# zzuiekongning/MGDT-YOLO

Measured on AMD Instinct MI355X. Metric: images/sec @640x640 bs=32 per GPU, detection forward + NMS (whole job: 1 GPU(s)), higher is better.
Workload: dtype bf16; 1 GPU; mspa_c2f_gd_yolov8-n (MSPA-C2f + GD neck + Detect, nc=80) 640x640 inference, batch 32/GPU: forward + decode + NMS(conf 0.25, iou 0.7), hipGraph replay, 4 batches in flight (one captured graph per resident batch, replayed round-robin on 4 streams); global_batch=32, parallelism=replicas x1 (batch-sharded, no data-path collective), rccl_ranks=1, input=bfloat16 NCHW images, 8 different batches resident in HBM (600 MiB) cycled, detections_last_step=9600, weights=seeded random init (no checkpoints offline), batches_in_flight=4

## Files before the change

include/mgdt.h:

```cpp
#ifndef MGDT_H
#define MGDT_H
#include <stddef.h>
#include <stdint.h>

#ifdef __cplusplus
extern "C" {
#endif

typedef void* mgdt_stream;

typedef enum { MGDT_OK = 0, MGDT_BAD_SHAPE = -1, MGDT_BAD_DTYPE = -2, MGDT_LAUNCH_FAIL = -3, MGDT_BAD_ARG = -4,
               MGDT_WORKSPACE = -5 } mgdt_status;
typedef enum { MGDT_F32 = 0, MGDT_BF16 = 1, MGDT_U8 = 2  } mgdt_dtype;
typedef enum { MGDT_ACT_NONE = 0, MGDT_ACT_SILU = 1, MGDT_ACT_RELU = 2, MGDT_ACT_GELU = 3 } mgdt_act;

typedef struct {
  void* p;
  int32_t n, h, w, c;
  int64_t sn, sh, sw, sc;
} mgdt_view;

const char* mgdt_last_error(void);
const char* mgdt_version(void);

// ... 55 lines not shown
                         float stride, int a_off, int a_total, const mgdt_view* feat, float* y, unsigned long long* best_keys,
                         const void* wb3, const float* bb3, mgdt_stream s);
int mgdt_detect_tail_aug_fwd(const mgdt_view* tb, const mgdt_view* tc, const void* wb, const float* bb, const void* wc, const float* bc, int nc,
                             float stride, int a_off, int a_total, const mgdt_view* feat, float* y, unsigned long long* best_keys,
                             const void* wb3, const float* bb3, float aug_scale, int aug_flip, float aug_img_w, mgdt_stream s);

int mgdt_scale_img_fwd(const mgdt_view* x, int x_dtype, int flip, int hs, int ws, float pad, const mgdt_view* y, int y_dtype, mgdt_stream s);

int mgdt_csp_block_supported(int mode, int cin, int cout, int wd, int nbtl, int h, int w, int dtype);
int mgdt_csp_block_tiles(int mode, int n, int cin, int cout, int wd, int nbtl, int h, int w, int* geom8);
int mgdt_csp_block_fwd(int mode, const mgdt_view* x, const void* front, const float* front_bias, const void* const* mid,
                       const float* const* mid_bias, int nbtl, int shortcut, const void* back, const float* back_bias, int wd, int act,
                       const mgdt_view* y, float* pool, int dtype, mgdt_stream s);

size_t mgdt_pw_chain_packed_bytes(int wd, int dtype);
int mgdt_pw_chain_pack(int idx, const float* w_oi, const float* conv_bias, const float* bn_gamma, const float* bn_beta, const float* bn_mean,
                       const float* bn_var, float bn_eps, int wd, int dtype, void* packed, mgdt_stream s);
int mgdt_pw_chain3_fwd(const mgdt_view* x, const void* packed, int wd, int act, const mgdt_view* y, int dtype, mgdt_stream s);

int mgdt_conv1x1_inject_supported(int cin, int cout, int h, int w, int hg, int wg, int dtype);
int mgdt_conv1x1_inject_fwd(const mgdt_view* x, const void* packed_w, const float* bias, const mgdt_view* ga, const mgdt_view* gf,
                            const mgdt_view* y, int dtype, mgdt_stream s);

int mgdt_conv1x1_inject_conv_supported(int cin, int cmid, int cout2, int h, int w, int hg, int wg, int dtype);
int mgdt_conv1x1_inject_conv_fwd(const mgdt_view* x, const void* packed_w, const float* bias, const mgdt_view* ga, const mgdt_view* gf,
                                 const mgdt_view* gsrc, const void* packed_wg, const float* bias_g, int cmid,
                                 const void* packed_w2, const float* bias2, int act2, const mgdt_view* y2, int dtype, mgdt_stream s);

size_t mgdt_groupnorm_workspace_bytes(int n, int c);
int mgdt_groupnorm_fwd(const mgdt_view* x, const float* gamma, const float* beta, int groups, float eps, int act, void* ws, const mgdt_view* y,
                       int dtype, mgdt_stream s);
int mgdt_tood_layer_attn_fwd(const float* sums, int n, int c, int hw, const float* w1, const float* b1, const float* w2, const float* b2, int hid,
                             int stacked, float* scale, mgdt_stream s);
int mgdt_dcnv2_fwd(const mgdt_view* x, const mgdt_view* offset_mask, const float* w_gemm, const float* bias, const mgdt_view* y, int dtype,
                   mgdt_stream s);
int mgdt_dcnv2_mfma_fwd(const mgdt_view* x, const mgdt_view* offset_mask, const void* packed_w, const mgdt_view* y, int dtype, mgdt_stream s);
int mgdt_pixel_gate_fwd(const mgdt_view* x, const mgdt_view* gate, const mgdt_view* y, int dtype, mgdt_stream s);

int mgdt_conv_pack_direct(const float* w_oihw, const float* conv_bias, const float* bn_gamma, const float* bn_beta,
                          const float* bn_mean, const float* bn_var, float bn_eps, int cin_g, int cout, int k,
                          float* w_out, float* bias_out, mgdt_stream s);
int mgdt_conv2d_direct_fwd(const mgdt_view* x, int x_dtype, const float* w_gemm, const float* bias, int k, int stride,
                           int groups, int act, const mgdt_view* y, int dtype, mgdt_stream s);
enum { MGDT_DIRECT_STEM = 0, MGDT_DIRECT_GENERIC = 1, MGDT_DIRECT_REFUSED = 2 };
int mgdt_conv2d_direct_route(const mgdt_view* x, int x_dtype, const mgdt_view* y, int dtype, int k, int stride, int groups, int* out);

#define MGDT_SPR_SPLITS 16
int mgdt_spr_pool_fwd(const mgdt_view* x, float* pooled, int dtype, mgdt_stream s);
int mgdt_spr_attn_fwd(const float* pooled, const float* fc1_w, const float* fc1_b, const float* fc2_w,
                      const float* fc2_b, int n, int c, int groups, int h, int w, int softmax, float* attn, mgdt_stream s);
int mgdt_scale_channels_fwd(const mgdt_view* x, const float* attn, const mgdt_view* y, int dtype, mgdt_stream s);
int mgdt_spr_attn_scale_fwd(const float* pooled, int nsplit, int tiles_x, int tiles_y, const float* fc1_w, const float* fc1_b, const float* fc2_w, const float* fc2_b, int groups,
                            const mgdt_view* x, const mgdt_view* y, const mgdt_view* pool_a, const mgdt_view* pool_b, int dtype, mgdt_stream s);

int mgdt_sppf_pool_fwd(const mgdt_view* x, const mgdt_view* y1, const mgdt_view* y2, const mgdt_view* y3, int dtype,
                       mgdt_stream s);

int mgdt_adaptive_avgpool_fwd(const mgdt_view* x, const mgdt_view* y, int dtype, mgdt_stream s);
int mgdt_bilinear_fwd(const mgdt_view* x, const mgdt_view* y, int dtype, mgdt_stream s);
int mgdt_nearest_fwd(const mgdt_view* x, const mgdt_view* y, int dtype, mgdt_stream s);
int mgdt_copy_fwd(const mgdt_view* x, int x_dtype, const mgdt_view* y, int y_dtype, mgdt_stream s);
int mgdt_image_pad4_fwd(const mgdt_view* x, int x_dtype, const mgdt_view* y, int y_dtype, mgdt_stream s);

int mgdt_space_to_depth2_channels(int c, int y_dtype);
int mgdt_conv_pack_stem6(const float* w6, const float* conv_bias, const float* bn_gamma, const float* bn_beta, const float* bn_mean, const float* bn_var,
                         float bn_eps, int c6, int cout, int dtype, void* packed_out, float* bias_out, mgdt_stream s);
int mgdt_space_to_depth2_fwd(const mgdt_view* x, int x_dtype, const mgdt_view* y, int y_dtype, mgdt_stream s);
int mgdt_stem6_wgrad_unpack(const float* dw3, int cout, int cin, int cp, float* dw6, mgdt_stream s);

#define MGDT_GRN_SPLITS 8
int mgdt_dwconv7_ln_fwd(const mgdt_view* x, const float* dw_w, const float* dw_b, const float* ln_w, const float* ln_b,
                        float eps, const mgdt_view* y, int dtype, mgdt_stream s);
int mgdt_grn_stats_fwd(const mgdt_view* t, const float* gamma, float* ws, float* scale, int dtype, mgdt_stream s);
enum { MGDT_DW_ROW8 = 0, MGDT_DW_ROW10 = 1, MGDT_DW_GENERIC = 2 };
int mgdt_dwconv7_ln_route(int n, int h, int w, int c, int dtype, int* out);

int mgdt_inject_fwd(const mgdt_view* local, const mgdt_view* ga, const mgdt_view* gf, const mgdt_view* y, int dtype,
                    mgdt_stream s);

int mgdt_detect_decode_fwd(const mgdt_view* feat, int reg_max, int nc, float stride, int a_off, int a_total, float* y,
                           int dtype, mgdt_stream s);
int mgdt_detect_decode_aug_fwd(const mgdt_view* feat, int reg_max, int nc, float stride, int a_off, int a_total, float* y,
                               unsigned long long* best_keys, float aug_scale, int aug_flip, float aug_img_w, int dtype, mgdt_stream s);

size_t mgdt_nms_workspace_bytes(int n, int nc, int a, int multi_label, int max_nms);
int mgdt_nms_fwd(const float* pred, int n, int nc, int a, float conf_thres, float iou_thres, const int32_t* classes,
                 int n_classes, int agnostic, int multi_label, int max_det, int max_nms, float max_wh, float* out,
                 int32_t* kept_anchor, int32_t* counts, const unsigned long long* best_keys, void* ws, size_t ws_bytes, mgdt_stream s);

int mgdt_nms_masks_fwd(const float* pred, int n, int nc, int nm, int a, float conf_thres, float iou_thres, const int32_t* classes,
                       int n_classes, int agnostic, int multi_label, int max_det, int max_nms, float max_wh, float* out,
                       int32_t* kept_anchor, int32_t* counts, const unsigned long long* best_keys, void* ws, size_t ws_bytes, mgdt_stream s);

int mgdt_deconv2x2_fwd(const mgdt_view* x, const void* const* packed4, const float* bias, const mgdt_view* y, int dtype, mgdt_stream s);
int mgdt_seg_concat_fwd(const float* y, int n, int rows, int a_total, const mgdt_view* const* mc, int n_levels, int nm, float* out, int dtype,
                        mgdt_stream s);
int mgdt_seg_mask_geometry(int win_h, int win_w, int out_h, int out_w, int* geom4);
int mgdt_seg_masks_fwd(const mgdt_view* protos, const float* rows, const int32_t* counts, const int32_t* offsets, int max_det, int nm,
                       int top, int left, int win_h, int win_w, int out_h, int out_w, int crop_before, float box_sx, float box_sy,
                       int crop_after, int no_skip, void* out, int out_u8, int dtype, mgdt_stream s);

int mgdt_pose_concat_fwd(const float* y, int n, int rows, int a_total, const mgdt_view* const* kpt, const float* strides, int n_levels, int nk,
                         int ndim, float* out, float* kpt_raw, int dtype, mgdt_stream s);
int mgdt_pose_scale_fwd(float* rows, const int32_t* counts, const float* meta, int n, int max_det, int lead, int nk, int ndim, mgdt_stream s);

size_t mgdt_mask_iou_workspace_bytes(int n, int max_det, int max_lab);
// ... 189 lines not shown
```

mgdt_yolo_amd/_lib.py:

```python
import ctypes as C
import os

_HERE = os.path.dirname(os.path.abspath(__file__))
LIB_PATH = os.environ.get('MGDT_LIB') or os.path.join(_HERE, 'csrc', 'libmgdt_hip.so')

F32, BF16 = 0, 1
ACT_NONE, ACT_SILU, ACT_RELU, ACT_GELU = 0, 1, 2, 3
SPR_SPLITS = 16
GRN_SPLITS = 8


class View(C.Structure):
    _fields_ = [('p', C.c_void_p), ('n', C.c_int32), ('h', C.c_int32), ('w', C.c_int32), ('c', C.c_int32),
                ('sn', C.c_int64), ('sh', C.c_int64), ('sw', C.c_int64), ('sc', C.c_int64)]


VP = C.POINTER(View)
_vp, _i, _f, _sz, _l = C.c_void_p, C.c_int, C.c_float, C.c_size_t, C.c_long

class PackDesc(C.Structure):
    _fields_ = [('w', C.c_void_p), ('conv_bias', C.c_void_p), ('bn_gamma', C.c_void_p), ('bn_beta', C.c_void_p), ('bn_mean', C.c_void_p), ('bn_var', C.c_void_p),
                ('bn_eps', C.c_float), ('cin', C.c_int32), ('cout', C.c_int32), ('k', C.c_int32), ('dtype', C.c_int32), ('mode', C.c_int32),
                ('packed', C.c_void_p), ('bias_out', C.c_void_p)]

# ... 9 lines not shown

ROUTE_X2, ROUTE_IN_SCALE, ROUTE_IN_SHIFT, ROUTE_R1, ROUTE_R2, ROUTE_FP8 = 1, 2, 4, 8, 16, 32
ROUTE_IGEMM, ROUTE_LDS3X3 = 0, 1
DIRECT_STEM, DIRECT_GENERIC, DIRECT_REFUSED = 0, 1, 2

PROTOTYPES = {
    'mgdt_last_error': (C.c_char_p, []),
    'mgdt_version': (C.c_char_p, []),
    'mgdt_conv_packed_bytes': (_sz, [_i, _i, _i, _i]),
    'mgdt_conv_pack': (_i, [_vp, _vp, _vp, _vp, _vp, _vp, _f, _i, _i, _i, _i, _vp, _vp, _vp]),
    'mgdt_conv2d_fwd': (_i, [VP, VP, _vp, _vp, _vp, _vp, _i, _i, _i, VP, VP, VP, _i, _vp]),
    'mgdt_conv_packed_bytes_fp8': (_sz, [_i, _i, _i]),
    'mgdt_conv_pack_fp8': (_i, [_vp, _vp, _vp, _vp, _vp, _vp, _f, _i, _i, _i, _f, _vp, _vp, _vp, _vp]),
    'mgdt_conv2d_fp8_fwd': (_i, [VP, VP, _vp, _vp, _vp, _vp, _vp, _f, _i, _i, _i, VP, VP, VP, _vp]),
    'mgdt_conv2d_route': (_i, [VP, VP, _i, _i, _i, _i, _i, C.POINTER(ConvRoute)]),
    'mgdt_conv_pack_batch': (_i, [_vp, _i, _vp]),
    'mgdt_conv2d_phase_fwd': (_i, [VP, _vp, _vp, _i, VP, VP, VP, _i, _vp]),
    'mgdt_conv_wgrad_splits': (_i, [_i, _i, _i]),
    'mgdt_wgrad_final_batch': (_i, [_vp, _i, _vp]),
    'mgdt_conv_pack_dgrad': (_i, [_vp, _i, _i, _i, _i, _i, _vp, _vp, _vp]),
    'mgdt_conv_pack_direct': (_i, [_vp, _vp, _vp, _vp, _vp, _vp, _f, _i, _i, _i, _vp, _vp, _vp]),
    'mgdt_conv2d_direct_fwd': (_i, [VP, _i, _vp, _vp, _i, _i, _i, _i, VP, _i, _vp]),
    'mgdt_conv2d_direct_route': (_i, [VP, _i, VP, _i, _i, _i, _i, C.POINTER(C.c_int)]),
    'mgdt_spr_pool_fwd': (_i, [VP, _vp, _i, _vp]),
    'mgdt_spr_attn_fwd': (_i, [_vp, _vp, _vp, _vp, _vp, _i, _i, _i, _i, _i, _i, _vp, _vp]),
    'mgdt_scale_channels_fwd': (_i, [VP, _vp, VP, _i, _vp]),
    'mgdt_sppf_pool_fwd': (_i, [VP, VP, VP, VP, _i, _vp]),
    'mgdt_adaptive_avgpool_fwd': (_i, [VP, VP, _i, _vp]),
    'mgdt_bilinear_fwd': (_i, [VP, VP, _i, _vp]),
    'mgdt_nearest_fwd': (_i, [VP, VP, _i, _vp]),
    'mgdt_copy_fwd': (_i, [VP, _i, VP, _i, _vp]),
    'mgdt_image_pad4_fwd': (_i, [VP, _i, VP, _i, _vp]),
    'mgdt_space_to_depth2_channels': (_i, [_i, _i]),
    'mgdt_space_to_depth2_fwd': (_i, [VP, _i, VP, _i, _vp]),
    'mgdt_conv_pack_stem6': (_i, [_vp, _vp, _vp, _vp, _vp, _vp, _f, _i, _i, _i, _vp, _vp, _vp]),
    'mgdt_stem6_wgrad_unpack': (_i, [_vp, _i, _i, _i, _vp, _vp]),
    'mgdt_dwconv7_ln_fwd': (_i, [VP, _vp, _vp, _vp, _vp, _f, VP, _i, _vp]),
    'mgdt_cnx_mlp_packed_bytes': (_sz, [_i, _i]),
    'mgdt_cnx_mlp_pack': (_i, [_vp, _vp, _vp, _vp, _i, _vp, _i, _vp]),
    'mgdt_cnx_mlp_workspace_bytes': (_sz, [_i, _i, _i, _i]),
    'mgdt_cnx_mlp_fwd': (_i, [VP, VP, _vp, _vp, _vp, _vp, VP, _i, _vp]),
    'mgdt_cnx_block_supported': (_i, [_i, _i, _i, _i, _i]),
    'mgdt_cnx_block_workspace_bytes': (_sz, [_i, _i, _i, _i]),
    'mgdt_cnx_block_geometry': (_i, [_i, _i, _i, C.POINTER(C.c_int)]),
    'mgdt_cnx_block_fwd': (_i, [VP, _vp, _vp, _vp, _vp, _f, _vp, _vp, _vp, _vp, _vp, _i, _vp, _sz, VP, _i, _vp]),
    'mgdt_pw_chain_packed_bytes': (_sz, [_i, _i]),
    'mgdt_pw_chain_pack': (_i, [_i, _vp, _vp, _vp, _vp, _vp, _vp, _f, _i, _i, _vp, _vp]),
    'mgdt_pw_chain3_fwd': (_i, [VP, _vp, _i, _i, VP, _i, _vp]),
    'mgdt_conv1x1_inject_supported': (_i, [_i, _i, _i, _i, _i, _i, _i]),
    'mgdt_conv1x1_inject_fwd': (_i, [VP, _vp, _vp, VP, VP, VP, _i, _vp]),
    'mgdt_conv1x1_inject_conv_supported': (_i, [_i, _i, _i, _i, _i, _i, _i, _i]),
    'mgdt_conv1x1_inject_conv_fwd': (_i, [VP, _vp, _vp, VP, VP, VP, _vp, _vp, _i, _vp, _vp, _i, VP, _i, _vp]),
    'mgdt_spr_attn_scale_fwd': (_i, [_vp, _i, _i, _i, _vp, _vp, _vp, _vp, _i, VP, VP, VP, VP, _i, _vp]),
    'mgdt_stem2_packed_bytes': (_sz, []),
    'mgdt_stem2_pack': (_i, [_vp, _vp, _vp]),
    'mgdt_stem2_fwd': (_i, [VP, _i, _vp, _vp, _vp, _vp, VP, _vp]),
    'mgdt_stem2_geometry': (_i, [_i, _i, _i, _i, C.POINTER(C.c_int)]),
    'mgdt_stem2_route': (_i, [VP, _i, VP, _i, C.POINTER(C.c_int)]),
    'mgdt_detect_tail_supported': (_i, [_i, _i, _i, _i, _i]),
    'mgdt_detect_tail_fwd': (_i, [VP, VP, _vp, _vp, _vp, _vp, _i, _f, _i, _i, VP, _vp, _vp, _vp, _vp, _vp]),
    'mgdt_detect_tail_aug_fwd': (_i, [VP, VP, _vp, _vp, _vp, _vp, _i, _f, _i, _i, VP, _vp, _vp, _vp, _vp, _f, _i, _f, _vp]),
    'mgdt_scale_img_fwd': (_i, [VP, _i, _i, _i, _i, _f, VP, _i, _vp]),
    'mgdt_csp_block_supported': (_i, [_i, _i, _i, _i, _i, _i, _i, _i]),
    'mgdt_csp_block_tiles': (_i, [_i, _i, _i, _i, _i, _i, _i, _i, _vp]),
    'mgdt_csp_block_fwd': (_i, [_i, VP, _vp, _vp, _vp, _vp, _i, _i, _vp, _vp, _i, _i, VP, _vp, _i, _vp]),
    'mgdt_groupnorm_workspace_bytes': (_sz, [_i, _i]),
    'mgdt_groupnorm_fwd': (_i, [VP, _vp, _vp, _i, _f, _i, _vp, VP, _i, _vp]),
    'mgdt_tood_layer_attn_fwd': (_i, [_vp, _i, _i, _i, _vp, _vp, _vp, _vp, _i, _i, _vp, _vp]),
    'mgdt_dcnv2_fwd': (_i, [VP, VP, _vp, _vp, VP, _i, _vp]),
    'mgdt_dcnv2_mfma_fwd': (_i, [VP, VP, _vp, VP, _i, _vp]),
    'mgdt_pixel_gate_fwd': (_i, [VP, VP, VP, _i, _vp]),
    'mgdt_gn_affine': (_i, [_vp, _vp, _i, _i, _i, _vp, _vp, _i, _f, _vp, _vp, _vp, _vp, _vp]),
    'mgdt_nc_affine_act_bwd': (_i, [VP, VP, _vp, _vp, _i, VP, _i, _vp]),
    'mgdt_gn_bwd_workspace_bytes': (_sz, [_i, _i]),
    'mgdt_gn_bwd_coef': (_i, [_vp, _vp, _vp, _vp, _vp, _i, _i, _i, _i, _vp, _vp, _vp, _vp, _vp, _i, _vp, _vp]),
    'mgdt_nc_axpby': (_i, [VP, _vp, VP, _vp, _vp, VP, _i, _vp]),
    'mgdt_pixel_gate_bwd': (_i, [VP, VP, VP, VP, VP, _i, _vp]),
    'mgdt_tood_layer_attn_bwd_workspace_bytes': (_sz, [_i, _i, _i, _i]),
    'mgdt_tood_layer_attn_bwd': (_i, [_vp, _vp, _i, _i, _i, _vp, _vp, _vp, _vp, _i, _i, _vp, _vp, _vp, _vp, _vp, _i, _vp, _vp]),
    'mgdt_dcn_im2col': (_i, [VP, VP, VP, _i, _vp]),
    'mgdt_dcn_col2im_bwd': (_i, [VP, VP, VP, _vp, VP, _i, _vp]),
    'mgdt_val_match_fwd': (_i, [_vp, _vp, _i, _i, _vp, _vp, _i, _vp, _i, _vp, _vp]),
    'mgdt_grn_stats_fwd': (_i, [VP, _vp, _vp, _vp, _i, _vp]),
    'mgdt_dwconv7_ln_route': (_i, [_i, _i, _i, _i, _i, C.POINTER(C.c_int)]),
    'mgdt_inject_fwd': (_i, [VP, VP, VP, VP, _i, _vp]),
    'mgdt_detect_decode_fwd': (_i, [VP, _i, _i, _f, _i, _i, _vp, _i, _vp]),
    'mgdt_detect_decode_aug_fwd': (_i, [VP, _i, _i, _f, _i, _i, _vp, _vp, _f, _i, _f, _i, _vp]),
    'mgdt_detect_loss_workspace_bytes': (_sz, [_i, _i, _i]),
    'mgdt_detect_loss_fwd': (_i, [_vp, _vp, _i, _i, _i, _vp, _i, _i, _f, _f, _f, _vp, _vp, _vp, _vp, _vp, _sz, _i, _vp]),
    'mgdt_detect_loss_fwd_dev': (_i, [_vp, _vp, _i, _i, _i, _vp, _i, _vp, _f, _f, _f, _vp, _vp, _vp, _vp, _vp, _sz, _i, _vp]),
    'mgdt_detect_loss_bwd': (_i, [_vp, _vp, _vp, _i, _i, _i, _vp, _i, _f, _f, _f, _f, _vp, _vp, _sz, _i, _vp]),
    'mgdt_reduce_workspace_bytes': (_sz, [_i]),
    'mgdt_bn_stats_fwd': (_i, [VP, _f, _f, _vp, _vp, _vp, _vp, _vp, _i, _vp]),
    'mgdt_bn_act_fwd': (_i, [VP, _vp, _vp, _vp, _vp, _i, VP, VP, VP, _i, _vp]),
    'mgdt_bn_act_bwd': (_i, [VP, VP, _vp, _vp, _vp, _vp, _i, _vp, _vp, VP, _vp, _i, _vp]),
    'mgdt_conv_dgrad': (_i, [VP, _vp, _i, _i, VP, _i, _i, _vp]),
    'mgdt_gconv_dgrad': (_i, [VP, _vp, _i, _i, _i, VP, _i, _i, _vp]),
    'mgdt_gconv_wgrad_workspace_bytes': (_sz, [_i, _i, _i, _i]),
    'mgdt_gconv_wgrad': (_i, [VP, VP, _i, _i, _i, _vp, _i, _vp, _i, _vp]),
    'mgdt_conv_wgrad_workspace_bytes': (_sz, [_i, _i, _i]),
    'mgdt_conv_wgrad': (_i, [VP, VP, VP, _i, _i, _vp, _vp, _i, _vp, _i, _vp]),
    'mgdt_add_fwd': (_i, [VP, VP, VP, _i, _vp]),
    'mgdt_maxpool5_bwd': (_i, [VP, VP, _vp, _i, _vp]),
    'mgdt_nearest_bwd': (_i, [VP, VP, _i, _vp]),
    'mgdt_ew_binary': (_i, [VP, VP, VP, _i, _i, _vp]),
    'mgdt_channel_affine': (_i, [VP, _vp, _vp, VP, _i, _vp]),
# ... 94 lines not shown
```

mgdt_yolo_amd/csrc/conv3x3_lds.hip:

```cpp
#include <type_traits>
#include <vector>

#include "common.h"

#define C3_OOB ((int)0x80000000)
#define C3_TW 16
#define C3_RW 18
#define C3_MAXI 14

struct C3Args {
  const char* x; int xsn, xsh, xsw; uint32_t x_bytes;
  char* y; int ysn, ysh, ysw; uint32_t y_bytes;
  const char* wpk; const float* bias;
  int N, H, W, Ho, Wo, Cin, Cout, CP, nchunks, NTtot, ncg, tiles_x, tiles_per_img, ntiles, XP, act;
  FastDiv fd_tpi, fd_tx, fd_cp;
  const float* oscale; float xq;
  unsigned long long* dbg;
};

template <int ACT> __device__ __forceinline__ float c3_act(float v) {
  if (ACT == MGDT_ACT_SILU) return v * fast_sigmoid(v);
  if (ACT == MGDT_ACT_RELU) return fmaxf(v, 0.f);
  return v;
}

template <int NBW, int ACT, int NCH, int MT, bool Q8 = false, int S = 1, int WS = 1>
__global__ __launch_bounds__(256 * WS, 1) void conv3x3_lds_kernel(const C3Args a) {
  constexpr int NTHR = 256 * WS, NBH = (NBW + WS - 1) / WS;
  constexpr int RW = 15 * S + 3, TH = 4 * MT, RH = (TH - 1) * S + 3, RPX = RH * RW;
  constexpr int MAXI = ((S == 1 ? C3_MAXI : 18) + WS - 1) / WS;
  constexpr int WB = Q8 ? 512 : 1024, PB = Q8 ? 8 : 16;
  extern __shared__ __attribute__((aligned(16))) char c3_lds[];
  int* tab = (int*)c3_lds;
  char* wl = c3_lds + (((size_t)a.nchunks * 16 + 15) & ~(size_t)15);
  char* xs = wl + (size_t)a.nchunks * NBW * WB;
  const int tid = threadIdx.x, lane = tid & 63, r = lane & 15, g = lane >> 4;
  const int wave_all = __builtin_amdgcn_readfirstlane(tid >> 6);
  const int wave = wave_all & 3, wcol = wave_all >> 2;
  const int cg = blockIdx.x % a.ncg, w0 = blockIdx.x / a.ncg, wstep = gridDim.x / a.ncg;
  const int nb0 = cg * NBW;
  const __amdgpu_buffer_rsrc_t xrs = __builtin_amdgcn_make_buffer_rsrc((void*)a.x, 0, a.x_bytes, 0x00020000);
  const __amdgpu_buffer_rsrc_t yrs = __builtin_amdgcn_make_buffer_rsrc((void*)a.y, 0, a.y_bytes, 0x00020000);

  for (int p = tid; p < a.nchunks * 4; p += NTHR) {
    const int tap = (int)fdiv((uint32_t)p, a.fd_cp), cp = p - tap * a.CP;
    tab[p] = tap < 9 ? ((tap / 3) * RW + (tap % 3)) * a.XP + cp * PB : 0;
  }
  constexpr int WV = WB / 16;
  {
    const int total = a.nchunks * NBW * WV;
    for (int i0 = tid; i0 < total; i0 += 8 * NTHR) {
      uint4 t[8];
#pragma unroll
      for (int u = 0; u < 8; ++u) {
        const int i = min(i0 + u * NTHR, total - 1);
        const int kc = i / (NBW * WV), rem = i - kc * NBW * WV, bw = rem / WV, ln = rem % WV;
        const bool ok = nb0 + bw < a.NTtot;
        t[u] = ok ? *(const uint4*)(a.wpk + ((size_t)(kc * a.NTtot + nb0 + bw) * WV + ln) * 16) : make_uint4(0u, 0u, 0u, 0u);
      }
#pragma unroll
      for (int u = 0; u < 8; ++u)
        if (i0 + u * NTHR < total) *(uint4*)(wl + (size_t)(i0 + u * NTHR) * 16) = t[u];
    }
  }
  const int nbw0 = nb0 + wcol * NBH;
  f32x4 bias[NBH], osc[Q8 ? NBH : 1];
#pragma unroll
  for (int bw = 0; bw < NBH; ++bw) {
    bias[bw] = nbw0 + bw < a.NTtot ? *(const f32x4*)(a.bias + (nbw0 + bw) * 16 + 4 * g) : f32x4{0.f, 0.f, 0.f, 0.f};
    if constexpr (Q8) {
      osc[bw] = nbw0 + bw < a.NTtot ? *(const f32x4*)(a.oscale + (nbw0 + bw) * 16 + 4 * g) : f32x4{1.f, 1.f, 1.f, 1.f};
      bias[bw] = bias[bw] / osc[bw];
    }
  }

  const int nitems = RPX * a.CP;
  uint4 stage[MAXI];
  auto issue = [&](int t) {
    const int n = (int)fdiv((uint32_t)t, a.fd_tpi), rt = t - n * a.tiles_per_img;
    const int tyi = (int)fdiv((uint32_t)rt, a.fd_tx), txi = rt - tyi * a.tiles_x;
    const int iy0 = tyi * TH * S - 1, ix0 = txi * C3_TW * S - 1;
#pragma unroll
    for (int u = 0; u < MAXI; ++u) {
      const int it = tid + u * NTHR;
      const int pix = (int)fdiv((uint32_t)it, a.fd_cp), c8 = it - pix * a.CP;
      const int py = pix / RW, px = pix - py * RW;
      const int iy = iy0 + py, ix = ix0 + px;
      const bool ok = it < nitems && (unsigned)iy < (unsigned)a.H && (unsigned)ix < (unsigned)a.W;
      stage[u] = __builtin_bit_cast(uint4, __builtin_amdgcn_raw_buffer_load_b128(xrs, ok ? (uint32_t)(n * a.xsn + iy * a.xsh + ix * a.xsw + c8 * 16) : (uint32_t)C3_OOB, 0, 0));
    }
  };
  auto commit = [&]() {
#pragma unroll
    for (int u = 0; u < MAXI; ++u) {
      const int it = tid + u * NTHR;
      if (it < nitems) {
        const int pix = (int)fdiv((uint32_t)it, a.fd_cp), c8 = it - pix * a.CP;
        if constexpr (Q8) *(long*)(xs + pix * a.XP + c8 * 8) = quant8(__builtin_bit_cast(bf16x8, stage[u]), a.xq);
        else *(uint4*)(xs + pix * a.XP + c8 * 16) = stage[u];
      }
    }
  };

  const char* const wlane = wl + lane * PB;
  int bbase[MT];
#pragma unroll
  for (int m = 0; m < MT; ++m) bbase[m] = ((wave * MT + m) * S * RW + r * S) * a.XP;

  __builtin_amdgcn_s_waitcnt(0x0F70);
  unsigned long long T0 = 0, Tc = 0, Tm = 0, Te = 0, tl = 0, ntl = 0;
  if (a.dbg) { T0 = __builtin_amdgcn_s_memrealtime(); tl = T0; }
  int t = w0;
  if (t < a.ntiles) issue(t);
  while (t < a.ntiles) {
    __syncthreads();
    commit();
    __syncthreads();
    if (a.dbg) { const unsigned long long n_ = __builtin_amdgcn_s_memrealtime(); Tc += n_ - tl; tl = n_; }
    const int tn = t + wstep;
    if (tn < a.ntiles) issue(tn);

    f32x4 acc[NBH][MT];
#pragma unroll
    for (int bw = 0; bw < NBH; ++bw)
#pragma unroll
      for (int m = 0; m < MT; ++m) acc[bw][m] = bias[bw];
    typedef typename std::conditional<Q8, long, bf16x8>::type frag_t;
    frag_t A[2][NBH], B[2][MT];
    auto load_frags = [&](int kc, int buf) {
      const int off = tab[kc * 4 + g];
#pragma unroll
      for (int bw = 0; bw < NBH; ++bw) A[buf][bw] = *(const frag_t*)(wlane + (size_t)(kc * NBW + wcol * NBH + bw) * WB);
#pragma unroll
      for (int m = 0; m < MT; ++m) B[buf][m] = *(const frag_t*)(xs + bbase[m] + off);
    };
    auto mm = [&](frag_t w, frag_t p, f32x4 c) __attribute__((always_inline)) {
      if constexpr (Q8) return mma_q8(w, p, c);
      else return __builtin_amdgcn_mfma_f32_16x16x32_bf16(w, p, c, 0, 0, 0);
    };
    load_frags(0, 0);
    if (NCH > 0) {
#pragma unroll
      for (int kc = 0; kc < NCH; ++kc) {
        if (kc + 1 < NCH) load_frags(kc + 1, (kc + 1) & 1);
#pragma unroll
        for (int bw = 0; bw < NBH; ++bw)
#pragma unroll
          for (int m = 0; m < MT; ++m) acc[bw][m] = mm(A[kc & 1][bw], B[kc & 1][m], acc[bw][m]);
      }
    } else {
      for (int kc = 0; kc < a.nchunks; kc += 2) {
        if (kc + 1 < a.nchunks) load_frags(kc + 1, 1);
#pragma unroll
        for (int bw = 0; bw < NBH; ++bw)
#pragma unroll
          for (int m = 0; m < MT; ++m) acc[bw][m] = mm(A[0][bw], B[0][m], acc[bw][m]);
        if (kc + 1 < a.nchunks) {
          if (kc + 2 < a.nchunks) load_frags(kc + 2, 0);
#pragma unroll
          for (int bw = 0; bw < NBH; ++bw)
#pragma unroll
            for (int m = 0; m < MT; ++m) acc[bw][m] = mm(A[1][bw], B[1][m], acc[bw][m]);
        }
      }
    }

    if (a.dbg) { const unsigned long long n_ = __builtin_amdgcn_s_memrealtime(); Tm += n_ - tl; tl = n_; }
    {
      const int n = (int)fdiv((uint32_t)t, a.fd_tpi), rt = t - n * a.tiles_per_img;
      const int tyi = (int)fdiv((uint32_t)rt, a.fd_tx), txi = rt - tyi * a.tiles_x;
#pragma unroll
      for (int m = 0; m < MT; ++m) {
        const int oy = tyi * TH + wave * MT + m, ox = txi * C3_TW + r;
// ... 8 lines not shown
          __builtin_amdgcn_raw_buffer_store_b64(__builtin_bit_cast(__attribute__((__vector_size__(2 * sizeof(unsigned int)))) unsigned int, o), yrs,
                                                (pin && co < a.Cout) ? (uint32_t)(po + co * 2) : (uint32_t)C3_OOB, 0, 0);
        }
      }
    }
    if (a.dbg) { const unsigned long long n_ = __builtin_amdgcn_s_memrealtime(); Te += n_ - tl; tl = n_; ++ntl; }
    t = tn;
  }
  if (a.dbg && tid == 0) { unsigned long long* d = a.dbg + (size_t)blockIdx.x * 6; d[0] = T0; d[1] = tl; d[2] = Tc; d[3] = Tm; d[4] = Te; d[5] = ntl; }
}

bool mgdt_conv3x3_lds_plan(const mgdt_view* x, const mgdt_view* y, int act, int CP, int nchunks, int NTtot, bool q8, int stride, C3Plan* p) {
  static const int mode = getenv("MGDT_CONV3_LDS") ? atoi(getenv("MGDT_CONV3_LDS")) : 1;
  if (!mode) return false;
  static const bool ws2 = !(getenv("MGDT_C3_WAVES8") && atoi(getenv("MGDT_C3_WAVES8")) == 0);
  const bool wide = mode >= 3 || ws2;
  const int Cin = x->c, Cout = y->c;
  if (stride == 2 && (q8 || Cin > 64 || NTtot % 4 || (nchunks != 9 && !(nchunks == 18 && wide)))) return false;
  if (Cin % 8 || Cin < 32 || Cin > 80 || Cout % 4 || Cout < 32 || (act != MGDT_ACT_SILU && act != MGDT_ACT_NONE && act != MGDT_ACT_RELU)) return false;
  const long M = (long)x->n * x->h * x->w;
  if (M < 16 * 1024 || x->h < 16 || x->w < 16) return false;
  p->extx = ((long)(x->n - 1) * x->sn + (long)(x->h - 1) * x->sh + (long)(x->w - 1) * x->sw + x->c) * 2;
  p->exty = ((long)(y->n - 1) * y->sn + (long)(y->h - 1) * y->sh + (long)(y->w - 1) * y->sw + y->c) * 2;
  if (p->extx >= 0x7fffffffL || p->exty >= 0x7fffffffL) return false;
  p->XP = q8 ? Cin + 16 : Cin * 2 + 16;
  const int NBW = stride == 2 ? 4 : NTtot;
  if (NBW != 2 && NBW != 3 && NBW != 4 && NBW != 5 && NBW != 6) return false;
  p->NBW = NBW;
  p->ncg = NTtot / NBW;
  const size_t fixed = (((size_t)nchunks * 16 + 15) & ~(size_t)15) + (size_t)nchunks * NBW * (q8 ? 512 : 1024);
  auto region = [&](int mt) { return stride == 2 ? (size_t)(8 * mt + 1) * 33 * p->XP : (size_t)(4 * mt + 2) * C3_RW * p->XP; };
  int MT = stride == 2 ? 2 : 4;
  if (stride == 1 && fixed + region(MT) > 160 * 1024) MT = NBW == 5 && !q8 && wide && fixed + region(3) <= 160 * 1024 ? 3 : 2;
  p->lds = fixed + region(MT);
  if (p->lds > 160 * 1024) return false;
  if (NBW == 5 && !q8 && MT == 2 && mode < 2) return false;
  if (stride == 1 && (q8 ? MT != 4 : ((NBW == 5 && MT == 4) || (NBW != 5 && MT != 4)))) return false;
  p->MT = MT;
  const int TH = 4 * MT;
  p->tiles_x = cdiv(y->w, C3_TW);
  p->tiles_per_img = p->tiles_x * cdiv(y->h, TH);
  p->ntiles = x->n * p->tiles_per_img;
  if ((stride == 2 ? (2 * TH + 1) * 33 * CP > 256 * 18 : (TH + 2) * C3_RW * CP > 256 * C3_MAXI)) return false;
  int nwg = 256 / p->ncg * p->ncg;
  nwg = (int)std::min<long>(nwg, (long)p->ntiles * p->ncg);
  nwg = nwg / p->ncg * p->ncg;
  if (nwg < p->ncg) return false;
  p->nwg = nwg;
  p->waves = q8 ? 4 : (ws2 && (stride == 2 || NBW == 6 || NBW == 4 || (NBW == 5 && MT == 3))) ? 8 : 4;
  return true;
}

bool mgdt_conv3x3_lds_launch(const mgdt_view* x, const mgdt_view* y, const void* packed_w, const float* bias, int act, int CP, int nchunks, int NTtot, hipStream_t st,
                             const float* q8_oscale, float q8_xq, int stride) {
  const bool q8 = q8_oscale != nullptr;
  C3Plan pl;
  if (!mgdt_conv3x3_lds_plan(x, y, act, CP, nchunks, NTtot, q8, stride, &pl)) return false;
  const int Cin = x->c, Cout = y->c, NBW = pl.NBW, MT = pl.MT, nwg = pl.nwg;
  const size_t lds = pl.lds;
  const bool ws2 = pl.waves == 8;
  C3Args a;
  memset(&a, 0, sizeof(a));
  a.x = (const char*)x->p; a.xsn = (int)(x->sn * 2); a.xsh = (int)(x->sh * 2); a.xsw = (int)(x->sw * 2); a.x_bytes = (uint32_t)pl.extx;
  a.y = (char*)y->p; a.ysn = (int)(y->sn * 2); a.ysh = (int)(y->sh * 2); a.ysw = (int)(y->sw * 2); a.y_bytes = (uint32_t)pl.exty;
  a.wpk = (const char*)packed_w; a.bias = bias;
  a.N = x->n; a.H = x->h; a.W = x->w; a.Ho = y->h; a.Wo = y->w; a.Cin = Cin; a.Cout = Cout; a.CP = CP; a.nchunks = nchunks; a.NTtot = NTtot; a.act = act;
  a.XP = pl.XP;
  a.oscale = q8_oscale; a.xq = q8_xq;
  a.ncg = pl.ncg;
  a.tiles_x = pl.tiles_x; a.tiles_per_img = pl.tiles_per_img; a.ntiles = pl.ntiles;
  a.fd_tpi = make_fastdiv((uint32_t)a.tiles_per_img); a.fd_tx = make_fastdiv((uint32_t)a.tiles_x); a.fd_cp = make_fastdiv((uint32_t)CP);
 #define C3_LAUNCH_Q8(NB, ACTV)                                                                                      \
  {                                                                                                                  \
    static std::atomic<bool> qattr{false}, qattr18{false}, qattr23{false};                                            \
    if (nchunks == 18) {                                                                                             \
      if (!qattr18) { (void)hipFuncSetAttribute((const void*)conv3x3_lds_kernel<NB, ACTV, 18, 4, true>, hipFuncAttributeMaxDynamicSharedMemorySize, 160 * 1024); qattr18 = true; } \
      conv3x3_lds_kernel<NB, ACTV, 18, 4, true><<<nwg, 256, lds, st>>>(a);                                           \
    } else if (nchunks == 23) {                                                                                      \
      if (!qattr23) { (void)hipFuncSetAttribute((const void*)conv3x3_lds_kernel<NB, ACTV, 23, 4, true>, hipFuncAttributeMaxDynamicSharedMemorySize, 160 * 1024); qattr23 = true; } \
      conv3x3_lds_kernel<NB, ACTV, 23, 4, true><<<nwg, 256, lds, st>>>(a);                                           \
    } else {                                                                                                         \
      if (!qattr) { (void)hipFuncSetAttribute((const void*)conv3x3_lds_kernel<NB, ACTV, 0, 4, true>, hipFuncAttributeMaxDynamicSharedMemorySize, 160 * 1024); qattr = true; } \
      conv3x3_lds_kernel<NB, ACTV, 0, 4, true><<<nwg, 256, lds, st>>>(a);                                            \
    }                                                                                                                \
  }
#define C3_ACT_Q8(NB) \
  if (act == MGDT_ACT_SILU) C3_LAUNCH_Q8(NB, MGDT_ACT_SILU) else if (act == MGDT_ACT_RELU) C3_LAUNCH_Q8(NB, MGDT_ACT_RELU) else C3_LAUNCH_Q8(NB, MGDT_ACT_NONE)
#define C3_LAUNCH(NB, ACTV, MTV, WSV)                                                                                     \
  {                                                                                                                  \
    static std::atomic<bool> attr{false}, attr18{false}, attr23{false};                                                                        \
    if (nchunks == 18) {                                                                                             \
      if (!attr18) { (void)hipFuncSetAttribute((const void*)conv3x3_lds_kernel<NB, ACTV, 18, MTV, false, 1, WSV>, hipFuncAttributeMaxDynamicSharedMemorySize, 160 * 1024); attr18 = true; } \
      conv3x3_lds_kernel<NB, ACTV, 18, MTV, false, 1, WSV><<<nwg, 256 * WSV, lds, st>>>(a);                                                    \
    } else if (nchunks == 23) {                                                                                      \
      if (!attr23) { (void)hipFuncSetAttribute((const void*)conv3x3_lds_kernel<NB, ACTV, 23, MTV, false, 1, WSV>, hipFuncAttributeMaxDynamicSharedMemorySize, 160 * 1024); attr23 = true; } \
      conv3x3_lds_kernel<NB, ACTV, 23, MTV, false, 1, WSV><<<nwg, 256 * WSV, lds, st>>>(a);                                               \
    } else {                                                                                                         \
      if (!attr) { (void)hipFuncSetAttribute((const void*)conv3x3_lds_kernel<NB, ACTV, 0, MTV, false, 1, WSV>, hipFuncAttributeMaxDynamicSharedMemorySize, 160 * 1024); attr = true; } \
      conv3x3_lds_kernel<NB, ACTV, 0, MTV, false, 1, WSV><<<nwg, 256 * WSV, lds, st>>>(a);                                                     \
    }                                                                                                                \
  }
#define C3_ACT(NB, MTV, WSV) \
  if (act == MGDT_ACT_SILU) C3_LAUNCH(NB, MGDT_ACT_SILU, MTV, WSV) else if (act == MGDT_ACT_RELU) C3_LAUNCH(NB, MGDT_ACT_RELU, MTV, WSV) else C3_LAUNCH(NB, MGDT_ACT_NONE, MTV, WSV)
  static unsigned long long* dbgbuf = nullptr;
  if (getenv("MGDT_C3_DBG") && !dbgbuf) (void)hipMalloc((void**)&dbgbuf, 256 * 6 * 8);
  a.dbg = dbgbuf;
#define C3_LAUNCH_S2(ACTV, NCHV)                                                                                      \
  {                                                                                                                  \
    static std::atomic<bool> sattr{false}, sattr8{false};                                                            \
    if (ws2) {                                                                                                       \
      if (!sattr8) { (void)hipFuncSetAttribute((const void*)conv3x3_lds_kernel<4, ACTV, NCHV, 2, false, 2, 2>, hipFuncAttributeMaxDynamicSharedMemorySize, 160 * 1024); sattr8 = true; } \
      conv3x3_lds_kernel<4, ACTV, NCHV, 2, false, 2, 2><<<nwg, 512, lds, st>>>(a);                                   \
    } else {                                                                                                         \
      if (!sattr) { (void)hipFuncSetAttribute((const void*)conv3x3_lds_kernel<4, ACTV, NCHV, 2, false, 2>, hipFuncAttributeMaxDynamicSharedMemorySize, 160 * 1024); sattr = true; } \
      conv3x3_lds_kernel<4, ACTV, NCHV, 2, false, 2><<<nwg, 256, lds, st>>>(a);                                      \
    }                                                                                                                \
  }
#define C3_ACT_S2(NCHV) \
  if (act == MGDT_ACT_SILU) C3_LAUNCH_S2(MGDT_ACT_SILU, NCHV) else if (act == MGDT_ACT_RELU) C3_LAUNCH_S2(MGDT_ACT_RELU, NCHV) else C3_LAUNCH_S2(MGDT_ACT_NONE, NCHV)
  if (stride == 2) {
    if (nchunks == 9) { C3_ACT_S2(9) } else { C3_ACT_S2(18) }
  } else if (q8) {
    if (NBW == 6) { C3_ACT_Q8(6) } else if (NBW == 5) { C3_ACT_Q8(5) } else if (NBW == 4) { C3_ACT_Q8(4) } else if (NBW == 3) { C3_ACT_Q8(3) } else { C3_ACT_Q8(2) }
  } else if (ws2 && (NBW == 6 || NBW == 4 || (NBW == 5 && MT == 3))) {
    if (NBW == 6) { C3_ACT(6, 4, 2) } else if (NBW == 4) { C3_ACT(4, 4, 2) } else { C3_ACT(5, 3, 2) }
  } else if (NBW == 6) { C3_ACT(6, 4, 1) } else if (NBW == 5 && MT == 3) { C3_ACT(5, 3, 1) } else if (NBW == 5) { C3_ACT(5, 2, 1) } else if (NBW == 4) { C3_ACT(4, 4, 1) } else if (NBW == 3) { C3_ACT(3, 4, 1) } else { C3_ACT(2, 4, 1) }
#undef C3_ACT
#undef C3_ACT_Q8
#undef C3_ACT_S2
#undef C3_LAUNCH_S2
#undef C3_LAUNCH_Q8
#undef C3_LAUNCH
  if (dbgbuf) {
    std::vector<unsigned long long> h(256 * 6);
    (void)hipStreamSynchronize(st);
    (void)hipMemcpy(h.data(), dbgbuf, h.size() * 8, hipMemcpyDeviceToHost);
    unsigned long long t0 = ~0ull, t1 = 0; double c = 0, m = 0, e = 0, nt = 0;
    for (int i = 0; i < nwg; ++i) { t0 = std::min(t0, h[i * 6]); t1 = std::max(t1, h[i * 6 + 1]); c += h[i * 6 + 2]; m += h[i * 6 + 3]; e += h[i * 6 + 4]; nt += h[i * 6 + 5]; }
    fprintf(stderr, "conv3x3_lds cin %d cout %d %dx%d: %d wgs, %d tiles, span %.1f us; per tile (us): wait+commit %.2f mfma %.2f epilogue %.2f\n", Cin, Cout, x->h, x->w, nwg,
            a.ntiles, (t1 - t0) * 0.01, c / nt * 0.01, m / nt * 0.01, e / nt * 0.01);
  }
  return true;
}
```

mgdt_yolo_amd/csrc/conv_igemm.hip:

```cpp
#include "conv_igemm_kernel.h"

struct FoldArgs { const float *cb, *g, *b, *mu, *var; float eps; int cout_real, cpad; float* bias_out; };
__device__ __forceinline__ float stem6_weight(const float* __restrict__ w6, int c6, int cout, int cs, int tap) {
  const int q = cs / c6, ci = cs - q * c6;
  return q < 4 ? w6[(((long)cout * c6 + ci) * 6 + 2 * (tap / 3) + (q >> 1)) * 6 + 2 * (tap % 3) + (q & 1)] : 0.f;
}
template <typename T>
__global__ void pack_kernel(const float* __restrict__ w, const float* __restrict__ scale, int Cin, int Cout, int KS,
                            int CP, int nchunks, int NTtot, T* __restrict__ out, int dgrad = 0, FoldArgs fa = FoldArgs{}) {
  constexpr int PE = Piece<T>::PE;
  long total = (long)nchunks * NTtot * 64 * PE;
  if (fa.bias_out && blockIdx.x == 0)
    for (int c = threadIdx.x; c < fa.cpad; c += blockDim.x) {
      float bo = 0.f;
      if (c < fa.cout_real) {
        if (fa.g) {
          const float s = fa.g[c] / sqrtf(fa.eps + fa.var[c]);
          bo = fa.b[c] - fa.g[c] * fa.mu[c] / sqrtf(fa.var[c] + fa.eps);
          if (fa.cb) bo += s * fa.cb[c];
        } else if (fa.cb) {
          bo = fa.cb[c];
        }
      }
      fa.bias_out[c] = bo;
// ... 259 lines not shown
    int cin = cp * PE + j, cout = nb * 16 + r;
    float v = 0.f;
    if (tap < KS * KS && cin < Cin && cout < Cout) {
      if (dgrad == 1) v = w[(((long)cin * Cout + cout) * KS + (KS - 1 - tap / KS)) * KS + (KS - 1 - tap % KS)];
      else if (dgrad >= 6) v = stem6_weight(w, dgrad - 5, cout, cin, tap);
      else if (dgrad >= 2) {
        const int py = (dgrad - 2) >> 1, px = (dgrad - 2) & 1;
        const int ky = py + 1 - 2 * (tap / KS - 1), kx = px + 1 - 2 * (tap % KS - 1);
        v = ((unsigned)ky < 3u && (unsigned)kx < 3u) ? w[(((long)cin * Cout + cout) * 3 + ky) * 3 + kx] : 0.f;
      }
      else v = w[(((long)cout * Cin + cin) * KS + tap / KS) * KS + tap % KS];
      if (fa.g) v *= fa.g[cout] / sqrtf(fa.eps + fa.var[cout]);
    }
    out[i] = (T)v;
  }
}

extern "C" int mgdt_conv_pack_batch(const mgdt_pack_desc* d, int n, mgdt_stream s) {
  if (!d || n < 0) MGDT_FAIL(MGDT_BAD_ARG, "conv_pack_batch: null descriptor array");
  hipStream_t st = (hipStream_t)s;
  for (int dtype : {MGDT_F32, MGDT_BF16}) {
    PackJobs jobs;
    int m = 0;
    auto flush = [&]() {
      if (!m) return;
      for (int q = m; q < PACK_BATCH; ++q) { jobs.j[q] = jobs.j[0]; jobs.j[q].nchunks = 0; jobs.j[q].fa.bias_out = nullptr; }
      if (dtype == MGDT_F32) pack_batch_kernel<float><<<dim3(32, m), 256, 0, st>>>(jobs);
      else pack_batch_kernel<bf16><<<dim3(32, m), 256, 0, st>>>(jobs);
      m = 0;
    };
    for (int i = 0; i < n; ++i) {
      const mgdt_pack_desc& e = d[i];
      if (e.dtype != dtype) continue;
      if (!e.w || !e.packed || !e.bias_out) MGDT_FAIL(MGDT_BAD_ARG, "conv_pack_batch: descriptor %d has a null pointer", i);
      if (e.mode < 0 || e.mode > 9 || (e.mode >= 2 && e.k != 3) || (e.mode >= 6 && e.cin != e.mode - 5))
        MGDT_FAIL(MGDT_BAD_SHAPE, "conv_pack_batch: descriptor %d mode %d", i, e.mode);
      PackJob& J = jobs.j[m++];
      const bool stem6 = e.mode >= 6, fwd = e.mode == 0 || stem6;
      const int gi = stem6 ? stem6_channels(e.cin, dtype) : fwd ? e.cin : e.cout, go = fwd ? e.cout : e.cin;
      conv_geometry(gi, go, e.k, dtype, &J.CP, &J.nchunks, &J.NTtot, (e.mode >= 2 && !stem6) ? phase_ntaps(e.mode) : 0);
      J.w = e.w; J.Cin = gi; J.Cout = go; J.KS = e.k; J.dgrad = e.mode; J.out = e.packed;
      J.fa = fwd ? FoldArgs{e.conv_bias, e.bn_gamma, e.bn_beta, e.bn_mean, e.bn_var, e.bn_eps, go, J.NTtot * 16, e.bias_out}
                         : FoldArgs{nullptr, nullptr, nullptr, nullptr, nullptr, 0.f, go, J.NTtot * 16, e.bias_out};
      if (m == PACK_BATCH) flush();
    }
    flush();
  }
  MGDT_CHECK_LAUNCH("conv_pack_batch");
  return MGDT_OK;
}

bool mgdt_conv3x3_lds_plan(const mgdt_view* x, const mgdt_view* y, int act, int CP, int nchunks, int NTtot, bool q8, int stride, C3Plan* p);
bool mgdt_conv3x3_lds_launch(const mgdt_view* x, const mgdt_view* y, const void* packed_w, const float* bias, int act, int CP, int nchunks, int NTtot, hipStream_t st,
                             const float* q8_oscale, float q8_xq, int stride);

template <typename T, int NT, int MT, bool Q8>
int launch_igemm(const ConvArgs& a, const IgemmPlan& p, hipStream_t st);

template <typename T>
static int dispatch_igemm(const ConvArgs& a, const IgemmPlan& p, hipStream_t st) {
  const int NT = p.NT, MT = p.MT;
#define CASE(nt, mt) \
  if (NT == nt && MT == mt) return launch_igemm<T, nt, mt, false>(a, p, st);
  CASE(1, 2) CASE(1, 4) CASE(2, 2) CASE(3, 2) CASE(4, 2) CASE(5, 2) CASE(6, 2) CASE(8, 2)
#undef CASE
  MGDT_FAIL(MGDT_BAD_SHAPE, "conv2d: no kernel for NT=%d MT=%d", NT, MT);
}

static int dispatch_igemm_q8(const ConvArgs& a, const IgemmPlan& p, hipStream_t st) {
  const int NT = p.NT;
#define CASE(nt) \
  if (NT == nt) return launch_igemm<bf16, nt, 2, true>(a, p, st);
  CASE(1) CASE(2) CASE(3) CASE(4) CASE(5) CASE(6) CASE(8)
#undef CASE
  MGDT_FAIL(MGDT_BAD_SHAPE, "conv2d_fp8: no kernel for NT=%d", NT);
}

static int conv_check_shapes(const mgdt_view* x, const mgdt_view* y, int k, int stride, int dtype, int* Ho_, int* Wo_) {
  if (dtype != MGDT_F32 && dtype != MGDT_BF16) MGDT_FAIL(MGDT_BAD_DTYPE, "conv2d: dtype %d", dtype);
  if ((k != 1 && k != 3) || (stride != 1 && stride != 2)) MGDT_FAIL(MGDT_BAD_SHAPE, "conv2d: k=%d stride=%d unsupported", k, stride);
  const int pe = piece_elems(dtype);
  const int pad = k / 2;
  const int Ho = (x->h + 2 * pad - k) / stride + 1, Wo = (x->w + 2 * pad - k) / stride + 1;
  if (y->n != x->n || y->h != Ho || y->w != Wo) MGDT_FAIL(MGDT_BAD_SHAPE, "conv2d: y is %dx%dx%d, expected %dx%dx%d", y->n, y->h, y->w, x->n, Ho, Wo);
  if (x->c % pe || y->c % 4) MGDT_FAIL(MGDT_BAD_SHAPE, "conv2d: cin=%d must be a multiple of %d and cout=%d of 4", x->c, pe, y->c);
  *Ho_ = Ho; *Wo_ = Wo;
  return MGDT_OK;
}
static inline bool conv_view_aligned(const mgdt_view* v, int q, int dtype) {
  return v->sc == 1 && v->sw % q == 0 && v->sh % q == 0 && v->sn % q == 0 && ((uintptr_t)v->p % (q * dtype_size(dtype))) == 0;
}
static inline bool conv_lds_candidate(int tapmode, int dtype, int k, bool x2, bool in_scale, bool in_shift, bool r1, bool r2) {
  return tapmode == 0 && dtype == MGDT_BF16 && k == 3 && !x2 && !in_scale && !in_shift && !r1 && !r2;
}
static int igemm_plan(int nchunks, int NTtot, long M, bool q8, bool extra, IgemmPlan* p) {
  const int WB = q8 ? 512 : 1024;
  int LDS_PANEL_KIB = 144;
  { const char* e = getenv("MGDT_CONV_PANEL_KIB"); if (e) LDS_PANEL_KIB = atoi(e); }
  int NT = 1;
  for (int c : {8, 6, 5, 4, 3, 2, 1})
    if (NTtot % c == 0 && (long)nchunks * c * WB <= LDS_PANEL_KIB * 1024L) { NT = c; break; }
  int MT = 2;
  if (!q8 && NT == 1 && NTtot == 1) { const char* e = getenv("MGDT_CONV_MT1"); MT = e && atoi(e) == 4 ? 4 : 2; }
  int waves = 8;
  auto wgs = [&](int nt, int wv) { return (long)cdiv(M, 16 * wv * MT) * (NTtot / nt); };
  {
    const char* e = getenv("MGDT_CONV_MINWG");
    const int minwg = e ? atoi(e) : 128;
    while (wgs(NT, waves) < minwg && NT > 1 && NT % 2 == 0) NT /= 2;
  }
  {
    static const bool tail_split = getenv("MGDT_CONV_TAIL_SPLIT") != nullptr;
    const long w0 = wgs(NT, waves);
    if (tail_split && w0 > 768 && w0 <= 960 && NT % 2 == 0) NT /= 2;
  }
  {
    const char* e;
    if ((e = getenv("MGDT_CONV_WAVES"))) waves = std::min(8, std::max(1, atoi(e)));
  }
  p->numTiles = cdiv(M, 16 * waves * MT);
  p->T8 = cdiv(p->numTiles, 8);
  p->tab_bytes = (nchunks + 3) / 4 * 4 * 4 * 16;
  size_t panel = (size_t)nchunks * NT * WB;
  if (panel <= (size_t)LDS_PANEL_KIB * 1024) { p->seg_chunks = nchunks; p->nseg = 1; }
  else { p->seg_chunks = 64; p->nseg = cdiv(nchunks, p->seg_chunks); }
  p->lds = p->tab_bytes + (size_t)(q8 ? 2 : 1) * NT * 16 * sizeof(float) + (size_t)p->seg_chunks * NT * WB;
  int gcap = waves == 8 ? 256 : 1024;
  { const char* e = getenv("MGDT_CONV_GCAP"); if (e) gcap = atoi(e); }
  if (p->lds > 160 * 1024) MGDT_FAIL(MGDT_BAD_SHAPE, "conv2d: %zu bytes of LDS for NT=%d, %d chunks", p->lds, NT, p->seg_chunks);
  p->gx = std::min(8 * p->T8, gcap); p->gy = NTtot / NT;
  p->NT = NT; p->MT = MT; p->waves = waves;
  p->D = nchunks >= 3 ? 4 : 2;
  p->extra = extra;
  return MGDT_OK;
}

static int conv2d_fwd_impl(const mgdt_view* x, const mgdt_view* x2, const float* in_scale, const float* in_shift,
                           const void* packed_w, const float* bias, int k, int stride, int act, const mgdt_view* r1,
                           const mgdt_view* r2, const mgdt_view* y, int dtype, int tapmode, mgdt_stream s,
                           const float* q8_oscale = nullptr, float q8_xq = 1.f);
extern "C" int mgdt_conv2d_fwd(const mgdt_view* x, const mgdt_view* x2, const float* in_scale, const float* in_shift,
                               const void* packed_w, const float* bias, int k, int stride, int act, const mgdt_view* r1,
                               const mgdt_view* r2, const mgdt_view* y, int dtype, mgdt_stream s) {
  return conv2d_fwd_impl(x, x2, in_scale, in_shift, packed_w, bias, k, stride, act, r1, r2, y, dtype, 0, s);
}
extern "C" int mgdt_conv2d_phase_fwd(const mgdt_view* x, const void* packed_w, const float* bias, int phase, const mgdt_view* r1, const mgdt_view* r2,
// ... 6 lines not shown
                                   const mgdt_view* r1, const mgdt_view* r2, const mgdt_view* y, mgdt_stream s) {
  if (!oscale) MGDT_FAIL(MGDT_BAD_ARG, "conv2d_fp8: null oscale");
  if (!(x_qscale > 0.f) || !(x_qscale < 3.0e38f)) MGDT_FAIL(MGDT_BAD_ARG, "conv2d_fp8: x_qscale must be a positive finite number");
  return conv2d_fwd_impl(x, x2, in_scale, in_shift, packed_w, bias, k, stride, act, r1, r2, y, MGDT_BF16, 0, s, oscale, x_qscale);
}
static int conv2d_fwd_impl(const mgdt_view* x, const mgdt_view* x2, const float* in_scale, const float* in_shift,
                           const void* packed_w, const float* bias, int k, int stride, int act, const mgdt_view* r1,
                           const mgdt_view* r2, const mgdt_view* y, int dtype, int tapmode, mgdt_stream s,
                           const float* q8_oscale, float q8_xq) {
  const bool q8 = q8_oscale != nullptr;
  if (!view_ok(x) || !view_ok(y) || !packed_w || !bias) MGDT_FAIL(MGDT_BAD_ARG, "conv2d: null/empty view or weights");
  int Ho, Wo;
  if (int rc = conv_check_shapes(x, y, k, stride, dtype, &Ho, &Wo)) return rc;
  const int pe = piece_elems(dtype);
  const int pad = k / 2;
  auto aligned = [&](const mgdt_view* v, int q) { return conv_view_aligned(v, q, dtype); };
  if (!aligned(x, pe) || !aligned(y, 4)) MGDT_FAIL(MGDT_BAD_SHAPE, "conv2d: x/y must be NHWC views (sc==1) with 16-byte aligned pieces");
  if (x2 && x2->p && (x2->n != x->n || x2->h != x->h || x2->w != x->w || x2->c != x->c || !aligned(x2, pe)))
    MGDT_FAIL(MGDT_BAD_SHAPE, "conv2d: x2 must match x");
  for (const mgdt_view* rr : {r1, r2})
    if (rr && rr->p && (rr->n != y->n || rr->h != Ho || rr->w != Wo || rr->c != y->c || !aligned(rr, 4)))
      MGDT_FAIL(MGDT_BAD_SHAPE, "conv2d: residual must match y");

  ConvArgs a;
  memset(&a, 0, sizeof(a));
  const long sz = (long)dtype_size(dtype);
  auto extent = [&](const mgdt_view* v) { return ((long)(v->n - 1) * v->sn + (long)(v->h - 1) * v->sh + (long)(v->w - 1) * v->sw + v->c) * sz; };
  bool fits = true;
  auto bind = [&](const mgdt_view* v, const char** p, int* sn, int* sh, int* sw, uint32_t* bytes) {
    if (!v || !v->p) return;
    if (extent(v) >= 0x7fffffffL || v->sh * sz >= (1L << 23) || v->sw * sz >= (1L << 23)) { fits = false; return; }
    *p = (const char*)v->p; *sn = (int)(v->sn * sz); *sh = (int)(v->sh * sz); *sw = (int)(v->sw * sz); *bytes = (uint32_t)extent(v);
  };
  const char* yp = nullptr;
  bind(x, &a.x, &a.xsn, &a.xsh, &a.xsw, &a.x_bytes);
  bind(x2, &a.x2, &a.x2sn, &a.x2sh, &a.x2sw, &a.x2_bytes);
  bind(y, &yp, &a.ysn, &a.ysh, &a.ysw, &a.y_bytes);
  bind(r1, &a.r1, &a.r1sn, &a.r1sh, &a.r1sw, &a.r1_bytes);
  bind(r2, &a.r2, &a.r2sn, &a.r2sh, &a.r2sw, &a.r2_bytes);
  if (!fits) MGDT_FAIL(MGDT_BAD_SHAPE, "conv2d: a view spans >= 2 GiB or has a row stride >= 8 MiB");
  a.y = (char*)yp;
  a.in_scale = in_scale; a.in_shift = in_shift;
  a.wpk = (const char*)packed_w; a.bias = bias;
  a.oscale = q8_oscale; a.xq = q8_xq;
  a.N = x->n; a.H = x->h; a.W = x->w; a.Cin = x->c; a.Ho = Ho; a.Wo = Wo; a.Cout = y->c;
  a.KS = k; a.stride = stride; a.pad = pad; a.act = act;
  a.ntaps = tapmode >= 2 ? phase_ntaps(tapmode) : k * k;
  a.taplist = phase_taplist(tapmode, k);
  conv_geometry(a.Cin, a.Cout, k, dtype, &a.CP, &a.nchunks, &a.NTtot, tapmode >= 2 ? a.ntaps : 0);
  long M = (long)a.N * Ho * Wo;
  if (M > 0x7fffffffL - (1 << 20)) MGDT_FAIL(MGDT_BAD_SHAPE, "conv2d: problem too large");
  a.M = (int)M; a.HoWo = Ho * Wo;
  a.fd_howo = make_fastdiv((uint32_t)a.HoWo); a.fd_wo = make_fastdiv((uint32_t)Wo);
  if (conv_lds_candidate(tapmode, dtype, k, x2 && x2->p, in_scale, in_shift, r1 && r1->p, r2 && r2->p) &&
      mgdt_conv3x3_lds_launch(x, y, packed_w, bias, act, a.CP, a.nchunks, a.NTtot, (hipStream_t)s, q8_oscale, q8_xq, stride)) {
    MGDT_CHECK_LAUNCH("conv2d(3x3 lds)");
    return MGDT_OK;
  }

  IgemmPlan pl;
  if (int rc = igemm_plan(a.nchunks, a.NTtot, M, q8, a.x2 || a.in_scale || a.in_shift, &pl)) return rc;
  a.numTiles = pl.numTiles; a.T8 = pl.T8; a.tab_bytes = pl.tab_bytes; a.seg_chunks = pl.seg_chunks; a.nseg = pl.nseg;
  hipStream_t st = (hipStream_t)s;
  if (q8) return dispatch_igemm_q8(a, pl, st);
  if (dtype == MGDT_F32) return dispatch_igemm<float>(a, pl, st);
  return dispatch_igemm<bf16>(a, pl, st);
}

extern "C" int mgdt_conv2d_route(const mgdt_view* x, const mgdt_view* y, int k, int stride, int dtype, int flags, int act, mgdt_conv_route* out) {
  if (!x || !y || !out || x->n <= 0 || x->h <= 0 || x->w <= 0 || x->c <= 0 || y->c <= 0) MGDT_FAIL(MGDT_BAD_ARG, "conv2d_route: null/empty view");
  const bool q8 = flags & MGDT_ROUTE_FP8;
  if (q8 && dtype != MGDT_BF16) MGDT_FAIL(MGDT_BAD_DTYPE, "conv2d_route: the fp8 kernels take bf16 views");
  int Ho, Wo;
  if (int rc = conv_check_shapes(x, y, k, stride, dtype, &Ho, &Wo)) return rc;
  mgdt_view xv = *x, yv = *y;
  xv.p = yv.p = nullptr;
  if (!conv_view_aligned(&xv, piece_elems(dtype), dtype) || !conv_view_aligned(&yv, 4, dtype))
    MGDT_FAIL(MGDT_BAD_SHAPE, "conv2d: x/y must be NHWC views (sc==1) with 16-byte aligned pieces");
  int CP, nchunks, NTtot;
  conv_geometry(x->c, y->c, k, dtype, &CP, &nchunks, &NTtot);
  const long M = (long)x->n * Ho * Wo;
  if (M > 0x7fffffffL - (1 << 20)) MGDT_FAIL(MGDT_BAD_SHAPE, "conv2d: problem too large");
  memset(out, 0, sizeof(*out));
  out->nchunks = nchunks;
  C3Plan c3;
  if (conv_lds_candidate(0, dtype, k, flags & MGDT_ROUTE_X2, flags & MGDT_ROUTE_IN_SCALE, flags & MGDT_ROUTE_IN_SHIFT, flags & MGDT_ROUTE_R1, flags & MGDT_ROUTE_R2) &&
      mgdt_conv3x3_lds_plan(&xv, &yv, act, CP, nchunks, NTtot, q8, stride, &c3)) {
    out->family = MGDT_ROUTE_LDS3X3;
    out->NBW = c3.NBW; out->tile_rows = 4 * c3.MT; out->ncg = c3.ncg; out->nwg = c3.nwg; out->ntiles = c3.ntiles; out->waves = c3.waves;
    out->lds_bytes = (int)c3.lds;
    return MGDT_OK;
  }
  IgemmPlan pl;
  if (int rc = igemm_plan(nchunks, NTtot, M, q8, flags & (MGDT_ROUTE_X2 | MGDT_ROUTE_IN_SCALE | MGDT_ROUTE_IN_SHIFT), &pl)) return rc;
  out->family = MGDT_ROUTE_IGEMM;
  out->NT = pl.NT; out->MT = pl.MT; out->D = pl.D; out->extra = pl.extra; out->nseg = pl.nseg; out->seg_chunks = pl.seg_chunks; out->waves = pl.waves;
  out->gx = pl.gx; out->gy = pl.gy; out->numTiles = pl.numTiles; out->lds_bytes = (int)pl.lds;
  out->ragged = NTtot * 16 > y->c;
  return MGDT_OK;
}
```

mgdt_yolo_amd/csrc/conv_igemm_kernel.h:

```cpp
#pragma once
#include <stdlib.h>

#include <type_traits>

#include "common.h"

template <typename T> struct Piece;
template <> struct Piece<float> { static constexpr int PE = 4; typedef f32x4 frag; };
template <> struct Piece<bf16> { static constexpr int PE = 8; typedef bf16x8 frag; };

struct ConvArgs {
  const char* x; int xsn, xsh, xsw;
  const char* x2; int x2sn, x2sh, x2sw;
  const float* in_scale; const float* in_shift;
  const char* wpk; const float* bias;
  char* y; int ysn, ysh, ysw;
  const char* r1; int r1sn, r1sh, r1sw;
  const char* r2; int r2sn, r2sh, r2sw;
  int N, H, W, Cin, Ho, Wo, Cout;
  int KS, stride, pad, CP, nchunks, NTtot, act;
  int M, HoWo, numTiles, T8, seg_chunks, nseg, tab_bytes;
  FastDiv fd_howo, fd_wo;
  uint32_t x_bytes, x2_bytes, y_bytes, r1_bytes, r2_bytes;
  int ntaps; unsigned long long taplist;
// ... 132 lines not shown
  const __amdgpu_buffer_rsrc_t x2rs = __builtin_amdgcn_make_buffer_rsrc((void*)(a.x2 ? a.x2 : a.x), 0, a.x2 ? a.x2_bytes : 0u, 0x00020000);
  const __amdgpu_buffer_rsrc_t yrs = __builtin_amdgcn_make_buffer_rsrc((void*)a.y, 0, a.y_bytes, 0x00020000);
  const __amdgpu_buffer_rsrc_t r1rs = __builtin_amdgcn_make_buffer_rsrc((void*)(a.r1 ? a.r1 : a.x), 0, a.r1 ? a.r1_bytes : 0u, 0x00020000);
  const __amdgpu_buffer_rsrc_t r2rs = __builtin_amdgcn_make_buffer_rsrc((void*)(a.r2 ? a.r2 : a.x), 0, a.r2 ? a.r2_bytes : 0u, 0x00020000);

  auto setup = [&](int v, TileState(&S)[MT]) __attribute__((always_inline)) {
    const int tile = (v & 7) * a.T8 + (v >> 3);
    const bool tv = (v >> 3) < a.T8 && tile < a.numTiles;
#pragma unroll
    for (int mt = 0; mt < MT; ++mt) {
      const int m0 = tv ? tile * BM + (wave * MT + mt) * 16 : 0;
      const bool pv = tv && m0 + r < a.M;
      int n, oy, ox, n0 = 0;
      bool bump = false;
      const bool fast = a.Wo >= 16;
      if (fast) {
        n0 = (int)fdiv((uint32_t)m0, a.fd_howo);
        const int rem = m0 - n0 * a.HoWo;
        const int oy0 = (int)fdiv((uint32_t)rem, a.fd_wo), ox0 = rem - oy0 * a.Wo;
        oy = oy0; ox = ox0 + r;
        if (ox >= a.Wo) { ox -= a.Wo; ++oy; }
        if (oy >= a.Ho) { oy = 0; bump = true; }
        n = n0 + (bump ? 1 : 0);
      } else {
        const int mm = pv ? m0 + r : 0;
        n = (int)fdiv((uint32_t)mm, a.fd_howo);
        const int rem = mm - n * a.HoWo;
        oy = (int)fdiv((uint32_t)rem, a.fd_wo); ox = rem - oy * a.Wo;
      }
      auto nmul = [&](int s) __attribute__((always_inline)) { return fast ? n0 * s + (bump ? s : 0) : n * s; };
      TileState t;
      t.pn = n;
      const int iy0 = (oy << ssh) - a.pad, ix0 = (ox << ssh) - a.pad;
      t.xo = nmul(a.xsn) + __mul24(iy0, a.xsh) + __mul24(ix0, a.xsw);
      t.yo = pv ? nmul(a.ysn) + __mul24(oy, a.ysh) + __mul24(ox, a.ysw) : MGDT_OOB;
      t.x2o = t.r1o = t.r2o = 0;
      if (EXTRA && a.x2) t.x2o = nmul(a.x2sn) + __mul24(iy0, a.x2sh) + __mul24(ix0, a.x2sw);
      if (a.r1) t.r1o = pv ? nmul(a.r1sn) + __mul24(oy, a.r1sh) + __mul24(ox, a.r1sw) : MGDT_OOB;
      if (a.r2) t.r2o = pv ? nmul(a.r2sn) + __mul24(oy, a.r2sh) + __mul24(ox, a.r2sw) : MGDT_OOB;
      uint32_t mask = 1u;
      if (a.KS == 3) {
        const uint32_t rm = (uint32_t)((unsigned)iy0 < (unsigned)a.H) | ((uint32_t)((unsigned)(iy0 + 1) < (unsigned)a.H) << 1) |
                            ((uint32_t)((unsigned)(iy0 + 2) < (unsigned)a.H) << 2);
        const uint32_t cm = (uint32_t)((unsigned)ix0 < (unsigned)a.W) | ((uint32_t)((unsigned)(ix0 + 1) < (unsigned)a.W) << 1) |
                            ((uint32_t)((unsigned)(ix0 + 2) < (unsigned)a.W) << 2);
        mask = ((rm & 1u) ? cm : 0u) | ((rm & 2u) ? cm << 3 : 0u) | ((rm & 4u) ? cm << 6 : 0u);
      }
      t.vm = pv ? mask : 0u;
      S[mt] = t;
    }
  };

  auto load_chunk = [&](const uint4* ep, const TileState(&S)[MT], frag(&P)[MT]) __attribute__((always_inline)) {
    uint32_t ex, ey, ez = 0, ew = 0;
    if (EXTRA) { const uint4 e = *ep; ex = e.x; ey = e.y; ez = e.z; ew = e.w; }
    else { const uint2 e = *(const uint2*)ep; ex = e.x; ey = e.y; }
#pragma unroll
    for (int mt = 0; mt < MT; ++mt) {
      const bool ok = (S[mt].vm >> ey) & 1u;
      const uint32_t off = ok ? (uint32_t)S[mt].xo + ex : (uint32_t)MGDT_OOB;
      frag v = __builtin_bit_cast(frag, __builtin_amdgcn_raw_buffer_load_b128(xrs, off, 0, 0));
      if (EXTRA) {
        if (a.x2) {
          const uint32_t off2 = ok ? (uint32_t)S[mt].x2o + ez : (uint32_t)MGDT_OOB;
          v = frag_add<T>(v, __builtin_bit_cast(frag, __builtin_amdgcn_raw_buffer_load_b128(x2rs, off2, 0, 0)));
        }
        if (ok && (a.in_scale || a.in_shift))
          v = frag_affine<T>(v, a.in_scale ? a.in_scale + (long)S[mt].pn * a.Cin + ew : nullptr, a.in_shift ? a.in_shift + ew : nullptr);
      }
      P[mt] = v;
    }
  };

  f32x4 acc[NT][MT];
  auto init_acc = [&]() __attribute__((always_inline)) {
#pragma unroll
    for (int nt = 0; nt < NT; ++nt) {
      const f32x4 b = *(const f32x4*)(blds + nt * 16 + 4 * g);
#pragma unroll
      for (int mt = 0; mt < MT; ++mt) acc[nt][mt] = b;
    }
  };
  auto compute = [&](const char* wp, const frag(&P)[MT]) __attribute__((always_inline)) {
    if constexpr (Q8) {
      long Pq[MT];
#pragma unroll
      for (int mt = 0; mt < MT; ++mt) Pq[mt] = quant8(P[mt], a.xq);
#pragma unroll
      for (int nt = 0; nt < NT; ++nt) {
        const long Wq = *(const long*)(wp + nt * WB);
#pragma unroll
        for (int mt = 0; mt < MT; ++mt) acc[nt][mt] = mma_q8(Wq, Pq[mt], acc[nt][mt]);
      }
    } else {
#pragma unroll
      for (int nt = 0; nt < NT; ++nt) {
        const frag Wf = *(const frag*)(wp + nt * WB);
#pragma unroll
        for (int mt = 0; mt < MT; ++mt) acc[nt][mt] = mma(Wf, P[mt], acc[nt][mt]);
      }
    }
  };
  const bool ragged = (nb0 + NT) * 16 > a.Cout;
  constexpr bool WIDE = std::is_same<T, bf16>::value && NT >= 4;
  constexpr int NTW = WIDE ? NT / 4 * 4 : 0;
  auto epilogue_act = [&](const TileState(&S)[MT], auto actf) __attribute__((always_inline)) {
    if constexpr (WIDE) {
      if (!ragged) {
        const bool odd = (g & 1) != 0, hi = (g & 2) != 0;
        const int pA = (lane ^ 16) << 2, pB = (lane ^ 32) << 2;
        auto xch = [&](int addr, uint2 v) __attribute__((always_inline)) {
          return make_uint2((unsigned)__builtin_amdgcn_ds_bpermute(addr, (int)v.x), (unsigned)__builtin_amdgcn_ds_bpermute(addr, (int)v.y));
        };
#pragma unroll
        for (int mt = 0; mt < MT; ++mt) {
#pragma unroll
          for (int q = 0; q < NTW / 4; ++q) {
            uint2 a4[4], c4[4];
#pragma unroll
            for (int j = 0; j < 4; ++j) {
              const int nt = 4 * q + j;
              const int cob = ((nb0 + nt) * 16 + 4 * g) * SZ;
              f32x4 v = acc[nt][mt];
              if constexpr (Q8) v *= *(const f32x4*)(olds + nt * 16 + 4 * g);
// ... 7 lines not shown
              a4[j] = __builtin_bit_cast(uint2, o);
            }
#pragma unroll
            for (int h = 0; h < 2; ++h) {
              const uint2 x = xch(pA, odd ? a4[2 * h] : a4[2 * h + 1]);
              c4[2 * h] = odd ? x : a4[2 * h];
              c4[2 * h + 1] = odd ? a4[2 * h + 1] : x;
            }
            const uint2 x0 = xch(pB, hi ? c4[0] : c4[2]), x1 = xch(pB, hi ? c4[1] : c4[3]);
            const uint2 b0 = hi ? x0 : c4[0], b1 = hi ? x1 : c4[1], b2 = hi ? c4[2] : x0, b3 = hi ? c4[3] : x1;
            const uint32_t off = (uint32_t)S[mt].yo + (uint32_t)(((nb0 + 4 * q + g) * 16) * SZ);
            typedef __attribute__((__vector_size__(4 * sizeof(unsigned int)))) unsigned int u32x4v;
            __builtin_amdgcn_raw_buffer_store_b128(u32x4v{b0.x, b0.y, b1.x, b1.y}, yrs, off, 0, 0);
            __builtin_amdgcn_raw_buffer_store_b128(u32x4v{b2.x, b2.y, b3.x, b3.y}, yrs, off + 16u, 0, 0);
          }
        }
      }
    }
    const int nt_first = (WIDE && !ragged) ? NTW : 0;
#pragma unroll
    for (int mt = 0; mt < MT; ++mt) {
#pragma unroll
      for (int nt = 0; nt < NT; ++nt) {
        if (nt < nt_first) continue;
        const int cob = ((nb0 + nt) * 16 + 4 * g) * SZ;
        const int dead = (ragged && cob >= a.Cout * SZ) ? MGDT_OOB : 0;
        f32x4 v = acc[nt][mt];
        if constexpr (Q8) v *= *(const f32x4*)(olds + nt * 16 + 4 * g);
#pragma unroll
        for (int j = 0; j < 4; ++j) v[j] = actf(v[j]);
        if (a.r1) v += bload4<T>(r1rs, (uint32_t)(S[mt].r1o | dead) + cob);
        if (a.r2) v += bload4<T>(r2rs, (uint32_t)(S[mt].r2o | dead) + cob);
        bstore4<T>(yrs, (uint32_t)(S[mt].yo | dead) + cob, v);
      }
    }
  };
  auto epilogue = [&](const TileState(&S)[MT]) __attribute__((always_inline)) {
    switch (a.act) {
      case MGDT_ACT_SILU: epilogue_act(S, [](float v) { return v * fast_sigmoid(v); }); break;
      case MGDT_ACT_RELU: epilogue_act(S, [](float v) { return fmaxf(v, 0.f); }); break;
      case MGDT_ACT_GELU: epilogue_act(S, [](float v) { return 0.5f * v * (1.0f + erff(v * 0.70710678118654752f)); }); break;
      default: epilogue_act(S, [](float v) { return v; }); break;
    }
  };

  TileState cur[MT], nxt[MT];
  int tile = blockIdx.x;
  setup(tile, cur);
  frag P[D][MT];
  const uint4* tab_g = ptab + g;
  load_chunk(tab_g, cur, P[0]);
  if constexpr (L > 1) load_chunk(tab_g + 4, cur, P[1]);
  if constexpr (L > 2) load_chunk(tab_g + 8, cur, P[2]);
  if (!MULTI) { stage(0); __syncthreads(); }
  const char* const wlane = wlds + lane * (WB / 64);
  constexpr bool multi = MULTI;

  for (; tile < 8 * a.T8; tile += gridDim.x) {
    init_acc();
    const uint4* tp = tab_g + 4 * L;
    const char* wp = wlane;
    int kl = 0;
    auto step_cur = [&](int j, auto dtag) __attribute__((always_inline)) {
      constexpr int d = decltype(dtag)::value;
      load_chunk(tp, cur, P[(d + L) % D]);
      tp += 4;
      if (multi && kl == 0) { __syncthreads(); stage(j / a.seg_chunks); __syncthreads(); wp = wlane; }
      compute(wp, P[d]);
      wp += NT * WB;
      if (multi && ++kl == a.seg_chunks) kl = 0;
    };
    int j0 = 0;
    for (; j0 < nchp - D; j0 += D) {
      step_cur(j0, std::integral_constant<int, 0>{});
      step_cur(j0 + 1, std::integral_constant<int, 1>{});
      if constexpr (D > 2) step_cur(j0 + 2, std::integral_constant<int, 2>{});
      if constexpr (D > 3) step_cur(j0 + 3, std::integral_constant<int, 3>{});
    }
    setup(tile + gridDim.x, nxt);
    step_cur(j0, std::integral_constant<int, 0>{});
    auto step_last = [&](int j, auto dtag) __attribute__((always_inline)) {
      constexpr int d = decltype(dtag)::value;
      load_chunk(tab_g + 4 * (d - 1), nxt, P[(d + L) % D]);
      if (j < a.nchunks) {
        if (multi && kl == 0) { __syncthreads(); stage(j / a.seg_chunks); __syncthreads(); wp = wlane; }
        compute(wp, P[d]);
        wp += NT * WB;
        if (multi && ++kl == a.seg_chunks) kl = 0;
      }
    };
    step_last(j0 + 1, std::integral_constant<int, 1>{});
    if constexpr (D > 2) step_last(j0 + 2, std::integral_constant<int, 2>{});
    if constexpr (D > 3) step_last(j0 + 3, std::integral_constant<int, 3>{});
    epilogue(cur);
#pragma unroll
    for (int mt = 0; mt < MT; ++mt) cur[mt] = nxt[mt];
  }
}

struct IgemmPlan { int NT, MT, D, extra, waves, gx, gy, numTiles, T8, tab_bytes, seg_chunks, nseg; size_t lds; };

template <typename T, int NT, int MT, bool Q8 = false>
int launch_igemm(const ConvArgs& a, const IgemmPlan& p, hipStream_t st) {
  static std::atomic<bool> attr_set{false};
  constexpr bool M1 = NT == 1;
  const void* ks[8] = {(const void*)conv_igemm_kernel<T, NT, MT, 2, false, false, Q8>, (const void*)conv_igemm_kernel<T, NT, MT, 4, false, false, Q8>,
                       (const void*)conv_igemm_kernel<T, NT, MT, 2, true, false, Q8>,  (const void*)conv_igemm_kernel<T, NT, MT, 4, true, false, Q8>,
                       (const void*)conv_igemm_kernel<T, NT, MT, 2, false, M1, Q8>,    (const void*)conv_igemm_kernel<T, NT, MT, 4, false, M1, Q8>,
                       (const void*)conv_igemm_kernel<T, NT, MT, 2, true, M1, Q8>,     (const void*)conv_igemm_kernel<T, NT, MT, 4, true, M1, Q8>};
  if (!attr_set) {
    for (const void* k : ks) {
      hipError_t e = hipFuncSetAttribute(k, hipFuncAttributeMaxDynamicSharedMemorySize, 160 * 1024);
      if (e != hipSuccess) MGDT_FAIL(MGDT_LAUNCH_FAIL, "conv2d: hipFuncSetAttribute: %s", hipGetErrorString(e));
    }
    attr_set = true;
  }
  void* kargs[] = {(void*)&a};
  hipError_t le = hipLaunchKernel(ks[(p.nseg > 1 ? 4 : 0) + (p.extra ? 2 : 0) + (p.D == 4 ? 1 : 0)], dim3(p.gx, p.gy), dim3(p.waves * 64), kargs, p.lds, st);
  if (le != hipSuccess) MGDT_FAIL(MGDT_LAUNCH_FAIL, "conv2d: launch: %s", hipGetErrorString(le));
  MGDT_CHECK_LAUNCH("conv2d_fwd");
  return MGDT_OK;
}


#define MGDT_IGEMM_INSTANTIATE(T, nt) template int launch_igemm<T, nt, 2>(const ConvArgs&, const IgemmPlan&, hipStream_t);
#define MGDT_IGEMM_INSTANTIATE_Q8(nt) template int launch_igemm<bf16, nt, 2, true>(const ConvArgs&, const IgemmPlan&, hipStream_t);
```

mgdt_yolo_amd/csrc/pointwise.hip:

```cpp
#include <algorithm>
#include <vector>

#include <type_traits>
#include "common.h"

#define SPR_SPLITS 16

static inline int grid_for(long work, int block = 256, int cap = 8192) { return (int)std::min<long>((work + block - 1) / block, cap); }

struct PixIdx { FastDiv fq, fw, fh; int Q, W, H; };
static inline PixIdx make_pixidx(int H, int W, int Q) { return PixIdx{make_fastdiv((uint32_t)Q), make_fastdiv((uint32_t)W), make_fastdiv((uint32_t)H), Q, W, H}; }
__device__ __forceinline__ void decode_idx(uint32_t i, const PixIdx& d, int& n, int& h, int& w, int& q) {
  uint32_t t = fdiv(i, d.fq);
  q = (int)(i - t * d.Q);
  uint32_t t2 = fdiv(t, d.fw);
  w = (int)(t - t2 * d.W);
  uint32_t t3 = fdiv(t2, d.fh);
  h = (int)(t2 - t3 * d.H);
  n = (int)t3;
}
template <typename T, int V> __device__ __forceinline__ void ldv(const T* p, float (&v)[V]) {
#pragma unroll
  for (int k = 0; k < V; k += 4) {
    f32x4 t = load4<T>(p + k);
// ... 361 lines not shown
  __syncthreads();
  for (int o = tid; o < C * 5; o += 256) {
    const int cc = o % C, k = o / C, gi = cc / cw, ci = cc - gi * cw;
    float sum = 0.f;
    for (int p = 0; p < ph; ++p) sum += red[k * 256 + p * C + cc];
    pvec[gi * L + (k == 0 ? ci : cw + 4 * ci + (k - 1))] = sum / cnt[k];
  }
  __syncthreads();
  SPR_STAMP();
  const int nout = G * hid;
  int tpo = 64;
  while (tpo > 1 && (256 / tpo < nout || tpo > L4)) tpo >>= 1;
  const int opp = 256 / tpo;
  for (int base = 0; base < nout; base += opp) {
    const int o = base + tid / tpo, p = tid % tpo;
    float a0 = 0.f, a1 = 0.f;
    if (o < nout) {
      const int gi = o / hid, hj = o - gi * hid;
      const float4* wr = (const float4*)(w1s + hj * r1);
      const float4* pg = (const float4*)(pvec + gi * L);
      int i = p;
      for (; i + tpo < L4; i += 2 * tpo) {
        const float4 wa = wr[i], xa = pg[i], wb = wr[i + tpo], xb = pg[i + tpo];
        a0 = fmaf(wa.w, xa.w, fmaf(wa.z, xa.z, fmaf(wa.y, xa.y, fmaf(wa.x, xa.x, a0))));
        a1 = fmaf(wb.w, xb.w, fmaf(wb.z, xb.z, fmaf(wb.y, xb.y, fmaf(wb.x, xb.x, a1))));
      }
      if (i < L4) { const float4 wa = wr[i], xa = pg[i]; a0 = fmaf(wa.w, xa.w, fmaf(wa.z, xa.z, fmaf(wa.y, xa.y, fmaf(wa.x, xa.x, a0)))); }
    }
    float s = a0 + a1;
    for (int m = tpo >> 1; m >= 1; m >>= 1) s += __shfl_xor(s, m, 64);
    if (o < nout && p == 0) hbuf[o] = fmaxf(s + b1s[o % hid], 0.f);
  }
  __syncthreads();
  SPR_STAMP();
  for (int o = tid; o < C; o += 256) {
    const int gi = o / cw, ci = o - gi * cw;
    float s = b2s[ci];
#pragma unroll 4
    for (int hj = 0; hj < hid; ++hj) s = fmaf(w2s[ci * r2 + hj], hbuf[gi * hid + hj], s);
    obuf[o] = 1.f / (1.f + expf(-s));
  }
  __syncthreads();
  SPR_STAMP();
  for (int ci = tid; ci < cw; ci += 256) {
    float mx = -INFINITY;
    for (int gi = 0; gi < G; ++gi) mx = fmaxf(mx, obuf[gi * cw + ci]);
    float den = 0.f;
    for (int gi = 0; gi < G; ++gi) { const float e = expf(obuf[gi * cw + ci] - mx); att[gi * cw + ci] = e; den += e; }
    for (int gi = 0; gi < G; ++gi) att[gi * cw + ci] /= den;
  }
  __syncthreads();
}

template <typename T, int V>
__global__ __launch_bounds__(256) void spr_attn_scale_kernel(const float* __restrict__ partial, const float* __restrict__ w1, const float* __restrict__ b1,
                                                             const float* __restrict__ w2, const float* __restrict__ b2, int C, int G, int H, int W,
                                                             const T* __restrict__ x, long xsn, long xsh, long xsw, T* __restrict__ y, long ysn, long ysh,
                                                             long ysw, FastDiv fd_q, FastDiv fd_w, int nsplit, int tiles_x, int tiles_y, SprPool pa, SprPool pb, FastDiv fd_gst,
                                                             FastDiv fd_tx, FastDiv fd_l4, int fast, unsigned long long* dbg) {
  extern __shared__ float sm[];
  unsigned long long TS[10]; int nt = 0;
  auto stamp = [&]() __attribute__((always_inline)) { if (dbg) TS[nt++] = __builtin_amdgcn_s_memrealtime(); };
  stamp();
  const int n = blockIdx.y, cw = C / G, hid = cw / 4;
  float* pooled = sm;
  float* hbuf = sm + C * 5;
  float* obuf = hbuf + G * hid;
  float* att = obuf + C;
  const int hs1 = bin_start(1, H, 2), he0 = bin_end(0, H, 2), ws1 = bin_start(1, W, 2), we0 = bin_end(0, W, 2);
  const float cnt[5] = {(float)H * W, (float)he0 * we0, (float)he0 * (W - ws1), (float)(H - hs1) * we0, (float)(H - hs1) * (W - ws1)};
  __shared__ float red[5 * 256];
  if (fast) {
    spr_prologue_fast(partial, w1, b1, w2, b2, C, G, n, nsplit, tiles_x, tiles_y, fd_gst, fd_tx, fd_l4, cnt, sm, red, att, dbg ? TS : nullptr, nt);
  } else {
    if (tiles_x > 0) {
      const int gst = nsplit / (tiles_x * tiles_y);
      for (int c0 = 0; c0 < C; c0 += 256) {
        const int lanes_c = min(C - c0, 256);
        const int ph = 256 / lanes_c;
        const int c = c0 + threadIdx.x % lanes_c, sp0 = threadIdx.x / lanes_c;
        float acc[5] = {0.f, 0.f, 0.f, 0.f, 0.f};
        if (sp0 < ph) {
          for (int sp = sp0; sp < nsplit; sp += ph) {
            const float v = partial[((long)n * nsplit + sp) * C + c];
            const int tile = sp / gst, ty = tile / tiles_x, tx = tile - ty * tiles_x;
            const int bin = (2 * ty >= tiles_y ? 2 : 0) + (2 * tx >= tiles_x ? 1 : 0);
            acc[0] += v;
            acc[1] += bin == 0 ? v : 0.f;
            acc[2] += bin == 1 ? v : 0.f;
            acc[3] += bin == 2 ? v : 0.f;
            acc[4] += bin == 3 ? v : 0.f;
          }
        }
#pragma unroll
        for (int k = 0; k < 5; ++k) red[k * 256 + threadIdx.x] = acc[k];
        __syncthreads();
        for (int o = threadIdx.x; o < lanes_c * 5; o += 256) {
          const int cc = o % lanes_c, k = o / lanes_c;
          float sum = 0.f;
          for (int p = 0; p < ph; ++p) sum += red[k * 256 + p * lanes_c + cc];
          pooled[(c0 + cc) * 5 + k] = sum / cnt[k];
        }
        __syncthreads();
      }
    } else {
      for (int i = threadIdx.x; i < C * 5; i += 256) {
        float sum = 0.f;
        for (int sp = 0; sp < nsplit; ++sp) sum += partial[((long)n * nsplit + sp) * C * 5 + i];
        pooled[i] = sum / cnt[i % 5];
      }
      __syncthreads();
    }
    for (int o = threadIdx.x; o < G * hid; o += 256) {
      int gi = o / hid, hj = o % hid;
      const float* wr = w1 + (long)hj * 5 * cw;
      float acc = b1[hj];
      for (int c = 0; c < cw; ++c) acc = fmaf(wr[c], pooled[(gi * cw + c) * 5 + 0], acc);
      for (int c = 0; c < cw; ++c)
        for (int bn = 0; bn < 4; ++bn) acc = fmaf(wr[cw + c * 4 + bn], pooled[(gi * cw + c) * 5 + 1 + bn], acc);
      hbuf[o] = fmaxf(acc, 0.f);
    }
    __syncthreads();
    for (int o = threadIdx.x; o < C; o += 256) {
      int gi = o / cw, c = o % cw;
      float acc = b2[c];
      for (int hj = 0; hj < hid; ++hj) acc = fmaf(w2[(long)c * hid + hj], hbuf[gi * hid + hj], acc);
      obuf[o] = 1.f / (1.f + expf(-acc));
    }
    __syncthreads();
    for (int c = threadIdx.x; c < cw; c += 256) {
      float mx = -INFINITY;
      for (int gi = 0; gi < G; ++gi) mx = fmaxf(mx, obuf[gi * cw + c]);
      float den = 0.f;
      for (int gi = 0; gi < G; ++gi) den += expf(obuf[gi * cw + c] - mx);
      for (int gi = 0; gi < G; ++gi) att[gi * cw + c] = expf(obuf[gi * cw + c] - mx) / den;
    }
    __syncthreads();
  }
  stamp();
  auto fin = [&]() __attribute__((always_inline)) { if (dbg) { __builtin_amdgcn_s_waitcnt(0); stamp(); if (threadIdx.x == 0) for (int k = 0; k < 8; ++k) dbg[((size_t)blockIdx.y * gridDim.x + blockIdx.x) * 8 + k] = TS[k]; } };
  {
    const int fa = pa.F, fb = pb.F, fm = max(fa, fb);
    const bool cells = fm > 0 && (fm == 2 || fm == 4) && (fa == 0 || fa == fm || (fm == 4 && fa == 2)) && (fb == 0 || fb == fm || (fm == 4 && fb == 2)) && !(fa == fb);
    if (cells) {
      const SprPool none = {nullptr, 0, 0, 0, 0};
      const SprPool big = fa == fm ? pa : (fb == fm ? pb : none), small = (fa && fa < fm) ? pa : ((fb && fb < fm) ? pb : none);
      if (fm == 4) spr_scale_cells<T, V, 4>(x, xsn, xsh, xsw, y, ysn, ysh, ysw, att, n, H, W, C, big, small);
      else spr_scale_cells<T, V, 2>(x, xsn, xsh, xsw, y, ysn, ysh, ysw, att, n, H, W, C, big, small);
      fin();
      return;
    }
  }
  const int Q = C / V, HW = H * W;
  const int p0 = (int)((long)blockIdx.x * HW / gridDim.x), p1 = (int)((long)(blockIdx.x + 1) * HW / gridDim.x);
  const uint32_t total = (uint32_t)(p1 - p0) * Q;
  auto one = [&](uint32_t i, long& xo, long& yo, int& qv) __attribute__((always_inline)) {
    const int pl = (int)fdiv(i, fd_q), q = (int)i - pl * Q;
    const int p = p0 + pl, h = (int)fdiv((uint32_t)p, fd_w), w = p - h * W;
    xo = n * xsn + h * xsh + w * xsw + q * V; yo = n * ysn + h * ysh + w * ysw + q * V; qv = q * V;
  };
  uint32_t i = threadIdx.x;
  for (; i + 3 * 256 < total; i += 4 * 256) {
    float v[4][V];
    long yo[4];
    int qv[4];
#pragma unroll
    for (int u = 0; u < 4; ++u) { long xo; one(i + u * 256, xo, yo[u], qv[u]); ldv<T, V>(x + xo, v[u]); }
#pragma unroll
    for (int u = 0; u < 4; ++u) {
#pragma unroll
      for (int k = 0; k < V; ++k) v[u][k] *= att[qv[u] + k];
      stv<T, V>(y + yo[u], v[u]);
    }
  }
  for (; i < total; i += 256) {
    long xo, yo; int qv; float v[V];
    one(i, xo, yo, qv);
    ldv<T, V>(x + xo, v);
#pragma unroll
    for (int k = 0; k < V; ++k) v[k] *= att[qv + k];
    stv<T, V>(y + yo, v);
  }
  const SprPool pools[2] = {pa, pb};
#pragma unroll
  for (int pi = 0; pi < 2; ++pi) {
    const SprPool P = pools[pi];
    if (P.F == 0) continue;
    const int F = P.F, Ho = H / F, Wo = W / F, HWo = Ho * Wo;
    const int q0 = (int)((long)blockIdx.x * HWo / gridDim.x), q1 = (int)((long)(blockIdx.x + 1) * HWo / gridDim.x);
    const float inv = 1.f / (float)(F * F);
    for (int j = threadIdx.x; j < (q1 - q0) * Q; j += 256) {
      const int pl = j / Q, q = j - pl * Q, po = q0 + pl, oy = po / Wo, ox = po - oy * Wo;
      float a[V], acc[V];
#pragma unroll
      for (int k = 0; k < V; ++k) { a[k] = att[q * V + k]; acc[k] = 0.f; }
      for (int yy = 0; yy < F; ++yy)
        for (int xx = 0; xx < F; ++xx) {
          float v[V];
          ldv<T, V>(x + n * xsn + (long)(oy * F + yy) * xsh + (long)(ox * F + xx) * xsw + q * V, v);
#pragma unroll
          for (int k = 0; k < V; ++k) acc[k] += (float)(T)(v[k] * a[k]);
        }
#pragma unroll
      for (int k = 0; k < V; ++k) acc[k] *= inv;
      stv<T, V>((T*)P.y + n * P.sn + oy * P.sh + ox * P.sw + q * V, acc);
    }
  }
  fin();
}

extern "C" int mgdt_spr_attn_scale_fwd(const float* pooled, int nsplit, int tiles_x, int tiles_y, const float* fc1_w, const float* fc1_b, const float* fc2_w, const float* fc2_b, int groups,
                                       const mgdt_view* x, const mgdt_view* y, const mgdt_view* pool_a, const mgdt_view* pool_b, int dtype, mgdt_stream s) {
  if (nsplit <= 0) nsplit = SPR_SPLITS;
  if (tiles_x > 0 && (tiles_y <= 0 || nsplit % (tiles_x * tiles_y) || tiles_x % 2 || tiles_y % 2 || x->h % 2 || x->w % 2))
    MGDT_FAIL(MGDT_BAD_SHAPE, "spr_attn_scale: per-tile sums need an even tile grid over an even map (nsplit=%d tiles %dx%d)", nsplit, tiles_y, tiles_x);
  if (!pooled || !fc1_w || !fc1_b || !fc2_w || !fc2_b || !view_ok(x) || !view_ok(y)) MGDT_FAIL(MGDT_BAD_ARG, "spr_attn_scale: null/empty argument");
  const int c = x->c;
  if (groups < 1 || c % groups || (c / groups) % 4 || c > 4096) MGDT_FAIL(MGDT_BAD_SHAPE, "spr_attn_scale: c=%d groups=%d", c, groups);
  if (!vec4_ok(x, dtype) || !vec4_ok(y, dtype) || x->n != y->n || x->h != y->h || x->w != y->w || y->c != c)
    MGDT_FAIL(MGDT_BAD_SHAPE, "spr_attn_scale: views must be matching NHWC, c%%4==0");
  const int cw = c / groups, hid = cw / 4;
  size_t lds = (size_t)(c * 5 + groups * hid + 2 * c) * sizeof(float);
  const size_t wbytes = ((size_t)hid * (5 * cw + 4) + (size_t)cw * (hid + 1) + hid + cw + 4) * sizeof(float);
  const int fast = tiles_x > 0 && c <= 256 && lds + wbytes <= 48 * 1024 && ((uintptr_t)fc1_w & 15) == 0;
  if (fast) lds += wbytes;
  SprPool pl[2] = {{nullptr, 0, 0, 0, 0}, {nullptr, 0, 0, 0, 0}};
  bool pool8 = true;
  const mgdt_view* pv[2] = {pool_a, pool_b};
  for (int i = 0; i < 2; ++i) {
    const mgdt_view* p = pv[i];
    if (!p || !p->p) continue;
    if (!view_ok(p) || !vec4_ok(p, dtype) || p->n != x->n || p->c != c || p->h < 1 || x->h % p->h || x->w % p->w || x->h / p->h != x->w / p->w)
      MGDT_FAIL(MGDT_BAD_SHAPE, "spr_attn_scale: a pooled output must be an NHWC view of the same n, c whose size divides the map by one factor");
    pl[i].y = p->p; pl[i].sn = p->sn; pl[i].sh = p->sh; pl[i].sw = p->sw; pl[i].F = x->h / p->h;
    pool8 = pool8 && vecN_ok(p, dtype, 8);
  }
  static unsigned long long* dbgbuf = nullptr;
  if (getenv("MGDT_SPR_DBG") && !dbgbuf) (void)hipMalloc((void**)&dbgbuf, 4096 * 8 * 8);
  int gK = 0;
  MGDT_DISPATCH_TV(dtype, vecN_ok(x, dtype, 8) && vecN_ok(y, dtype, 8) && pool8, {
    const long vecs = (long)x->h * x->w * (c / V);
    static const long per_wg = getenv("MGDT_SPR_VECS") ? atol(getenv("MGDT_SPR_VECS")) : 2048;
    static const long kmax = getenv("MGDT_SPR_KMAX") ? atol(getenv("MGDT_SPR_KMAX")) : 12;
    const int K = (int)std::max<long>(1, std::min<long>(kmax, vecs / per_wg));
    spr_attn_scale_kernel<T, V><<<dim3(K, x->n), 256, lds, (hipStream_t)s>>>(pooled, fc1_w, fc1_b, fc2_w, fc2_b, c, groups, x->h, x->w, (const T*)x->p, x->sn,
                                                                              x->sh, x->sw, (T*)y->p, y->sn, y->sh, y->sw, make_fastdiv((uint32_t)(c / V)),
                                                                              make_fastdiv((uint32_t)x->w), nsplit, tiles_x, tiles_y, pl[0], pl[1],
                                                                              make_fastdiv((uint32_t)(tiles_x > 0 ? nsplit / (tiles_x * tiles_y) : 1)),
                                                                              make_fastdiv((uint32_t)std::max(tiles_x, 1)), make_fastdiv((uint32_t)(5 * cw / 4)), fast, dbgbuf);
    gK = K;
  });
  MGDT_CHECK_LAUNCH("spr_attn_scale_fwd");
  if (dbgbuf && gK * x->n <= 4096) {
    (void)hipStreamSynchronize((hipStream_t)s);
    std::vector<unsigned long long> h((size_t)gK * x->n * 8);
    (void)hipMemcpy(h.data(), dbgbuf, h.size() * 8, hipMemcpyDeviceToHost);
    unsigned long long t0 = ~0ull, t1 = 0; double ph[7] = {0, 0, 0, 0, 0, 0, 0};
    const int ns = fast ? 8 : 3;
    for (int i = 0; i < gK * x->n; ++i) { t0 = std::min(t0, h[i * 8]); t1 = std::max(t1, h[i * 8 + ns - 1]); for (int k = 0; k + 1 < ns; ++k) ph[k] += (double)(h[i * 8 + k + 1] - h[i * 8 + k]); }
    fprintf(stderr, "spr_attn_scale c %d %dx%d: %d wgs, span %.1f us; mean per wg (us):", c, x->h, x->w, gK * x->n, (t1 - t0) * 0.01);
    for (int k = 0; k + 1 < ns; ++k) fprintf(stderr, " %.2f", ph[k] * 0.01 / (gK * x->n));
    fprintf(stderr, fast ? "  (issue | loads land | sums | fc1 | fc2 | softmax | scale)\n" : "  (prologue | scale)\n");
  }
  return MGDT_OK;
}

template <typename T, int V>
__global__ void scale_channels_kernel(const T* __restrict__ x, long xsn, long xsh, long xsw, const float* __restrict__ attn,
                                      T* __restrict__ y, long ysn, long ysh, long ysw, uint32_t total, int C, PixIdx d) {
  for (uint32_t i = blockIdx.x * blockDim.x + threadIdx.x; i < total; i += gridDim.x * blockDim.x) {
    int n, h, w, q;
    decode_idx(i, d, n, h, w, q);
    float v[V], a[V];
    ldv<T, V>(x + n * xsn + h * xsh + w * xsw + q * V, v);
    ldv<float, V>(attn + (long)n * C + q * V, a);
#pragma unroll
    for (int k = 0; k < V; ++k) v[k] *= a[k];
    stv<T, V>(y + n * ysn + h * ysh + w * ysw + q * V, v);
  }
}

extern "C" int mgdt_scale_channels_fwd(const mgdt_view* x, const float* attn, const mgdt_view* y, int dtype, mgdt_stream s) {
  if (!view_ok(x) || !view_ok(y) || !attn) MGDT_FAIL(MGDT_BAD_ARG, "scale_channels: null/empty argument");
  if (!vec4_ok(x, dtype) || !vec4_ok(y, dtype) || x->n != y->n || x->h != y->h || x->w != y->w || x->c != y->c)
    MGDT_FAIL(MGDT_BAD_SHAPE, "scale_channels: views must be matching NHWC, c%%4==0");
  long tot = (long)x->n * x->h * x->w * x->c;
  if (tot >= 0x7fffffffL) MGDT_FAIL(MGDT_BAD_SHAPE, "scale_channels: too large");
  MGDT_DISPATCH_TV(dtype, vecN_ok(x, dtype, 8) && vecN_ok(y, dtype, 8), {
    PixIdx d = make_pixidx(x->h, x->w, x->c / V);
    uint32_t total = (uint32_t)(tot / V);
    scale_channels_kernel<T, V><<<grid_for(total), 256, 0, (hipStream_t)s>>>((const T*)x->p, x->sn, x->sh, x->sw, attn, (T*)y->p, y->sn, y->sh, y->sw, total, x->c, d);
  });
  MGDT_CHECK_LAUNCH("scale_channels_fwd");
  return MGDT_OK;
}

__device__ __forceinline__ float pool_max(float a, float b) { return __builtin_elementwise_maximum(a, b); }

template <typename T, int SPPF_CG>
__global__ __launch_bounds__(256) void sppf_pool_kernel(const T* __restrict__ x, long xsn, long xsh, long xsw, T* __restrict__ y1, long s1n,
                                                        long s1h, long s1w, T* __restrict__ y2, long s2n, long s2h, long s2w,
                                                        T* __restrict__ y3, long s3n, long s3h, long s3w, int H, int W) {
  extern __shared__ float sm[];
  const int n = blockIdx.x, c0 = blockIdx.y * SPPF_CG, HW = H * W, WP = W + 4, PP = (H + 4) * WP;
  float* A = sm;
  float* Bf = sm + PP * SPPF_CG;
  constexpr int QN = SPPF_CG / 4;
  const f32x4 ninf = {-INFINITY, -INFINITY, -INFINITY, -INFINITY};
  for (int i = threadIdx.x; i < PP * QN; i += 256) {
    const int pp = i / QN, qq = (i % QN) * 4;
    const int hh = pp / WP - 2, ww = pp % WP - 2;
    const bool in = (unsigned)hh < (unsigned)H && (unsigned)ww < (unsigned)W;
    *(f32x4*)(A + pp * SPPF_CG + qq) = in ? load4<T>(x + n * xsn + hh * xsh + ww * xsw + c0 + qq) : ninf;
    *(f32x4*)(Bf + pp * SPPF_CG + qq) = ninf;
  }
  __syncthreads();
// ... 765 lines not shown
```

mgdt_yolo_amd/nn/modules/block.py:

```python
import torch
import torch.nn as nn

from ... import ops
from .conv import Conv, HipModule, act_code
from .convnextv2 import ConvNeXtV2_Block
from .spr_module import SPRModule

__all__ = ('DFL', 'SPPF', 'C2f', 'C3', 'MSPA_C2f', 'Bottleneck', 'SimFusion_4in', 'SimFusion_3in', 'IFM', 'h_sigmoid',
           'InjectionMultiSum_Auto_pool', 'Upsample', 'Proto')


def _plain_block(first, last, bottlenecks):
    def conv_ok(c, k):
        return (isinstance(c, Conv) and c.plain_affine() and c.conv.kernel_size == (k, k) and c.conv.stride == (1, 1) and c.conv.groups == 1
                and act_code(c.act) == a0)
    try:
        a0 = act_code(first.act)
    except RuntimeError:
        return False
    if a0 != ops.ACT_SILU:
        return False
    if not (conv_ok(first, 1) and conv_ok(last, 1)) or len(bottlenecks) == 0:
        return False
    return all(isinstance(m, Bottleneck) and conv_ok(m.cv1, 3) and conv_ok(m.cv2, 3) and m.add == bottlenecks[0].add
# ... 126 lines not shown
        dt0 = self.cv1.out_dtype(x)
        if (not train and dt0 == torch.bfloat16 and x.dtype == dt0 and ops.c3_fused_route(c, n) and self._plain()
                and ops.conv_can_mfma(x, x.shape[1], 2 * c, 1, 1, 1, dt0)):
            ab = ops.new_act(b, 2 * c, h, w, dt0, x.device)
            if ops.csp_block_supported(ops.CSP_C3, ab, self.cv3.conv.out_channels, c, n, dt0):
                ops.conv2d(x, self._merged_front(dt0), 1, ops.ACT_SILU, out=ab)
                mids = [pk for m in self.m for pk in (m.cv1.packed(dt0, False), m.cv2.packed(dt0, False))]
                return ops.csp_block(ops.CSP_C3, ab, None, None, mids, self.m[0].add, self.cv3.packed(dt0, False), c, ops.ACT_SILU,
                                     self.cv3.conv.out_channels, False)[0]
        f = (lambda m: m.train_fwd) if train else (lambda m: m.run)
        cat = ops.new_act(b, 2 * c, h, w, self.cv1.out_dtype(x), x.device)
        f(self.cv2)(x, out=cat[:, c:])
        t = f(self.cv1)(x, out=cat[:, :c] if n == 0 else None)
        for j, m in enumerate(self.m):
            t = m.run(t, out=cat[:, :c] if j == n - 1 else None)
        return f(self.cv3)(cat)

    def backward(self, g):
        c = self.c
        gcat = self.cv3.backward(g)
        ga = gcat[:, :c]
        for m in reversed(list(self.m)):
            ga = m.backward(ga)
        dx = self.cv1.backward(ga)
        return self.cv2.backward(gcat[:, c:], dx_out=dx, acc=True)


class MSPA_C2f(HipModule):

    def __init__(self, inplanes, outplanes, n=1, shortcut=False, g=1, e=0.5, scale=4, stride=1, stype='normal'):
        super().__init__()
        self.nums = scale
        self.inwidth = inplanes // self.nums
        self.outwidth = outplanes // self.nums
        self.stride = stride
        assert stype in ['stage', 'normal'], 'One of these is suppported (stage or normal)'
        self.stype = stype
        self.convs = nn.ModuleList([])
        self.btnk_nums = n
        for i in range(self.nums):
            if self.stride == 1 and i != self.nums - 1:
                self.convs.append(Conv(self.inwidth, self.inwidth, 1, 1))
            else:
                self.convs.append(Conv(inplanes + self.outwidth * (n - 1), outplanes, 1, 1))
        self.bottleneck = nn.ModuleList(Bottleneck(self.inwidth, self.inwidth, shortcut, g, k=((3, 3), (3, 3)), e=1.0) for _ in range(n))
        self.attention = SPRModule(self.outwidth)
        self.softmax = nn.Softmax(dim=1)

    def forward(self, x, deliver=None):
        if self.stride != 1:
            raise RuntimeError('MSPA_C2f: only stride=1 is wired by parse_model and built here')
        d_out = deliver.get('out') if deliver else None
        d_pools = deliver.get('pools', ()) if deliver else ()
        b, _, h, w = x.shape
        wd, s, n = self.inwidth, self.nums, self.btnk_nums
        train = self.training and hasattr(self.convs[0], 'bn')
        run = (lambda m: m.train_fwd) if train else (lambda m: m.run)
        dt = self.convs[0].out_dtype(x)
        at = self.attention
        if (not train and s == 4 and self.inwidth == self.outwidth and self._chain_ok() and _plain_block(self.convs[0], self.convs[3], self.bottleneck)
                and ops.csp_block_supported(ops.CSP_MSPA, x, self.convs[3].conv.out_channels, wd, n, dt)):
            mids = [pk for m in self.bottleneck for pk in (m.cv1.packed(dt, False), m.cv2.packed(dt, False))]
            out, pool, slots, tiles = ops.csp_block(ops.CSP_MSPA, x, self._packed_chain(dt).blob, None, mids, self.bottleneck[0].add,
                                                    self.convs[3].packed(dt, False), wd, act_code(self.convs[0].act), self.convs[3].conv.out_channels, True)
            return ops.spr_attention_scale(out, at.fc1.weight, at.fc1.bias, at.fc2.weight, at.fc2.bias, s, out=d_out, part=pool, nsplit=slots, tiles=tiles, pools=d_pools)
        cat = ops.new_act(b, (s - 1 + n) * wd, h, w, dt, x.device)
        if not train and s == 4 and ops.pw_chain_supported(wd, cat.dtype) and x.dtype == cat.dtype and self._chain_ok():
            ops.pw_chain3(x[:, :3 * wd], self._packed_chain(cat.dtype), act_code(self.convs[0].act), cat[:, :3 * wd])
        else:
            run(self.convs[0])(x[:, :wd], out=cat[:, :wd])
            for i in range(1, s - 1):
                run(self.convs[i])(cat[:, (i - 1) * wd:i * wd], x2=x[:, i * wd:(i + 1) * wd], out=cat[:, i * wd:(i + 1) * wd])
        src, pending = cat[:, (s - 2) * wd:(s - 1) * wd], x[:, (s - 1) * wd:s * wd]
        for j, m in enumerate(self.bottleneck):
            dst = cat[:, (s - 1 + j) * wd:(s + j) * wd]
            m.run(src, out=dst, x2=pending)
            src, pending = dst, None
        out = run(self.convs[s - 1])(cat)
        if train:
            attn, part = ops.spr_attention_train(out, at.fc1.weight, at.fc1.bias, at.fc2.weight, at.fc2.bias, s)
            self._save_ctx((out, attn, part, x.shape))
        else:
            return ops.spr_attention_scale(out, at.fc1.weight, at.fc1.bias, at.fc2.weight, at.fc2.bias, s, out=d_out, pools=d_pools)
        return ops.scale_channels(out, attn)

    def _chain_ok(self):
        cs = list(self.convs)[:3]
        return all(c.plain_affine() and c.conv.kernel_size == (1, 1) and c.conv.groups == 1 and c.conv.in_channels == self.inwidth
                   and c.conv.out_channels == self.inwidth and act_code(c.act) == act_code(cs[0].act) for c in cs)

    def _packed_chain(self, dtype):
        cs = list(self.convs)[:3]
        tens = [t for c in cs for t in c.affine_tensors()]
        return self._cached(('chain', dtype), tens, lambda: ops.PackedPwChain([(c.conv.weight, c.conv.bias, c.bn_tuple()) for c in cs], dtype))

    def backward(self, g):
        out, attn, part, xshape = self._ctx.pop()
        wd, s, n = self.inwidth, self.nums, self.btnk_nums
        at = self.attention
        dattn = ops.nc_reduce(g, out)
        prms = (at.fc1.weight, at.fc1.bias, at.fc2.weight, at.fc2.bias)
        gb = [ops.grad_buf(p) for p in prms]
        chained = all(t.is_contiguous() and t.dtype == torch.float32 for t in gb) and all(
            a.untyped_storage().data_ptr() == b.untyped_storage().data_ptr() and a.storage_offset() + a.numel() == b.storage_offset() for a, b in zip(gb, gb[1:]))
        pg_out = gb[0].new_empty(0).set_(gb[0].untyped_storage(), gb[0].storage_offset(), (sum(t.numel() for t in gb),)) if chained else None
        gout, pg = ops.spr_bwd(g, part, attn, dattn, at.fc1.weight, at.fc1.bias, at.fc2.weight, at.fc2.bias, s, out=pg_out)
        if not chained:
            o = 0
            for prm, t in zip(prms, gb):
                t.copy_(pg[o:o + t.numel()].view_as(prm))
                o += t.numel()
        gcat = self.convs[s - 1].backward(gout)
        gx = ops.new_act(xshape[0], xshape[1], xshape[2], xshape[3], g.dtype, g.device)
        sl = lambda t, i: t[:, i * wd:(i + 1) * wd]
        for j in reversed(range(n)):
            if j > 0:
                self.bottleneck[j].backward(sl(gcat, s - 1 + j), acc_into=sl(gcat, s - 2 + j))
                continue
            gin = self.bottleneck[j].backward(sl(gcat, s - 1 + j))
            dst = sl(gcat, s - 2 + j)
            ops.add(dst, gin, out=dst)
            ops.copy(gin, sl(gx, s - 1))
        for i in reversed(range(1, s - 1)):
            gi = self.convs[i].backward(sl(gcat, i), dx_out=sl(gx, i))
            dst = sl(gcat, i - 1)
            ops.add(dst, gi, out=dst)
        self.convs[0].backward(sl(gcat, 0), dx_out=sl(gx, 0))
        return gx


class SPPF(HipModule):

    def __init__(self, c1, c2, k=5):
        super().__init__()
        if k != 5:
            raise RuntimeError('SPPF: k=5 is what the YAMLs use and what the fused pooling kernel implements')
        c_ = c1 // 2
        self.cv1 = Conv(c1, c_, 1, 1)
        self.cv2 = Conv(c_ * 4, c2, 1, 1)
        self.m = nn.MaxPool2d(kernel_size=k, stride=1, padding=k // 2)

    def forward(self, x):
        b, _, h, w = x.shape
        c_ = self.cv1.conv.out_channels
        train = self.training and hasattr(self.cv1, 'bn')
        cat = ops.new_act(b, 4 * c_, h, w, self.cv1.out_dtype(x), x.device)
        (self.cv1.train_fwd if train else self.cv1.run)(x, out=cat[:, :c_])
        ops.sppf_pools(cat[:, :c_], cat[:, c_:2 * c_], cat[:, 2 * c_:3 * c_], cat[:, 3 * c_:])
        if train:
            self._cat = cat if ops.ctx_enabled() else None
        return (self.cv2.train_fwd if train else self.cv2.run)(cat)

    def backward(self, g):
        c_ = self.cv1.conv.out_channels
        cat, self._cat = self._cat, None
        gcat = self.cv2.backward(g)
        sl = lambda t, i: t[:, i * c_:(i + 1) * c_]
        g2 = ops.add(sl(gcat, 2), ops.maxpool5_bwd(sl(cat, 2), sl(gcat, 3)))
        g1 = ops.add(sl(gcat, 1), ops.maxpool5_bwd(sl(cat, 1), g2))
        g0 = ops.add(sl(gcat, 0), ops.maxpool5_bwd(sl(cat, 0), g1))
        return self.cv1.backward(g0)


class Proto(HipModule):

    def __init__(self, c1, c_=256, c2=32):
        super().__init__()
        self.cv1 = Conv(c1, c_, k=3)
        self.upsample = nn.ConvTranspose2d(c_, c_, 2, 2, 0, bias=True)
        self.cv2 = Conv(c_, c_, k=3)
        self.cv3 = Conv(c_, c2)

    def run_upsample(self, x):
        up = self.upsample
        ops.check_deconv2x2(up.kernel_size, up.stride, up.padding, up.groups, up.output_padding, up.dilation)
        if up.bias is None:
            raise RuntimeError('Proto.upsample is built with its bias (block.py:63)')
        dt = self.out_dtype(x)
        pk = self._cached(('deconv', dt), [up.weight, up.bias], lambda: ops.PackedDeconv2x2(up.weight, up.bias, dt))
        return ops.deconv2x2(x, pk)

    def forward(self, x):
        if self.training:
            raise NotImplementedError('segmentation training is not built (the reference\'s v8SegmentationLoss cannot run in this fork): Proto runs in eval()')
        return self.cv3(self.cv2(self.run_upsample(self.cv1(x))))


class Upsample(nn.Module):

    def __init__(self, size=None, scale_factor=None, mode='nearest'):
        super().__init__()
        if mode != 'nearest' or size is not None:
            raise RuntimeError("Upsample: only (None, scale_factor, 'nearest') is on the detection path")
        self.scale_factor, self.mode, self.size = scale_factor, mode, size

    def forward(self, x):
        b, c, h, w = x.shape
        out = ops.new_act(b, c, int(h * self.scale_factor), int(w * self.scale_factor), x.dtype, x.device)
        return ops.nearest(x, out)

# ... 41 lines not shown
        super().__init__()
        self.cv1 = Conv(in_channel_list[0], out_channels, act=nn.ReLU()) if in_channel_list[0] != out_channels else nn.Identity()
        self.cv2 = Conv(in_channel_list[1], out_channels, act=nn.ReLU()) if in_channel_list[1] != out_channels else nn.Identity()
        self.cv3 = Conv(in_channel_list[2], out_channels, act=nn.ReLU()) if in_channel_list[2] != out_channels else nn.Identity()
        self.cv_fuse = Conv(out_channels * 3, out_channels, act=nn.ReLU())

    def forward(self, x, pre=None):
        b, _, h, w = x[1].shape
        oc = self.cv_fuse.conv.out_channels
        dt, dev = x[1].dtype, x[1].device
        self._shapes = [t.shape for t in x]
        cat, done, pooled0 = None, (), None
        if pre is not None and pre.get('out') is not None and tuple(pre['out'].shape) == (b, 3 * oc, h, w) and pre['out'].dtype == dt:
            cat, done, pooled0 = pre['out'], pre['done'], pre.get('pooled0')
        if cat is None:
            cat = ops.new_act(b, 3 * oc, h, w, dt, dev)
        if isinstance(self.cv1, nn.Identity):
            if 0 not in done:
                ops.adaptive_avgpool(x[0], cat[:, :oc])
        else:
            if pooled0 is None or tuple(pooled0.shape) != (b, x[0].shape[1], h, w):
                pooled0 = ops.adaptive_avgpool(x[0], ops.new_act(b, x[0].shape[1], h, w, dt, dev))
            (self.cv1.train_fwd if (self.training and hasattr(self.cv1, 'bn')) else self.cv1.run)(pooled0, out=cat[:, :oc])
        if isinstance(self.cv2, nn.Identity):
            if not (1 in done and x[1].data_ptr() == cat[:, oc:2 * oc].data_ptr()):
                ops.copy(x[1], cat[:, oc:2 * oc])
        else:
            (self.cv2.train_fwd if (self.training and hasattr(self.cv2, 'bn')) else self.cv2.run)(x[1], out=cat[:, oc:2 * oc])
        if isinstance(self.cv3, nn.Identity):
            ops.bilinear(x[2], cat[:, 2 * oc:])
        else:
            (self.cv3.train_fwd if (self.training and hasattr(self.cv3, 'bn')) else self.cv3.run)(
                ops.bilinear(x[2], ops.new_act(b, x[2].shape[1], h, w, dt, dev)), out=cat[:, 2 * oc:])
        return self.cv_fuse(cat)

    def backward(self, g):
        oc = self.cv_fuse.conv.out_channels
        sh = self._shapes
        mk = lambda i: ops.new_act(sh[i][0], sh[i][1], sh[i][2], sh[i][3], g.dtype, g.device)
        gcat = self.cv_fuse.backward(g)
        g0 = gcat[:, :oc] if isinstance(self.cv1, nn.Identity) else self.cv1.backward(gcat[:, :oc])
        g1 = gcat[:, oc:2 * oc] if isinstance(self.cv2, nn.Identity) else self.cv2.backward(gcat[:, oc:2 * oc])
        g2 = gcat[:, 2 * oc:] if isinstance(self.cv3, nn.Identity) else self.cv3.backward(gcat[:, 2 * oc:])
        return [ops.adaptive_avgpool_bwd(g0, mk(0)), g1, ops.bilinear_bwd(g2, mk(2))]


class IFM(nn.Module):

    def __init__(self, inc, ouc, embed_dim_p=96, fuse_block_num=3) -> None:
        super().__init__()
        self.conv = nn.Sequential(Conv(inc, embed_dim_p), *[ConvNeXtV2_Block(embed_dim_p) for _ in range(fuse_block_num)],
                                  Conv(embed_dim_p, sum(ouc)))

    def forward(self, x):
        mods = list(self.conv)
        if (not self.training and len(mods) >= 2 and isinstance(mods[-2], ConvNeXtV2_Block) and not mods[-2]._forward_hooks and not self.conv._forward_hooks):
            for m in mods[:-2]:
                x = m(x)
            r = mods[-2](x, tail=mods[-1])
            return r[0] if isinstance(r, tuple) else mods[-1](r)
        return self.conv(x)

    def backward(self, g):
        for m in reversed(list(self.conv)):
            g = m.backward(g)
        return g


class h_sigmoid(nn.Module):

    def __init__(self, inplace=True):
        super().__init__()
        self.relu = nn.ReLU6(inplace=inplace)


class InjectionMultiSum_Auto_pool(HipModule):

    def __init__(self, inp: int, oup: int, global_inp: list, flag: int) -> None:
        super().__init__()
        self.global_inp = global_inp
        self.flag = flag
        self.local_embedding = Conv(inp, oup, 1, act=False)
        self.global_embedding = Conv(global_inp[self.flag], oup, 1, act=False)
        self.global_act = Conv(global_inp[self.flag], oup, 1, act=False)
        self.act = h_sigmoid()

    def _merged_global(self, g, xq=None):
        a, b = self.global_act, self.global_embedding
        ok = all(m.plain_affine() and act_code(m.act) == ops.ACT_NONE and m.conv.kernel_size == (1, 1) and m.conv.groups == 1 for m in (a, b))
        dt = a.out_dtype(g)
        fused = not hasattr(a, 'bn')
        if (not ok or fused != (not hasattr(b, 'bn')) or (not fused and a.bn.eps != b.bn.eps) or a.conv.out_channels % 8
                or not ops.conv_can_mfma(g, a.conv.in_channels, a.conv.out_channels + b.conv.out_channels, 1, 1, 1, dt)):
            return None
        tens = [t for m in (a, b) for t in m.affine_tensors()]
        cat = lambda fn: torch.cat([fn(a).detach().float(), fn(b).detach().float()])
        zb = lambda m: m.conv.bias if m.conv.bias is not None else torch.zeros(m.conv.out_channels, device=m.conv.weight.device)
        bn = lambda: None if fused else (cat(lambda m: m.bn.weight), cat(lambda m: m.bn.bias), cat(lambda m: m.bn.running_mean), cat(lambda m: m.bn.running_var), a.bn.eps)
        cb = lambda: cat(zb) if fused else None
        if xq is not None:
            return self._cached(('gaf', 'fp8', float(xq)), tens, lambda: ops.PackedConvFp8(cat(lambda m: m.conv.weight), cb(), bn(), 1, xq))
        return self._cached(('gaf', dt), tens, lambda: ops.PackedConv(cat(lambda m: m.conv.weight), cb(), bn(), 1, dt))

    def forward_into_conv(self, x, conv):
        x_l, x_g = x
        le = self.local_embedding
        if self.training or not isinstance(conv, Conv) or not conv.plain_affine() or not le.plain_affine():
            return None
        if ops.Q8_CALIB is not None or self.__dict__.get('_q8') or conv.__dict__.get('_q8') or le.__dict__.get('_q8'):
            return None
        dt = le.out_dtype(x_l)
        c0 = sum(self.global_inp[:self.flag])
        g = x_g[:, c0:c0 + self.global_inp[self.flag]]
        pk2g = self._merged_global(g)
# ... 72 lines not shown
```

mgdt_yolo_amd/nn/modules/conv.py:

```python
import math

import torch
import torch.nn as nn

from ... import ops

__all__ = ('Conv', 'DWConv', 'Concat', 'autopad')


def autopad(k, p=None, d=1):
    if d > 1:
        k = d * (k - 1) + 1 if isinstance(k, int) else [d * (x - 1) + 1 for x in k]
    if p is None:
        p = k // 2 if isinstance(k, int) else [x // 2 for x in k]
    return p


def act_code(m):
    if isinstance(m, nn.SiLU):
        return ops.ACT_SILU
    if isinstance(m, nn.ReLU):
        return ops.ACT_RELU
    if isinstance(m, nn.Identity):
        return ops.ACT_NONE
# ... 91 lines not shown
        if x.dim() != 4 or x.shape[1] != self.conv.in_channels or x.shape[2] % 2 or x.shape[3] % 2:
            raise RuntimeError(f'Conv: the 6x6 / stride 2 / padding 2 stem takes a (B, {self.conv.in_channels}, H, W) image with even H and W '
                               f'(model inputs are multiples of the stride), got {tuple(x.shape)}')
        return ops.space_to_depth2(x, dt)

    def _stem6_packed(self, dt, direct, raw=False):
        tens = [self.conv.weight] if raw else self.affine_tensors()
        cb, bn = (None, None) if raw else (self.conv.bias, self.bn_tuple())
        if not direct:
            return self._cached(('stem6', raw, dt), tens, lambda: ops.PackedStem6(self.conv.weight, cb, bn, dt))
        cp = ops.space_to_depth2_channels(self.conv.in_channels, dt)
        return self._cached(('stem6', raw, dt, 'direct'), tens, lambda: ops.PackedConv(ops.stem6_w3(self.conv.weight, cp), cb, bn, 3, dt, direct=True))

    def packed(self, dtype, direct):
        has_bn = hasattr(self, 'bn')
        tens = [self.conv.weight, self.conv.bias] + ([self.bn.weight, self.bn.bias, self.bn.running_mean, self.bn.running_var] if has_bn else [])
        k, _ = self._geometry()
        if k == 6:
            return self._stem6_packed(dtype, direct)

        def build():
            bn = (self.bn.weight, self.bn.bias, self.bn.running_mean, self.bn.running_var, self.bn.eps) if has_bn else None
            return ops.PackedConv(self.conv.weight, self.conv.bias, bn, k, dtype, direct=direct, groups=self.conv.groups)
        return self._cached((dtype, direct), tens, build)

    def packed_fp8(self, xq):
        has_bn = hasattr(self, 'bn')
        tens = [self.conv.weight, self.conv.bias] + ([self.bn.weight, self.bn.bias, self.bn.running_mean, self.bn.running_var] if has_bn else [])
        k, _ = self._geometry()

        def build():
            bn = (self.bn.weight, self.bn.bias, self.bn.running_mean, self.bn.running_var, self.bn.eps) if has_bn else None
            return ops.PackedConvFp8(self.conv.weight, self.conv.bias, bn, k, xq)
        return self._cached(('fp8', float(xq)), tens, build)

    def run(self, x, out=None, x2=None, r1=None, r2=None, in_scale=None, in_shift=None):
        if hasattr(self, 'bn'):
            self._no_train_bn(self.bn)
        k, s = self._geometry()
        dt = self.out_dtype(x) if out is None else out.dtype
        if k == 6:
            if x2 is not None or in_scale is not None or in_shift is not None:
                raise RuntimeError('Conv: the 6x6 stem reads the image (no fused pre-add or input affine)')
            sd = self._stem6_input(x, dt)
            mfma = ops.conv_can_mfma(sd, sd.shape[1], self.conv.out_channels, 3, 1, 1, dt)
            return ops.conv2d(sd, self._stem6_packed(dt, not mfma), 1, act_code(self.act), out=out, r1=r1, r2=r2)
        mfma = ops.conv_can_mfma(x, self.conv.in_channels, self.conv.out_channels, k, s, self.conv.groups, dt)
        if mfma and dt == torch.bfloat16:
            xq = self.q8_site(None, x, x2)
            if xq is not None:
                return ops.conv2d_fp8(x, self.packed_fp8(xq), s, act_code(self.act), out=out, x2=x2, r1=r1, r2=r2, in_scale=in_scale, in_shift=in_shift)
        pk = self.packed(dt, direct=not mfma)
        return ops.conv2d(x, pk, s, act_code(self.act), out=out, x2=x2, r1=r1, r2=r2, in_scale=in_scale, in_shift=in_shift)

    def forward(self, x):
        if self.training and hasattr(self, 'bn'):
            return self.train_fwd(x)
        return self.run(x)

    def train_fwd(self, x, out=None, x2=None, r1=None, r2=None):
        k, s = self._geometry()
        dt = self.out_dtype(x) if out is None else out.dtype
        if k == 6:
            if x2 is not None:
                raise RuntimeError('Conv.train_fwd: the 6x6 stem reads the image (no fused pre-add)')
            x = self._stem6_input(x, dt)
            mfma = ops.conv_can_mfma(x, x.shape[1], self.conv.out_channels, 3, 1, 1, dt)
            y = ops.conv2d(x, self._stem6_packed(dt, not mfma, raw=True), 1, ops.ACT_NONE)
        else:
            mfma = ops.conv_can_mfma(x, self.conv.in_channels, self.conv.out_channels, k, s, self.conv.groups, dt)
            pk = self._cached(('raw', dt, not mfma), [self.conv.weight],
                              lambda: ops.PackedConv(self.conv.weight, None, None, k, dt, direct=not mfma, groups=self.conv.groups))
            if x2 is not None and not mfma:
                raise RuntimeError('Conv.train_fwd: the fused pre-add needs the MFMA path (NHWC input, cin % 4 == 0)')
            y = ops.conv2d(x, pk, s, ops.ACT_NONE, x2=x2)
        bn = self.bn
        mean, rstd = ops.bn_stats(y, bn.eps, bn.momentum, bn.running_mean, bn.running_var)
        z = ops.bn_act(y, mean, rstd, bn.weight, bn.bias, act_code(self.act), out=out, r1=r1, r2=r2)
        self._save_ctx((x, x2, y, mean, rstd, k, s))
        return z

    def backward(self, gz, need_dx=True, dx_out=None, acc=False, r2=None):
        x, x2, y, mean, rstd, k, s = self._ctx.pop()
        if k == 6:
            return self._backward_stem6(gz, x, y, mean, rstd, need_dx)
        if self.conv.groups != 1:
            return self._backward_grouped(gz, x, y, mean, rstd, k, s, need_dx, dx_out, acc, r2)
        bn = self.bn
        ops.grad_buf(bn.weight)
        ops.grad_buf(bn.bias)
        dy = ops.bn_act_bwd(gz, y, mean, rstd, bn.weight, bn.bias, act_code(self.act), bn.weight.grad, bn.bias.grad)
        ops.grad_buf(self.conv.weight)
        ops.conv_wgrad(x, dy, k, s, self.conv.weight.grad, x2=x2)
        if not need_dx:
            return None
        dx = dx_out if dx_out is not None else ops.new_act(x.shape[0], x.shape[1], x.shape[2], x.shape[3], dy.dtype, dy.device)
        return ops.conv_dgrad(dy, self.conv.weight, k, s, dx, accumulate=bool(acc and dx_out is not None), r2=r2)

    def _backward_stem6(self, gz, sd, y, mean, rstd, need_dx):
        if need_dx:
            raise RuntimeError('Conv.backward: the 6x6 stem has no data gradient (it reads the image: call backward(g, need_dx=False))')
        bn = self.bn
        dy = ops.bn_act_bwd(gz, y, mean, rstd, bn.weight, bn.bias, act_code(self.act), ops.grad_buf(bn.weight), ops.grad_buf(bn.bias))
        dw3 = torch.empty((self.conv.out_channels, sd.shape[1], 3, 3), dtype=torch.float32, device=sd.device)
        ops.conv_wgrad(sd, dy, 3, 1, dw3)
        ops.stem6_wgrad_unpack(dw3, ops.grad_buf(self.conv.weight))
# ... 47 lines not shown
```

mgdt_yolo_amd/nn/tasks.py:

```python
import ast
import contextlib
import math
import re
from copy import deepcopy
from pathlib import Path

import torch
import torch.nn as nn

from .. import ops
from ..yolo.utils.torch_utils import fuse_conv_and_bn, initialize_weights, intersect_dicts, make_divisible
from .modules import (C2f, C3, IFM, MSPA_C2f, SPPF, Bottleneck, Classify, Concat, Conv, Detect, DWConv, InjectionMultiSum_Auto_pool,
                      Pose, RTDETRDecoder, Segment, SimFusion_3in, SimFusion_4in, TOODHead, Upsample)

REGISTRY = {c.__name__: c for c in (Conv, DWConv, Concat, Bottleneck, C2f, C3, MSPA_C2f, SPPF, SimFusion_4in, SimFusion_3in, IFM,
                                    InjectionMultiSum_Auto_pool, Detect, TOODHead, Segment, Pose, Classify, RTDETRDecoder)}
REGISTRY['nn.Upsample'] = Upsample


class _TrainForwardFn(torch.autograd.Function):

    @staticmethod
    def forward(ctx, model, x, anchor):
        with ops.force_ctx():
# ... 5 lines not shown
        ctx.n = len(feats)
        return tuple(feats)

    @staticmethod
    def backward(ctx, *gfeats):
        model = ctx.model
        if ctx.single:
            gfeats = gfeats[0].contiguous()
        else:
            gfeats = [g if g.is_contiguous(memory_format=torch.channels_last) else g.contiguous(memory_format=torch.channels_last) for g in gfeats]
        acc = model._accumulate_snapshot() if getattr(model, 'grad_accumulate', False) else None
        model.backward(gfeats)
        if acc is not None:
            model._accumulate_restore(acc)
        return None, None, None


class BaseModel(nn.Module):

    def forward(self, x, *args, **kwargs):
        if isinstance(x, dict):
            return self.loss(x, *args, **kwargs)
        return self.predict(x, *args, **kwargs)

    def predict(self, x, profile=False, visualize=False, augment=False):
        if profile or visualize:
            raise RuntimeError('profile / visualize are host-side tooling outside the hot path')
        if augment:
            if self.training or not hasattr(self, '_predict_augment'):
                raise RuntimeError('augment=True is an inference call form: put the detection model in eval() (augmented training is not built)')
            return self._predict_augment(x)
        if self.training and torch.is_grad_enabled() and any(p.requires_grad for p in self.model[0].parameters()):
            if not hasattr(self, '_anchor'):
                self._anchor = torch.zeros((), device=x.device, requires_grad=True)
            out = _TrainForwardFn.apply(self, x, self._anchor)
            return out if torch.is_tensor(out) else list(out)
        return self._predict_once(x)

    def _predict_once(self, x, profile=False, visualize=False):
        if not x.is_cuda:
            raise RuntimeError('mgdt_yolo_amd runs on MI355X (HIP) only: move the model and the input to cuda (no CPU fallback)')
        if self.training:
            for m in self.modules():
                m.__dict__.pop('_ctx', None)
        y = []
        layers = self.model
        if not self.training and self._stem_fusable(x):
            m0, m1 = self.model[0], self.model[1]
            pk0 = m0._cached(('stem2',), m0.affine_tensors(), lambda: ops.PackedStem2(m0.conv.weight, m0.folded_bn_like()))
            x = ops.stem2(x, pk0, m1.packed(torch.bfloat16, direct=False))
            y = [None, x if 1 in self.save else None]
            layers = list(self.model)[2:]
        plan = self._neck_plan(x) if not self.training else None
        bufs = {}
        head = None
        side = self._side_branch() if not self.training else None
        first = layers[0].i
        y += [None] * (len(self.model) - len(y))
        prev = {first - 1: x}

        def run(m):
            nonlocal head
            src = lambda j: prev[m.i - 1] if j == -1 else y[m.i + j if j < 0 else j]
            xin = src(m.f) if isinstance(m.f, int) else [src(j) for j in m.f]
            if head is not None:
                out, head = m(None, head=head), None
            elif self._injection_feeds_next(m):
                head, out = (m, xin), None
            elif plan is not None and m.i in plan['producers']:
                out = m(xin, deliver=self._neck_deliveries(plan, m, xin, bufs))
            elif plan is not None and m.i in plan['consumers']:
                out = m(xin, pre=bufs.get(m.i))
            else:
                out = m(xin)
            prev.pop(m.i - 1, None)
            prev[m.i] = out
            y[m.i] = out if m.i in self.save else None

        if side is None or side[2] < first:
            for m in layers:
                run(m)
            return prev[len(self.model) - 1]
        s0, s1, dep = side
        main, other = torch.cuda.current_stream(), ops.side_stream(x.device)
        for m in layers:
            if s0 <= m.i <= s1:
                continue
            if m.i == s1 + 1:
                main.wait_stream(other)
            run(m)
            if m.i == dep:
                other.wait_stream(main)
                with torch.cuda.stream(other):
                    for k in range(s0, s1 + 1):
                        run(self.model[k])
        if s1 + 1 >= len(self.model):
            main.wait_stream(other)
        return prev[len(self.model) - 1]

    def _side_branch(self):
        if not ops.SIDE_STREAM:
            return None
        if '_side_branch_cache' not in self.__dict__:
            absf = lambda m: [m.i + f if f < 0 else f for f in ([m.f] if isinstance(m.f, int) else m.f)]
            best = None
            n = len(self.model)
            for s0 in range(2, n - 1):
                deps, s1 = set(), s0 - 1
                for k in range(s0, n - 1):
                    ext = {j for j in absf(self.model[k]) if j < s0}
                    if ext and max(ext) >= s0 - 1:
                        break
                    deps |= ext
                    s1 = k
                if s1 < s0 or not deps:
                    continue
                dep = max(deps)
                if best is None or (s0 - 1 - dep, s1 - s0) > (best[0] - 1 - best[2], best[1] - best[0]):
                    best = (s0, s1, dep)
            self.__dict__['_side_branch_cache'] = best
        best = self.__dict__['_side_branch_cache']
        if best is None or any(self.model[k]._forward_hooks for k in range(best[2] + 1, best[1] + 1)):
            return None
        return best

    def _injection_feeds_next(self, m):
        if (self.training or not ops.FUSED_INJECT_CONV or getattr(self, 'compute_dtype', None) != torch.bfloat16 or not isinstance(m, InjectionMultiSum_Auto_pool)
                or m.i in self.save or m.i + 1 >= len(self.model)):
            return False
        nxt = self.model[m.i + 1]
        return isinstance(nxt, C2f) and nxt.f == -1 and not m._forward_hooks and not nxt._forward_hooks and len(nxt.m) >= 1

    def _neck_plan(self, x):
        if not ops.FUSED_NECK or getattr(self, 'compute_dtype', None) != torch.bfloat16 or not hasattr(self, '_reductions'):
            return None
        plan = self.__dict__.get('_neck_plan_cache')
        if plan is None:
            prod, cons = {}, set()
            absf = lambda m: [m.i + f if f < 0 else f for f in ([m.f] if isinstance(m.f, int) else m.f)]
            for m in self.model:
                if isinstance(m, SimFusion_4in):
                    src = absf(m)
                    kinds = ('pool', 'pool', 'main')
                elif isinstance(m, SimFusion_3in):
                    src = absf(m)
                    kinds = ('pool', 'main' if isinstance(m.cv2, nn.Identity) else None)
                else:
                    continue
                for slot, kind in enumerate(kinds):
                    j = src[slot]
                    if kind is None or not isinstance(self.model[j], MSPA_C2f):
                        continue
                    if kind == 'main' and any(k == 'main' for k, _, _ in prod.get(j, [])):
                        continue
                    prod.setdefault(j, []).append((kind, m.i, slot))
                    cons.add(m.i)
            plan = self.__dict__['_neck_plan_cache'] = {'producers': prod, 'consumers': cons} if prod else False
        if not plan:
            return None
        if any(self.model[i]._forward_hooks for i in list(plan['producers']) + list(plan['consumers'])):
            return None
        return plan

    def _neck_deliveries(self, plan, m, x, bufs):
        b, c, h, w = x.shape
        out, pools = None, []
        red = self._reductions
        absf = lambda mm: [mm.i + f if f < 0 else f for f in ([mm.f] if isinstance(mm.f, int) else mm.f)]
        for kind, ci, slot in plan['producers'][m.i]:
            cm = self.model[ci]
            src = absf(cm)
            tgt = src[2] if isinstance(cm, SimFusion_4in) else src[1]
            if red[tgt] % red[m.i]:
                continue
            F = int(red[tgt] // red[m.i])
            if F < 1 or h % F or w % F or (kind == 'main' and F != 1) or (kind == 'pool' and F == 1):
                continue
            th, tw = h // F, w // F
            if isinstance(cm, SimFusion_4in):
                cs = [self.model[j].c2 for j in src]
                total, off = sum(cs), sum(cs[:slot])
            else:
                oc = cm.cv_fuse.conv.out_channels
                total, off = 3 * oc, slot * oc
            st = bufs.setdefault(ci, {'out': None, 'done': set()})
            if st['out'] is None:
                st['out'] = ops.new_act(b, total, th, tw, x.dtype, x.device)
            if tuple(st['out'].shape) != (b, total, th, tw):
                continue
            if isinstance(cm, SimFusion_3in) and slot == 0 and not isinstance(cm.cv1, nn.Identity):
                st['pooled0'] = ops.new_act(b, c, th, tw, x.dtype, x.device)
                pools.append(st['pooled0'])
                continue
            view = st['out'][:, off:off + c]
            if kind == 'pool':
                pools.append(view)
            else:
                out = view
            st['done'].add(slot)
        return {'out': out, 'pools': pools[:2]} if (out is not None or pools) else None

    def _stem_fusable(self, x):
        if not ops.FUSED_STEM or getattr(self, 'compute_dtype', None) != torch.bfloat16 or len(self.model) < 3 or 0 in self.save:
            return False
        if x.dtype not in (torch.bfloat16, torch.float32, torch.uint8) or x.dim() != 4 or x.shape[1] != 3:
            return False
        m0, m1 = self.model[0], self.model[1]
        for m, (ci, co) in ((m0, (3, 16)), (m1, (16, 32))):
            if not (isinstance(m, Conv) and not isinstance(m, DWConv) and m.plain_affine() and isinstance(m.act, nn.SiLU) and m.f == -1 and not m._forward_hooks
                    and m.conv.kernel_size == (3, 3) and m.conv.stride == (2, 2) and m.conv.padding == (1, 1) and m.conv.groups == 1
                    and m.conv.in_channels == ci and m.conv.out_channels == co):
                return False
        return True

    def backward(self, head_grads, layer_done=None):
# ... 640 lines not shown
```

mgdt_yolo_amd/ops.py:

```python
import ctypes as C
import os

import numpy as np
import torch

from . import _lib as L
from ._lib import ACT_GELU, ACT_NONE, ACT_RELU, ACT_SILU, BF16, F32, View

U8 = 2
_DT = {torch.float32: F32, torch.bfloat16: BF16}


def dtype_code(dt):
    try:
        return _DT[dt]
    except KeyError:
        raise RuntimeError(f'mgdt_yolo_amd computes in float32 or bfloat16, not {dt}') from None


def _need_gpu(t):
    if not t.is_cuda:
        raise RuntimeError('mgdt_yolo_amd runs on MI355X (HIP) only: got a CPU tensor and there is no CPU/PyTorch fallback')


# ... 200 lines not shown
    arr = (L.PackDesc * len(live))()
    for d, o in zip(arr, live):
        w, cb, g, b, mu, var, eps, cin, cout, k, code, mode = o.src
        d.w, d.conv_bias, d.bn_gamma, d.bn_beta, d.bn_mean, d.bn_var = ptr(w), ptr(cb), ptr(g), ptr(b), ptr(mu), ptr(var)
        d.bn_eps, d.cin, d.cout, d.k, d.dtype, d.mode = eps, cin, cout, k, code, mode
        d.packed, d.bias_out = ptr(o.w), ptr(o.bias)
    _launch('conv_pack_batch', 'mgdt_conv_pack_batch', arr, len(live), stream())
    for o in live:
        o.epoch = PARAM_EPOCH[0]
    return live


def pack_is_current(obj):
    return getattr(obj, 'epoch', None) == PARAM_EPOCH[0]


def conv_can_mfma(x, cin, cout, k, s, groups, dtype):
    pe = 8 if dtype == torch.bfloat16 else 4
    return (groups == 1 and k in (1, 3) and s in (1, 2) and cin % pe == 0 and cout % 4 == 0 and x.dtype == dtype
            and is_nhwc(x) and x.stride(3) % pe == 0 and x.stride(2) % pe == 0 and x.stride(0) % pe == 0
            and x.data_ptr() % 16 == 0)


def conv_out_hw(h, w, k, s):
    p = k // 2
    return (h + 2 * p - k) // s + 1, (w + 2 * p - k) // s + 1


def conv2d(x, pk, stride, act, out=None, x2=None, r1=None, r2=None, in_scale=None, in_shift=None):
    _need_gpu(x)
    b, _, h, w = x.shape
    ho, wo = conv_out_hw(h, w, pk.k, stride)
    if out is None:
        out = new_act(b, pk.cout, ho, wo, pk.dtype, x.device)
    if _PROF is not None:
        es = out.element_size()
        _META['conv2d_direct_fwd' if pk.direct else 'conv2d_fwd'] = dict(
            shape=(b, pk.cin, h, w, pk.cout, pk.k, stride), flops=2.0 * b * ho * wo * pk.cout * pk.cin // pk.groups * pk.k * pk.k,
            bytes=float(b * h * w * pk.cin * x.element_size() + b * ho * wo * pk.cout * es + pk.w.numel() * pk.w.element_size()))
    if pk.direct:
        if x2 is not None or r1 is not None or r2 is not None or in_scale is not None or in_shift is not None:
            raise RuntimeError('direct convolution path has no fused extras')
        _launch('conv2d_direct_fwd', 'mgdt_conv2d_direct_fwd', vp(x), U8 if x.dtype == torch.uint8 else dtype_code(x.dtype), ptr(pk.w), ptr(pk.bias), pk.k, stride, pk.groups, act,
                                           vp(out), dtype_code(out.dtype), stream())
    else:
        _same(x, x2, r1, r2, out)
        if x.dtype != pk.dtype:
            raise RuntimeError(f'conv2d: the weights are packed for {pk.dtype}, the input is {x.dtype}')
        _launch('conv2d_fwd', 'mgdt_conv2d_fwd', vp(x), vp(x2), ptr(in_scale), ptr(in_shift), ptr(pk.w), ptr(pk.bias), pk.k, stride, act,
                                    vp(r1), vp(r2), vp(out), dtype_code(pk.dtype), stream())
    return out


def conv2d_route(x, y, k, stride, dtype=None, act=ACT_SILU, x2=False, in_scale=False, in_shift=False, r1=False, r2=False, fp8=False):
    def shape_view(t):
        b, c, h, w = t.shape
        sn, sc, sh, sw = t.stride()
        return View(None, b, h, w, c, sn, sh, sw, sc)
    flags = sum(f for on, f in ((x2, L.ROUTE_X2), (in_scale, L.ROUTE_IN_SCALE), (in_shift, L.ROUTE_IN_SHIFT), (r1, L.ROUTE_R1), (r2, L.ROUTE_R2),
                                (fp8, L.ROUTE_FP8)) if on)
    r = L.ConvRoute()
    L.check(L.lib().mgdt_conv2d_route(C.byref(shape_view(x)), C.byref(shape_view(y)), k, stride, dtype_code(dtype or x.dtype), flags, act, C.byref(r)),
            'conv2d_route')
    keys = (('NT', 'MT', 'D', 'extra', 'nseg', 'seg_chunks', 'gx', 'gy', 'numTiles', 'ragged') if r.family == L.ROUTE_IGEMM
            else ('NBW', 'tile_rows', 'ncg', 'nwg', 'ntiles'))
    out = {'family': 'igemm' if r.family == L.ROUTE_IGEMM else 'lds3x3'}
    out.update((n, getattr(r, n)) for n in keys + ('waves', 'nchunks', 'lds_bytes'))
    return out


def _route_view(t):
    b, c, h, w = t.shape
    sn, sc, sh, sw = t.stride()
    p = 4096 + t.storage_offset() * t.element_size() if t.device.type == 'meta' else t.data_ptr()
    return View(p, b, h, w, c, sn, sh, sw, sc)


def _image_code(dt):
    return dt if isinstance(dt, int) else (U8 if dt == torch.uint8 else dtype_code(dt))


def conv2d_direct_route(x, y, k, stride, groups=1, x_dtype=None, dtype=None):
    out = (C.c_int * 4)()
    L.check(L.lib().mgdt_conv2d_direct_route(C.byref(_route_view(x)), _image_code(x.dtype if x_dtype is None else x_dtype), C.byref(_route_view(y)),
                                             _image_code(y.dtype if dtype is None else dtype), int(k), int(stride), int(groups), out), 'conv2d_direct_route')
    return dict(family=('stem', 'generic', 'refused')[out[0]], gx=out[1], gy=out[2], status=out[3])


def spr_attention(x, fc1_w, fc1_b, fc2_w, fc2_b, groups, softmax=True):
    b, c, h, w = x.shape
    lib = L.lib()
    part = torch.empty(b * L.SPR_SPLITS * c * 5, dtype=torch.float32, device=x.device)
    _launch('spr_pool_fwd', 'mgdt_spr_pool_fwd', vp(x), ptr(part), dtype_code(x.dtype), stream())
    attn = torch.empty(b, c, dtype=torch.float32, device=x.device)
    _launch('spr_attn_fwd', 'mgdt_spr_attn_fwd', ptr(part), ptr(fc1_w), ptr(fc1_b), ptr(fc2_w), ptr(fc2_b), b, c, groups, h, w, int(bool(softmax)),
            ptr(attn), stream())
    return attn


def spr_attention_scale(x, fc1_w, fc1_b, fc2_w, fc2_b, groups, out=None, part=None, nsplit=0, tiles=(0, 0), pools=()):
    b, c, h, w = x.shape
    if part is None:
        part = torch.empty(b * L.SPR_SPLITS * c * 5, dtype=torch.float32, device=x.device)
        _launch('spr_pool_fwd', 'mgdt_spr_pool_fwd', vp(x), ptr(part), dtype_code(x.dtype), stream())
        nsplit, tiles = L.SPR_SPLITS, (0, 0)
    out = like(x) if out is None else out
    pools = list(pools)
    if len(pools) > 2:
        raise RuntimeError('spr_attention_scale: at most two pooled outputs')
    _same(x, out, *pools)
    pa, pb = (pools + [None, None])[:2]
    _launch('spr_attn_scale_fwd', 'mgdt_spr_attn_scale_fwd', ptr(part), int(nsplit), int(tiles[0]), int(tiles[1]), ptr(fc1_w), ptr(fc1_b), ptr(fc2_w), ptr(fc2_b), groups, vp(x), vp(out),
            vp(pa), vp(pb), dtype_code(x.dtype), stream())
    return out


FUSED_NECK = True


FUSED_STEM = True


class PackedStem2:

    def __init__(self, weight, bn):
        g, b, mu, var, eps = bn
        scale = (g.detach().float() / torch.sqrt(eps + var.detach().float()))
        wf = (weight.detach().float() * scale.view(-1, 1, 1, 1)).contiguous()
        self.bias = (b.detach().float() - g.detach().float() * mu.detach().float() / torch.sqrt(var.detach().float() + eps)).contiguous()
        self.blob = torch.empty(L.lib().mgdt_stem2_packed_bytes(), dtype=torch.uint8, device=weight.device)
        L.check(L.lib().mgdt_stem2_pack(ptr(wf), ptr(self.blob), stream()), 'stem2_pack')


def stem2(x, pk0, pk1):
    _need_gpu(x)
    b, _, h, w = x.shape
    h0, w0 = (h - 1) // 2 + 1, (w - 1) // 2 + 1
    h1, w1 = (h0 - 1) // 2 + 1, (w0 - 1) // 2 + 1
    y = new_act(b, 32, h1, w1, torch.bfloat16, x.device)
    if _PROF is not None:
        _META['stem2_fwd'] = dict(shape=(b, 3, h, w, 32, 3, 4), flops=2.0 * b * (h0 * w0 * 16 * 27 + h1 * w1 * 32 * 144),
                                  bytes=float(x.numel() * x.element_size() + y.numel() * 2))
    _launch('stem2_fwd', 'mgdt_stem2_fwd', vp(x), U8 if x.dtype == torch.uint8 else dtype_code(x.dtype), ptr(pk0.blob), ptr(pk0.bias), ptr(pk1.w), ptr(pk1.bias),
            vp(y), stream())
    return y


def stem2_route(x, y, cu_count=0, x_dtype=None):
    out = (C.c_int * 7)()
    L.check(L.lib().mgdt_stem2_route(C.byref(_route_view(x)), _image_code(x.dtype if x_dtype is None else x_dtype), C.byref(_route_view(y)), int(cu_count), out),
            'stem2_route')
    if out[6]:
        return dict(loader='refused', status=out[6])
    return dict(loader='fast' if out[0] else 'generic', tiles_x=out[1], tiles_y=out[2], tiles=out[3], grid=out[4], per_xcd=out[5])


def space_to_depth2_channels(c, dtype):
    v = 8 if dtype == torch.bfloat16 else 4
    return (4 * c + v - 1) // v * v


def space_to_depth2(x, dtype, out=None):
    b, c, h, w = x.shape
    if c > 4 or h % 2 or w % 2:
        raise RuntimeError(f'space_to_depth2: an image of at most 4 channels with even height and width, got {tuple(x.shape)}')
    _need_gpu(x)
    if x.dtype != torch.uint8 and dtype_code(x.dtype) == BF16 and dtype != torch.bfloat16:
# ... 18 lines not shown
            raise RuntimeError(f'PackedStem6: a (cout, <= 4, 6, 6) weight, got {tuple(weight.shape)}')
        g, b, mu, var, eps = (None, None, None, None, 0.0) if bn is None else bn
        f = lambda t: None if t is None else t.detach().float().contiguous()
        g, b, mu, var, cb = f(g), f(b), f(mu), f(var), f(conv_bias)
        code = dtype_code(dtype)
        cp = space_to_depth2_channels(c6, dtype)
        self.k, self.cin, self.cout, self.dtype, self.direct, self.groups = 3, cp, cout, dtype, False, 1
        self.w = torch.empty(lib.mgdt_conv_packed_bytes(cp, cout, 3, code), dtype=torch.uint8, device=weight.device)
        self.bias = torch.empty((cout + 15) // 16 * 16, dtype=torch.float32, device=weight.device)
        _launch('conv_pack', 'mgdt_conv_pack_stem6', ptr(weight), ptr(cb), ptr(g), ptr(b), ptr(mu), ptr(var), eps, c6, cout, code, ptr(self.w), ptr(self.bias), stream())
        _register_pack(self, (weight, cb, g, b, mu, var, float(eps), c6, cout, 3, code, 5 + c6))


def stem6_w3(w6, cp=None):
    co, c = w6.shape[0], w6.shape[1]
    w3 = w6.detach().reshape(co, c, 3, 2, 3, 2).permute(0, 3, 5, 1, 2, 4).reshape(co, 4 * c, 3, 3)
    if cp is not None and cp > 4 * c:
        w3 = torch.cat([w3, w3.new_zeros(co, cp - 4 * c, 3, 3)], 1)
    return w3.contiguous()


def stem6_w6(w3, c):
    co = w3.shape[0]
    return w3[:, :4 * c].reshape(co, 2, 2, c, 3, 3).permute(0, 3, 4, 1, 5, 2).reshape(co, c, 6, 6).contiguous()


def stem6_wgrad_unpack(dw3, dw6):
    flush_wgrad()
    if not (dw3.is_contiguous() and dw6.is_contiguous() and dw3.dtype == dw6.dtype == torch.float32 and dw3.shape[0] == dw6.shape[0]
            and tuple(dw3.shape[2:]) == (3, 3) and tuple(dw6.shape[2:]) == (6, 6) and dw3.shape[1] >= 4 * dw6.shape[1]):
        raise RuntimeError(f'stem6_wgrad_unpack: contiguous fp32 (cout, cp, 3, 3) -> (cout, c, 6, 6), got {tuple(dw3.shape)} -> {tuple(dw6.shape)}')
    _launch('stem6_wgrad_unpack', 'mgdt_stem6_wgrad_unpack', ptr(dw3), dw6.shape[0], dw6.shape[1], dw3.shape[1], ptr(dw6), stream())
    return dw6


FUSED_CSP_BLOCK = True
CSP_MSPA, CSP_C2F, CSP_C3 = 0, 1, 2
C3_FUSED_CLASSES = ((16, 1), (32, 1), (32, 2), (64, 1))


def c3_fused_route(wd, nbtl):
    return FUSED_CSP_BLOCK and (C3_FUSED_CLASSES is None or (int(wd), int(nbtl)) in C3_FUSED_CLASSES)


def csp_block_supported(mode, x, cout, wd, nbtl, dtype):
    if not (FUSED_CSP_BLOCK and dtype == torch.bfloat16 and x.dtype == dtype and is_nhwc(x)):
        return False
    lib = L.lib()
    if not lib.mgdt_csp_block_supported(mode, x.shape[1], int(cout), int(wd), int(nbtl), x.shape[2], x.shape[3], dtype_code(dtype)):
        return False
    return lib.mgdt_csp_block_tiles(mode, x.shape[0], x.shape[1], int(cout), int(wd), int(nbtl), x.shape[2], x.shape[3], None) > 0


def csp_block(mode, x, front, front_bias, mids, shortcut, back, wd, act, cout, want_pool):
    lib = L.lib()
    b, cin, h, w = x.shape
    nb = len(mids) // 2
    geom = (C.c_int * 8)()
    slots = lib.mgdt_csp_block_tiles(mode, b, cin, cout, wd, nb, h, w, geom)
    if slots <= 0:
        raise RuntimeError('csp_block: configuration not covered')
    y = new_act(b, cout, h, w, x.dtype, x.device)
    pool = torch.empty(b * slots * cout, dtype=torch.float32, device=x.device) if want_pool else None
    marr = (C.c_void_p * len(mids))(*[m.w.data_ptr() for m in mids])
    barr = (C.c_void_p * len(mids))(*[m.bias.data_ptr() for m in mids])
    if _PROF is not None:
        es = x.element_size()
        catc = 2 * wd if mode == CSP_C3 else (3 if mode == CSP_MSPA else 2) * wd + nb * wd
        fl = 2.0 * b * h * w * ((3 * wd * wd if mode == CSP_MSPA else 0) + (10 if mode == CSP_C3 else 18) * nb * wd * wd + catc * cout)
        _META['csp_block_fwd'] = dict(shape=(b, cin, h, w, cout, wd, nb), flops=fl, bytes=float(b * h * w * (cin + cout) * es))
    _launch('csp_block_fwd', 'mgdt_csp_block_fwd', mode, vp(x), ptr(front), ptr(front_bias), marr, barr, nb, int(bool(shortcut)), ptr(back.w), ptr(back.bias),
            int(wd), act, vp(y), ptr(pool), dtype_code(x.dtype), stream())
    return y, pool, slots, (geom[6], geom[7])


def scale_channels(x, attn, out=None):
    out = like(x) if out is None else out
    _same(x, out)
    _launch('scale_channels_fwd', 'mgdt_scale_channels_fwd', vp(x), ptr(attn), vp(out), dtype_code(x.dtype), stream())
    return out


def sppf_pools(x, y1, y2, y3):
    _launch('sppf_pool_fwd', 'mgdt_sppf_pool_fwd', vp(x), vp(y1), vp(y2), vp(y3), dtype_code(x.dtype), stream())


def adaptive_avgpool(x, out):
    _same(x, out)
    _launch('adaptive_avgpool_fwd', 'mgdt_adaptive_avgpool_fwd', vp(x), vp(out), dtype_code(x.dtype), stream())
    return out


def bilinear(x, out):
    _same(x, out)
    _launch('bilinear_fwd', 'mgdt_bilinear_fwd', vp(x), vp(out), dtype_code(x.dtype), stream())
    return out


def nearest(x, out):
    _same(x, out)
    _launch('nearest_fwd', 'mgdt_nearest_fwd', vp(x), vp(out), dtype_code(x.dtype), stream())
    return out


def copy(x, out):
    _launch('copy_fwd', 'mgdt_copy_fwd', vp(x), U8 if x.dtype == torch.uint8 else dtype_code(x.dtype), vp(out), dtype_code(out.dtype), stream())
    return out


def dwconv7_ln(x, dw_w49c, dw_b, ln_w, ln_b, eps, out=None):
    out = like(x) if out is None else out
    _launch('dwconv7_ln_fwd', 'mgdt_dwconv7_ln_fwd', vp(x), ptr(dw_w49c), ptr(dw_b), ptr(ln_w), ptr(ln_b), eps, vp(out), dtype_code(x.dtype),
                                        stream())
    return out

# ... 1642 lines not shown
```

Measured before the change: 40780 images/sec.

## Defer SPR channel attention into the downstream stride-2 conv with fused pooled side outputs

Adds a stride-2 LDS 3x3 conv variant that multiplies the staged input tile by per-image channel attention scales and also writes 2x/4x average-pooled side outputs from that tile. The model gains a planner that defers the MSPA_C2f attention scaling to its consumers: the stride-2 conv, or igemm convs via in_scale. The intent is to drop the separate scale-and-write pass over the MSPA output and the separate pooling reads. The cost is more template variants and register pressure in the conv kernel, plus a complex routing plan with fallbacks.

Measured after the change: 41140 images/sec (median of 6 runs). No clear change (+0.9%).

```diff
diff --git a/include/mgdt.h b/include/mgdt.h
--- a/include/mgdt.h
+++ b/include/mgdt.h
@@ -131,6 +131,10 @@
 int mgdt_scale_channels_fwd(const mgdt_view* x, const float* attn, const mgdt_view* y, int dtype, mgdt_stream s);
 int mgdt_spr_attn_scale_fwd(const float* pooled, int nsplit, int tiles_x, int tiles_y, const float* fc1_w, const float* fc1_b, const float* fc2_w, const float* fc2_b, int groups,
                             const mgdt_view* x, const mgdt_view* y, const mgdt_view* pool_a, const mgdt_view* pool_b, int dtype, mgdt_stream s);
+int mgdt_conv3x3s2_scaled_fwd(const mgdt_view* x, const float* in_scale, const void* packed_w, const float* bias, int act, const mgdt_view* y,
+                              const mgdt_view* pool_a, const mgdt_view* pool_b, int dtype, mgdt_stream s);
+int mgdt_spr_attn_tiles_fwd(const float* pooled, int nsplit, int tiles_x, int tiles_y, const float* fc1_w, const float* fc1_b, const float* fc2_w,
+                            const float* fc2_b, int groups, int n, int c, int h, int w, float* attn, float* row, int row_len, int seg_off, mgdt_stream s);
 
 int mgdt_sppf_pool_fwd(const mgdt_view* x, const mgdt_view* y1, const mgdt_view* y2, const mgdt_view* y3, int dtype,
                        mgdt_stream s);
diff --git a/mgdt_yolo_amd/_lib.py b/mgdt_yolo_amd/_lib.py
--- a/mgdt_yolo_amd/_lib.py
+++ b/mgdt_yolo_amd/_lib.py
@@ -85,6 +85,8 @@
     'mgdt_conv1x1_inject_conv_supported': (_i, [_i, _i, _i, _i, _i, _i, _i, _i]),
     'mgdt_conv1x1_inject_conv_fwd': (_i, [VP, _vp, _vp, VP, VP, VP, _vp, _vp, _i, _vp, _vp, _i, VP, _i, _vp]),
     'mgdt_spr_attn_scale_fwd': (_i, [_vp, _i, _i, _i, _vp, _vp, _vp, _vp, _i, VP, VP, VP, VP, _i, _vp]),
+    'mgdt_conv3x3s2_scaled_fwd': (_i, [VP, _vp, _vp, _vp, _i, VP, VP, VP, _i, _vp]),
+    'mgdt_spr_attn_tiles_fwd': (_i, [_vp, _i, _i, _i, _vp, _vp, _vp, _vp, _i, _i, _i, _i, _i, _vp, _vp, _i, _i, _vp]),
     'mgdt_stem2_packed_bytes': (_sz, []),
     'mgdt_stem2_pack': (_i, [_vp, _vp, _vp]),
     'mgdt_stem2_fwd': (_i, [VP, _i, _vp, _vp, _vp, _vp, VP, _vp]),
diff --git a/mgdt_yolo_amd/csrc/conv3x3_lds.hip b/mgdt_yolo_amd/csrc/conv3x3_lds.hip
--- a/mgdt_yolo_amd/csrc/conv3x3_lds.hip
+++ b/mgdt_yolo_amd/csrc/conv3x3_lds.hip
@@ -15,6 +15,8 @@
   int N, H, W, Ho, Wo, Cin, Cout, CP, nchunks, NTtot, ncg, tiles_x, tiles_per_img, ntiles, XP, act;
   FastDiv fd_tpi, fd_tx, fd_cp;
   const float* oscale; float xq;
+  const float* in_scale;
+  struct Pool { char* y; int sn, sh, sw; uint32_t bytes; int F; } pool[2];
   unsigned long long* dbg;
 };
 
@@ -24,8 +26,9 @@
   return v;
 }
 
-template <int NBW, int ACT, int NCH, int MT, bool Q8 = false, int S = 1, int WS = 1>
+template <int NBW, int ACT, int NCH, int MT, bool Q8 = false, int S = 1, int WS = 1, bool SC = false>
 __global__ __launch_bounds__(256 * WS, 1) void conv3x3_lds_kernel(const C3Args a) {
+  static_assert(!SC || (S == 2 && !Q8), "input scaling + pooled side outputs: the bf16 stride-2 forms");
   constexpr int NTHR = 256 * WS, NBH = (NBW + WS - 1) / WS;
   constexpr int RW = 15 * S + 3, TH = 4 * MT, RH = (TH - 1) * S + 3, RPX = RH * RW;
   constexpr int MAXI = ((S == 1 ? C3_MAXI : 18) + WS - 1) / WS;
@@ -76,8 +79,15 @@
 
   const int nitems = RPX * a.CP;
   uint4 stage[MAXI];
+  const int c8t = tid - (int)fdiv((uint32_t)tid, a.fd_cp) * a.CP;
+  float scn[SC ? 8 : 1];
   auto issue = [&](int t) {
     const int n = (int)fdiv((uint32_t)t, a.fd_tpi), rt = t - n * a.tiles_per_img;
+    if constexpr (SC) {
+      const float4* sp = (const float4*)(a.in_scale + (long)n * a.Cin + c8t * 8);
+      const float4 s0 = sp[0], s1 = sp[1];
+      scn[0] = s0.x; scn[1] = s0.y; scn[2] = s0.z; scn[3] = s0.w; scn[4] = s1.x; scn[5] = s1.y; scn[6] = s1.z; scn[7] = s1.w;
+    }
     const int tyi = (int)fdiv((uint32_t)rt, a.fd_tx), txi = rt - tyi * a.tiles_x;
     const int iy0 = tyi * TH * S - 1, ix0 = txi * C3_TW * S - 1;
 #pragma unroll
@@ -97,7 +107,13 @@
       if (it < nitems) {
         const int pix = (int)fdiv((uint32_t)it, a.fd_cp), c8 = it - pix * a.CP;
         if constexpr (Q8) *(long*)(xs + pix * a.XP + c8 * 8) = quant8(__builtin_bit_cast(bf16x8, stage[u]), a.xq);
-        else *(uint4*)(xs + pix * a.XP + c8 * 16) = stage[u];
+        else if constexpr (SC) {
+          const bf16x8 v = __builtin_bit_cast(bf16x8, stage[u]);
+          bf16x8 o;
+#pragma unroll
+          for (int i = 0; i < 8; ++i) o[i] = (bf16)((float)v[i] * scn[i]);
+          *(bf16x8*)(xs + pix * a.XP + c8 * 16) = o;
+        } else *(uint4*)(xs + pix * a.XP + c8 * 16) = stage[u];
       }
     }
   };
@@ -119,6 +135,45 @@
     if (a.dbg) { const unsigned long long n_ = __builtin_amdgcn_s_memrealtime(); Tc += n_ - tl; tl = n_; }
     const int tn = t + wstep;
     if (tn < a.ntiles) issue(tn);
+    if constexpr (SC) {
+      if (cg == 0 && (a.pool[0].F | a.pool[1].F)) {
+        const int n = (int)fdiv((uint32_t)t, a.fd_tpi), rt = t - n * a.tiles_per_img;
+        const int tyi = (int)fdiv((uint32_t)rt, a.fd_tx), txi = rt - tyi * a.tiles_x;
+        auto pool_cells = [&](int pi, auto ftag) __attribute__((always_inline)) {
+          constexpr int F = decltype(ftag)::value;
+          const __amdgpu_buffer_rsrc_t prs = __builtin_amdgcn_make_buffer_rsrc((void*)a.pool[pi].y, 0, a.pool[pi].bytes, 0x00020000);
+          const int fs = F == 4 ? 2 : 1, cws = 5 - fs, nit = ((2 * TH) >> fs << cws) * a.CP;
+          const float inv = F == 4 ? 0.0625f : 0.25f;
+          for (int it = tid; it < nit; it += NTHR) {
+            const int cell = (int)fdiv((uint32_t)it, a.fd_cp), c8 = it - cell * a.CP;
+            const int cy = cell >> cws, cx = cell & ((1 << cws) - 1);
+            const int iy = tyi * TH * 2 + (cy << fs), ix = txi * 32 + (cx << fs);
+            float acc[8];
+#pragma unroll
+            for (int k = 0; k < 8; ++k) acc[k] = 0.f;
+            const char* cp0 = xs + ((1 + (cy << fs)) * RW + 1 + (cx << fs)) * a.XP + c8 * 16;
+            bf16x8 v[F * F];
+#pragma unroll
+            for (int e = 0; e < F * F; ++e) v[e] = *(const bf16x8*)(cp0 + ((e / F) * RW + e % F) * a.XP);
+#pragma unroll
+            for (int e = 0; e < F * F; ++e)
+#pragma unroll
+              for (int k = 0; k < 8; ++k) acc[k] += (float)v[e][k];
+            bf16x8 o;
+#pragma unroll
+            for (int k = 0; k < 8; ++k) o[k] = (bf16)(acc[k] * inv);
+            const bool in = iy < a.H && ix < a.W;
+            __builtin_amdgcn_raw_buffer_store_b128(__builtin_bit_cast(__attribute__((__vector_size__(4 * sizeof(unsigned int)))) unsigned int, o), prs,
+                                                   in ? (uint32_t)(n * a.pool[pi].sn + (iy >> fs) * a.pool[pi].sh + (ix >> fs) * a.pool[pi].sw + c8 * 16) : (uint32_t)C3_OOB, 0, 0);
+          }
+        };
+#pragma unroll
+        for (int pi = 0; pi < 2; ++pi) {
+          if (a.pool[pi].F == 2) pool_cells(pi, std::integral_constant<int, 2>{});
+          else if (a.pool[pi].F == 4) pool_cells(pi, std::integral_constant<int, 4>{});
+        }
+      }
+    }
 
     f32x4 acc[NBH][MT];
 #pragma unroll
@@ -233,10 +288,11 @@
 }
 
 bool mgdt_conv3x3_lds_launch(const mgdt_view* x, const mgdt_view* y, const void* packed_w, const float* bias, int act, int CP, int nchunks, int NTtot, hipStream_t st,
-                             const float* q8_oscale, float q8_xq, int stride) {
+                             const float* q8_oscale, float q8_xq, int stride, const float* in_scale, const mgdt_view* pool_a, const mgdt_view* pool_b) {
   const bool q8 = q8_oscale != nullptr;
   C3Plan pl;
   if (!mgdt_conv3x3_lds_plan(x, y, act, CP, nchunks, NTtot, q8, stride, &pl)) return false;
+  if (in_scale && (stride != 2 || q8 || 512 % CP)) return false;
   const int Cin = x->c, Cout = y->c, NBW = pl.NBW, MT = pl.MT, nwg = pl.nwg;
   const size_t lds = pl.lds;
   const bool ws2 = pl.waves == 8;
@@ -248,6 +304,17 @@
   a.N = x->n; a.H = x->h; a.W = x->w; a.Ho = y->h; a.Wo = y->w; a.Cin = Cin; a.Cout = Cout; a.CP = CP; a.nchunks = nchunks; a.NTtot = NTtot; a.act = act;
   a.XP = pl.XP;
   a.oscale = q8_oscale; a.xq = q8_xq;
+  a.in_scale = in_scale;
+  if (in_scale) {
+    const mgdt_view* pv[2] = {pool_a, pool_b};
+    for (int i = 0; i < 2; ++i) {
+      const mgdt_view* p = pv[i];
+      if (!p || !p->p) continue;
+      a.pool[i].y = (char*)p->p; a.pool[i].sn = (int)(p->sn * 2); a.pool[i].sh = (int)(p->sh * 2); a.pool[i].sw = (int)(p->sw * 2);
+      a.pool[i].bytes = (uint32_t)(((long)(p->n - 1) * p->sn + (long)(p->h - 1) * p->sh + (long)(p->w - 1) * p->sw + p->c) * 2);
+      a.pool[i].F = x->h / p->h;
+    }
+  }
   a.ncg = pl.ncg;
   a.tiles_x = pl.tiles_x; a.tiles_per_img = pl.tiles_per_img; a.ntiles = pl.ntiles;
   a.fd_tpi = make_fastdiv((uint32_t)a.tiles_per_img); a.fd_tx = make_fastdiv((uint32_t)a.tiles_x); a.fd_cp = make_fastdiv((uint32_t)CP);
@@ -288,8 +355,14 @@
   a.dbg = dbgbuf;
 #define C3_LAUNCH_S2(ACTV, NCHV)                                                                                      \
   {                                                                                                                  \
-    static std::atomic<bool> sattr{false}, sattr8{false};                                                            \
-    if (ws2) {                                                                                                       \
+    static std::atomic<bool> sattr{false}, sattr8{false}, sattrsc{false}, sattr8sc{false};                           \
+    if (in_scale && ws2) {                                                                                           \
+      if (!sattr8sc) { (void)hipFuncSetAttribute((const void*)conv3x3_lds_kernel<4, ACTV, NCHV, 2, false, 2, 2, true>, hipFuncAttributeMaxDynamicSharedMemorySize, 160 * 1024); sattr8sc = true; } \
+      conv3x3_lds_kernel<4, ACTV, NCHV, 2, false, 2, 2, true><<<nwg, 512, lds, st>>>(a);                             \
+    } else if (in_scale) {                                                                                           \
+      if (!sattrsc) { (void)hipFuncSetAttribute((const void*)conv3x3_lds_kernel<4, ACTV, NCHV, 2, false, 2, 1, true>, hipFuncAttributeMaxDynamicSharedMemorySize, 160 * 1024); sattrsc = true; } \
+      conv3x3_lds_kernel<4, ACTV, NCHV, 2, false, 2, 1, true><<<nwg, 256, lds, st>>>(a);                             \
+    } else if (ws2) {                                                                                                       \
       if (!sattr8) { (void)hipFuncSetAttribute((const void*)conv3x3_lds_kernel<4, ACTV, NCHV, 2, false, 2, 2>, hipFuncAttributeMaxDynamicSharedMemorySize, 160 * 1024); sattr8 = true; } \
       conv3x3_lds_kernel<4, ACTV, NCHV, 2, false, 2, 2><<<nwg, 512, lds, st>>>(a);                                   \
     } else {                                                                                                         \
diff --git a/mgdt_yolo_amd/csrc/conv_igemm.hip b/mgdt_yolo_amd/csrc/conv_igemm.hip
--- a/mgdt_yolo_amd/csrc/conv_igemm.hip
+++ b/mgdt_yolo_amd/csrc/conv_igemm.hip
@@ -335,7 +335,7 @@
 
 bool mgdt_conv3x3_lds_plan(const mgdt_view* x, const mgdt_view* y, int act, int CP, int nchunks, int NTtot, bool q8, int stride, C3Plan* p);
 bool mgdt_conv3x3_lds_launch(const mgdt_view* x, const mgdt_view* y, const void* packed_w, const float* bias, int act, int CP, int nchunks, int NTtot, hipStream_t st,
-                             const float* q8_oscale, float q8_xq, int stride);
+                             const float* q8_oscale, float q8_xq, int stride, const float* in_scale, const mgdt_view* pool_a, const mgdt_view* pool_b);
 
 template <typename T, int NT, int MT, bool Q8>
 int launch_igemm(const ConvArgs& a, const IgemmPlan& p, hipStream_t st);
@@ -373,8 +373,8 @@
 static inline bool conv_view_aligned(const mgdt_view* v, int q, int dtype) {
   return v->sc == 1 && v->sw % q == 0 && v->sh % q == 0 && v->sn % q == 0 && ((uintptr_t)v->p % (q * dtype_size(dtype))) == 0;
 }
-static inline bool conv_lds_candidate(int tapmode, int dtype, int k, bool x2, bool in_scale, bool in_shift, bool r1, bool r2) {
-  return tapmode == 0 && dtype == MGDT_BF16 && k == 3 && !x2 && !in_scale && !in_shift && !r1 && !r2;
+static inline bool conv_lds_candidate(int tapmode, int dtype, int k, int stride, bool q8, bool x2, bool in_scale, bool in_shift, bool r1, bool r2) {
+  return tapmode == 0 && dtype == MGDT_BF16 && k == 3 && !x2 && (!in_scale || (stride == 2 && !q8)) && !in_shift && !r1 && !r2;
 }
 static int igemm_plan(int nchunks, int NTtot, long M, bool q8, bool extra, IgemmPlan* p) {
   const int WB = q8 ? 512 : 1024;
@@ -487,8 +487,8 @@
   if (M > 0x7fffffffL - (1 << 20)) MGDT_FAIL(MGDT_BAD_SHAPE, "conv2d: problem too large");
   a.M = (int)M; a.HoWo = Ho * Wo;
   a.fd_howo = make_fastdiv((uint32_t)a.HoWo); a.fd_wo = make_fastdiv((uint32_t)Wo);
-  if (conv_lds_candidate(tapmode, dtype, k, x2 && x2->p, in_scale, in_shift, r1 && r1->p, r2 && r2->p) &&
-      mgdt_conv3x3_lds_launch(x, y, packed_w, bias, act, a.CP, a.nchunks, a.NTtot, (hipStream_t)s, q8_oscale, q8_xq, stride)) {
+  if (conv_lds_candidate(tapmode, dtype, k, stride, q8, x2 && x2->p, in_scale, in_shift, r1 && r1->p, r2 && r2->p) &&
+      mgdt_conv3x3_lds_launch(x, y, packed_w, bias, act, a.CP, a.nchunks, a.NTtot, (hipStream_t)s, q8_oscale, q8_xq, stride, in_scale, nullptr, nullptr)) {
     MGDT_CHECK_LAUNCH("conv2d(3x3 lds)");
     return MGDT_OK;
   }
@@ -500,6 +500,34 @@
   if (q8) return dispatch_igemm_q8(a, pl, st);
   if (dtype == MGDT_F32) return dispatch_igemm<float>(a, pl, st);
   return dispatch_igemm<bf16>(a, pl, st);
+}
+
+extern "C" int mgdt_conv3x3s2_scaled_fwd(const mgdt_view* x, const float* in_scale, const void* packed_w, const float* bias, int act, const mgdt_view* y,
+                                         const mgdt_view* pool_a, const mgdt_view* pool_b, int dtype, mgdt_stream s) {
+  if (!view_ok(x) || !view_ok(y) || !packed_w || !bias || !in_scale) MGDT_FAIL(MGDT_BAD_ARG, "conv3x3s2_scaled: null/empty argument");
+  if (dtype != MGDT_BF16) MGDT_FAIL(MGDT_BAD_DTYPE, "conv3x3s2_scaled: bf16 only");
+  int Ho, Wo;
+  if (int rc = conv_check_shapes(x, y, 3, 2, dtype, &Ho, &Wo)) return rc;
+  if (!conv_view_aligned(x, 8, dtype) || !conv_view_aligned(y, 4, dtype)) MGDT_FAIL(MGDT_BAD_SHAPE, "conv3x3s2_scaled: x/y must be NHWC views (sc==1) with 16-byte aligned pieces");
+  const mgdt_view* pv[2] = {pool_a, pool_b};
+  int F[2] = {0, 0};
+  for (int i = 0; i < 2; ++i) {
+    const mgdt_view* p = pv[i];
+    if (!p || !p->p) continue;
+    if (!view_ok(p) || p->n != x->n || p->c != x->c || p->h < 1 || p->w < 1 || x->h % p->h || x->w % p->w || x->h / p->h != x->w / p->w || !conv_view_aligned(p, 8, dtype))
+      MGDT_FAIL(MGDT_BAD_SHAPE, "conv3x3s2_scaled: a pooled output must be a 16-byte aligned NHWC view of the same n, c whose size divides the map by one factor");
+    F[i] = x->h / p->h;
+    if (F[i] != 2 && F[i] != 4) MGDT_FAIL(MGDT_BAD_SHAPE, "conv3x3s2_scaled: pooling factor %d (2 and 4 are built)", F[i]);
+    const long ext = ((long)(p->n - 1) * p->sn + (long)(p->h - 1) * p->sh + (long)(p->w - 1) * p->sw + p->c) * 2;
+    if (ext >= 0x7fffffffL) MGDT_FAIL(MGDT_BAD_SHAPE, "conv3x3s2_scaled: a pooled view spans >= 2 GiB");
+  }
+  if (F[0] && F[0] == F[1]) MGDT_FAIL(MGDT_BAD_SHAPE, "conv3x3s2_scaled: two pooled outputs with one factor");
+  int CP, nchunks, NTtot;
+  conv_geometry(x->c, y->c, 3, dtype, &CP, &nchunks, &NTtot);
+  if (!mgdt_conv3x3_lds_launch(x, y, packed_w, bias, act, CP, nchunks, NTtot, (hipStream_t)s, nullptr, 1.f, 2, in_scale, pool_a, pool_b))
+    MGDT_FAIL(MGDT_BAD_SHAPE, "conv3x3s2_scaled: cin=%d cout=%d %dx%d n=%d is not a layer the LDS-staged stride-2 kernel takes", x->c, y->c, x->h, x->w, x->n);
+  MGDT_CHECK_LAUNCH("conv3x3s2_scaled");
+  return MGDT_OK;
 }
 
 extern "C" int mgdt_conv2d_route(const mgdt_view* x, const mgdt_view* y, int k, int stride, int dtype, int flags, int act, mgdt_conv_route* out) {
@@ -519,7 +547,7 @@
   memset(out, 0, sizeof(*out));
   out->nchunks = nchunks;
   C3Plan c3;
-  if (conv_lds_candidate(0, dtype, k, flags & MGDT_ROUTE_X2, flags & MGDT_ROUTE_IN_SCALE, flags & MGDT_ROUTE_IN_SHIFT, flags & MGDT_ROUTE_R1, flags & MGDT_ROUTE_R2) &&
+  if (conv_lds_candidate(0, dtype, k, stride, q8, flags & MGDT_ROUTE_X2, flags & MGDT_ROUTE_IN_SCALE, flags & MGDT_ROUTE_IN_SHIFT, flags & MGDT_ROUTE_R1, flags & MGDT_ROUTE_R2) &&
       mgdt_conv3x3_lds_plan(&xv, &yv, act, CP, nchunks, NTtot, q8, stride, &c3)) {
     out->family = MGDT_ROUTE_LDS3X3;
     out->NBW = c3.NBW; out->tile_rows = 4 * c3.MT; out->ncg = c3.ncg; out->nwg = c3.nwg; out->ntiles = c3.ntiles; out->waves = c3.waves;
diff --git a/mgdt_yolo_amd/csrc/conv_igemm_kernel.h b/mgdt_yolo_amd/csrc/conv_igemm_kernel.h
--- a/mgdt_yolo_amd/csrc/conv_igemm_kernel.h
+++ b/mgdt_yolo_amd/csrc/conv_igemm_kernel.h
@@ -208,8 +208,8 @@
   };
 
   auto load_chunk = [&](const uint4* ep, const TileState(&S)[MT], frag(&P)[MT]) __attribute__((always_inline)) {
-    uint32_t ex, ey, ez = 0, ew = 0;
-    if (EXTRA) { const uint4 e = *ep; ex = e.x; ey = e.y; ez = e.z; ew = e.w; }
+    uint32_t ex, ey, ez = 0;
+    if (EXTRA) { const uint4 e = *ep; ex = e.x; ey = e.y; ez = e.z; }
     else { const uint2 e = *(const uint2*)ep; ex = e.x; ey = e.y; }
 #pragma unroll
     for (int mt = 0; mt < MT; ++mt) {
@@ -221,11 +221,27 @@
           const uint32_t off2 = ok ? (uint32_t)S[mt].x2o + ez : (uint32_t)MGDT_OOB;
           v = frag_add<T>(v, __builtin_bit_cast(frag, __builtin_amdgcn_raw_buffer_load_b128(x2rs, off2, 0, 0)));
         }
-        if (ok && (a.in_scale || a.in_shift))
-          v = frag_affine<T>(v, a.in_scale ? a.in_scale + (long)S[mt].pn * a.Cin + ew : nullptr, a.in_shift ? a.in_shift + ew : nullptr);
       }
       P[mt] = v;
     }
+  };
+  auto load_scale = [&](const uint4* ep, const TileState(&S)[MT], float(&Q)[MT][PE]) __attribute__((always_inline)) {
+    if (!a.in_scale) return;
+    const uint4 e = *ep;
+#pragma unroll
+    for (int mt = 0; mt < MT; ++mt) {
+      const bool ok = (S[mt].vm >> e.y) & 1u;
+      const float* p = a.in_scale + (ok ? (long)S[mt].pn * a.Cin + e.w : 0l);
+#pragma unroll
+      for (int i = 0; i < PE; ++i) Q[mt][i] = p[i];
+    }
+  };
+  auto affine_chunk = [&](const uint4* ep, const TileState(&S)[MT], frag(&P)[MT], const float(&Q)[MT][PE]) __attribute__((always_inline)) {
+    if (!(a.in_scale || a.in_shift)) return;
+    const uint4 e = *ep;
+#pragma unroll
+    for (int mt = 0; mt < MT; ++mt)
+      if ((S[mt].vm >> e.y) & 1u) P[mt] = frag_affine<T>(P[mt], a.in_scale ? Q[mt] : nullptr, a.in_shift ? a.in_shift + e.w : nullptr);
   };
 
   f32x4 acc[NT][MT];
@@ -339,6 +355,8 @@
   load_chunk(tab_g, cur, P[0]);
   if constexpr (L > 1) load_chunk(tab_g + 4, cur, P[1]);
   if constexpr (L > 2) load_chunk(tab_g + 8, cur, P[2]);
+  float SC[2][MT][PE];
+  if constexpr (EXTRA) load_scale(tab_g, cur, SC[0]);
   if (!MULTI) { stage(0); __syncthreads(); }
   const char* const wlane = wlds + lane * (WB / 64);
   constexpr bool multi = MULTI;
@@ -351,8 +369,10 @@
     auto step_cur = [&](int j, auto dtag) __attribute__((always_inline)) {
       constexpr int d = decltype(dtag)::value;
       load_chunk(tp, cur, P[(d + L) % D]);
+      if constexpr (EXTRA) load_scale(tp - 4 * L + 4, cur, SC[(d + 1) & 1]);
+      if (multi && kl == 0) { __syncthreads(); stage(j / a.seg_chunks); __syncthreads(); wp = wlane; }
+      if constexpr (EXTRA) affine_chunk(tp - 4 * L, cur, P[d], SC[d & 1]);
       tp += 4;
-      if (multi && kl == 0) { __syncthreads(); stage(j / a.seg_chunks); __syncthreads(); wp = wlane; }
       compute(wp, P[d]);
       wp += NT * WB;
       if (multi && ++kl == a.seg_chunks) kl = 0;
@@ -369,8 +389,13 @@
     auto step_last = [&](int j, auto dtag) __attribute__((always_inline)) {
       constexpr int d = decltype(dtag)::value;
       load_chunk(tab_g + 4 * (d - 1), nxt, P[(d + L) % D]);
+      if constexpr (EXTRA) {
+        if constexpr (d == D - 1) load_scale(tab_g, nxt, SC[0]);
+        else load_scale(tab_g + 4 * (j + 1), cur, SC[(d + 1) & 1]);
+      }
       if (j < a.nchunks) {
         if (multi && kl == 0) { __syncthreads(); stage(j / a.seg_chunks); __syncthreads(); wp = wlane; }
+        if constexpr (EXTRA) affine_chunk(tab_g + 4 * j, cur, P[d], SC[d & 1]);
         compute(wp, P[d]);
         wp += NT * WB;
         if (multi && ++kl == a.seg_chunks) kl = 0;
diff --git a/mgdt_yolo_amd/csrc/pointwise.hip b/mgdt_yolo_amd/csrc/pointwise.hip
--- a/mgdt_yolo_amd/csrc/pointwise.hip
+++ b/mgdt_yolo_amd/csrc/pointwise.hip
@@ -437,26 +437,19 @@
   __syncthreads();
 }
 
-template <typename T, int V>
-__global__ __launch_bounds__(256) void spr_attn_scale_kernel(const float* __restrict__ partial, const float* __restrict__ w1, const float* __restrict__ b1,
-                                                             const float* __restrict__ w2, const float* __restrict__ b2, int C, int G, int H, int W,
-                                                             const T* __restrict__ x, long xsn, long xsh, long xsw, T* __restrict__ y, long ysn, long ysh,
-                                                             long ysw, FastDiv fd_q, FastDiv fd_w, int nsplit, int tiles_x, int tiles_y, SprPool pa, SprPool pb, FastDiv fd_gst,
-                                                             FastDiv fd_tx, FastDiv fd_l4, int fast, unsigned long long* dbg) {
-  extern __shared__ float sm[];
-  unsigned long long TS[10]; int nt = 0;
-  auto stamp = [&]() __attribute__((always_inline)) { if (dbg) TS[nt++] = __builtin_amdgcn_s_memrealtime(); };
-  stamp();
-  const int n = blockIdx.y, cw = C / G, hid = cw / 4;
+__device__ __forceinline__ float* spr_prologue(const float* __restrict__ partial, const float* __restrict__ w1, const float* __restrict__ b1,
+                                               const float* __restrict__ w2, const float* __restrict__ b2, int C, int G, int H, int W, int n, int nsplit,
+                                               int tiles_x, int tiles_y, FastDiv fd_gst, FastDiv fd_tx, FastDiv fd_l4, int fast, float* sm, float* red,
+                                               unsigned long long* TS, int& nt) {
+  const int cw = C / G, hid = cw / 4;
   float* pooled = sm;
   float* hbuf = sm + C * 5;
   float* obuf = hbuf + G * hid;
   float* att = obuf + C;
   const int hs1 = bin_start(1, H, 2), he0 = bin_end(0, H, 2), ws1 = bin_start(1, W, 2), we0 = bin_end(0, W, 2);
   const float cnt[5] = {(float)H * W, (float)he0 * we0, (float)he0 * (W - ws1), (float)(H - hs1) * we0, (float)(H - hs1) * (W - ws1)};
-  __shared__ float red[5 * 256];
   if (fast) {
-    spr_prologue_fast(partial, w1, b1, w2, b2, C, G, n, nsplit, tiles_x, tiles_y, fd_gst, fd_tx, fd_l4, cnt, sm, red, att, dbg ? TS : nullptr, nt);
+    spr_prologue_fast(partial, w1, b1, w2, b2, C, G, n, nsplit, tiles_x, tiles_y, fd_gst, fd_tx, fd_l4, cnt, sm, red, att, TS, nt);
   } else {
     if (tiles_x > 0) {
       const int gst = nsplit / (tiles_x * tiles_y);
@@ -522,6 +515,22 @@
     }
     __syncthreads();
   }
+  return att;
+}
+
+template <typename T, int V>
+__global__ __launch_bounds__(256) void spr_attn_scale_kernel(const float* __restrict__ partial, const float* __restrict__ w1, const float* __restrict__ b1,
+                                                             const float* __restrict__ w2, const float* __restrict__ b2, int C, int G, int H, int W,
+                                                             const T* __restrict__ x, long xsn, long xsh, long xsw, T* __restrict__ y, long ysn, long ysh,
+                                                             long ysw, FastDiv fd_q, FastDiv fd_w, int nsplit, int tiles_x, int tiles_y, SprPool pa, SprPool pb, FastDiv fd_gst,
+                                                             FastDiv fd_tx, FastDiv fd_l4, int fast, unsigned long long* dbg) {
+  extern __shared__ float sm[];
+  unsigned long long TS[10]; int nt = 0;
+  auto stamp = [&]() __attribute__((always_inline)) { if (dbg) TS[nt++] = __builtin_amdgcn_s_memrealtime(); };
+  stamp();
+  const int n = blockIdx.y;
+  __shared__ float red[5 * 256];
+  float* att = spr_prologue(partial, w1, b1, w2, b2, C, G, H, W, n, nsplit, tiles_x, tiles_y, fd_gst, fd_tx, fd_l4, fast, sm, red, dbg ? TS : nullptr, nt);
   stamp();
   auto fin = [&]() __attribute__((always_inline)) { if (dbg) { __builtin_amdgcn_s_waitcnt(0); stamp(); if (threadIdx.x == 0) for (int k = 0; k < 8; ++k) dbg[((size_t)blockIdx.y * gridDim.x + blockIdx.x) * 8 + k] = TS[k]; } };
   {
@@ -594,6 +603,15 @@
   fin();
 }
 
+static size_t spr_prologue_lds(int c, int groups, int tiles_x, const float* fc1_w, int* fast) {
+  const int cw = c / groups, hid = cw / 4;
+  size_t lds = (size_t)(c * 5 + groups * hid + 2 * c) * sizeof(float);
+  const size_t wbytes = ((size_t)hid * (5 * cw + 4) + (size_t)cw * (hid + 1) + hid + cw + 4) * sizeof(float);
+  *fast = tiles_x > 0 && c <= 256 && lds + wbytes <= 48 * 1024 && ((uintptr_t)fc1_w & 15) == 0;
+  if (*fast) lds += wbytes;
+  return lds;
+}
+
 extern "C" int mgdt_spr_attn_scale_fwd(const float* pooled, int nsplit, int tiles_x, int tiles_y, const float* fc1_w, const float* fc1_b, const float* fc2_w, const float* fc2_b, int groups,
                                        const mgdt_view* x, const mgdt_view* y, const mgdt_view* pool_a, const mgdt_view* pool_b, int dtype, mgdt_stream s) {
   if (nsplit <= 0) nsplit = SPR_SPLITS;
@@ -604,11 +622,9 @@
   if (groups < 1 || c % groups || (c / groups) % 4 || c > 4096) MGDT_FAIL(MGDT_BAD_SHAPE, "spr_attn_scale: c=%d groups=%d", c, groups);
   if (!vec4_ok(x, dtype) || !vec4_ok(y, dtype) || x->n != y->n || x->h != y->h || x->w != y->w || y->c != c)
     MGDT_FAIL(MGDT_BAD_SHAPE, "spr_attn_scale: views must be matching NHWC, c%%4==0");
-  const int cw = c / groups, hid = cw / 4;
-  size_t lds = (size_t)(c * 5 + groups * hid + 2 * c) * sizeof(float);
-  const size_t wbytes = ((size_t)hid * (5 * cw + 4) + (size_t)cw * (hid + 1) + hid + cw + 4) * sizeof(float);
-  const int fast = tiles_x > 0 && c <= 256 && lds + wbytes <= 48 * 1024 && ((uintptr_t)fc1_w & 15) == 0;
-  if (fast) lds += wbytes;
+  const int cw = c / groups;
+  int fast;
+  const size_t lds = spr_prologue_lds(c, groups, tiles_x, fc1_w, &fast);
   SprPool pl[2] = {{nullptr, 0, 0, 0, 0}, {nullptr, 0, 0, 0, 0}};
   bool pool8 = true;
   const mgdt_view* pv[2] = {pool_a, pool_b};
@@ -647,6 +663,41 @@
     for (int k = 0; k + 1 < ns; ++k) fprintf(stderr, " %.2f", ph[k] * 0.01 / (gK * x->n));
     fprintf(stderr, fast ? "  (issue | loads land | sums | fc1 | fc2 | softmax | scale)\n" : "  (prologue | scale)\n");
   }
+  return MGDT_OK;
+}
+
+__global__ __launch_bounds__(256) void spr_attn_tiles_kernel(const float* __restrict__ partial, const float* __restrict__ w1, const float* __restrict__ b1,
+                                                             const float* __restrict__ w2, const float* __restrict__ b2, int C, int G, int H, int W, int nsplit,
+                                                             int tiles_x, int tiles_y, FastDiv fd_gst, FastDiv fd_tx, FastDiv fd_l4, int fast, float* __restrict__ attn,
+                                                             float* __restrict__ row, int row_len, int off) {
+  extern __shared__ float sm[];
+  __shared__ float red[5 * 256];
+  const int n = blockIdx.x;
+  int nt = 0;
+  const float* att = spr_prologue(partial, w1, b1, w2, b2, C, G, H, W, n, nsplit, tiles_x, tiles_y, fd_gst, fd_tx, fd_l4, fast, sm, red, nullptr, nt);
+  if (attn)
+    for (int i = threadIdx.x; i < C; i += 256) attn[(long)n * C + i] = att[i];
+  if (row) {
+    float* r = row + (long)n * row_len;
+    for (int i = threadIdx.x; i < row_len; i += 256) r[i] = (i >= off && i < off + C) ? att[i - off] : 1.0f;
+  }
+}
+
+extern "C" int mgdt_spr_attn_tiles_fwd(const float* pooled, int nsplit, int tiles_x, int tiles_y, const float* fc1_w, const float* fc1_b, const float* fc2_w,
+                                       const float* fc2_b, int groups, int n, int c, int h, int w, float* attn, float* row, int row_len, int seg_off, mgdt_stream s) {
+  if (!pooled || !fc1_w || !fc1_b || !fc2_w || !fc2_b || (!attn && !row)) MGDT_FAIL(MGDT_BAD_ARG, "spr_attn_tiles: null pointer");
+  if (n < 1 || h < 1 || w < 1 || groups < 1 || c < 1 || c % groups || (c / groups) % 4 || c > 4096) MGDT_FAIL(MGDT_BAD_SHAPE, "spr_attn_tiles: n=%d c=%d groups=%d map %dx%d", n, c, groups, h, w);
+  if (row && (seg_off < 0 || row_len < c || seg_off > row_len - c)) MGDT_FAIL(MGDT_BAD_SHAPE, "spr_attn_tiles: segment [%d, %d) outside a row of %d", seg_off, seg_off + c, row_len);
+  if (nsplit <= 0) nsplit = SPR_SPLITS;
+  if (tiles_x > 0 && (tiles_y <= 0 || nsplit % (tiles_x * tiles_y) || tiles_x % 2 || tiles_y % 2 || h % 2 || w % 2))
+    MGDT_FAIL(MGDT_BAD_SHAPE, "spr_attn_tiles: per-tile sums need an even tile grid over an even map (nsplit=%d tiles %dx%d)", nsplit, tiles_y, tiles_x);
+  int fast;
+  const size_t lds = spr_prologue_lds(c, groups, tiles_x, fc1_w, &fast);
+  if (lds + 5 * 256 * sizeof(float) > 64 * 1024) MGDT_FAIL(MGDT_BAD_SHAPE, "spr_attn_tiles: c=%d needs %zu bytes of LDS", c, lds);
+  spr_attn_tiles_kernel<<<n, 256, lds, (hipStream_t)s>>>(pooled, fc1_w, fc1_b, fc2_w, fc2_b, c, groups, h, w, nsplit, tiles_x, tiles_y,
+                                                         make_fastdiv((uint32_t)(tiles_x > 0 ? nsplit / (tiles_x * tiles_y) : 1)), make_fastdiv((uint32_t)std::max(tiles_x, 1)),
+                                                         make_fastdiv((uint32_t)(5 * (c / groups) / 4)), fast, attn, row, row_len, seg_off);
+  MGDT_CHECK_LAUNCH("spr_attn_tiles_fwd");
   return MGDT_OK;
 }
 
diff --git a/mgdt_yolo_amd/nn/modules/block.py b/mgdt_yolo_amd/nn/modules/block.py
--- a/mgdt_yolo_amd/nn/modules/block.py
+++ b/mgdt_yolo_amd/nn/modules/block.py
@@ -202,17 +202,22 @@
             raise RuntimeError('MSPA_C2f: only stride=1 is wired by parse_model and built here')
         d_out = deliver.get('out') if deliver else None
         d_pools = deliver.get('pools', ()) if deliver else ()
+        defer = deliver.get('defer') if deliver and not d_pools else None
         b, _, h, w = x.shape
         wd, s, n = self.inwidth, self.nums, self.btnk_nums
         train = self.training and hasattr(self.convs[0], 'bn')
         run = (lambda m: m.train_fwd) if train else (lambda m: m.run)
         dt = self.convs[0].out_dtype(x)
         at = self.attention
-        if (not train and s == 4 and self.inwidth == self.outwidth and self._chain_ok() and _plain_block(self.convs[0], self.convs[3], self.bottleneck)
-                and ops.csp_block_supported(ops.CSP_MSPA, x, self.convs[3].conv.out_channels, wd, n, dt)):
+        if not train and self.csp_route_ok(x):
             mids = [pk for m in self.bottleneck for pk in (m.cv1.packed(dt, False), m.cv2.packed(dt, False))]
             out, pool, slots, tiles = ops.csp_block(ops.CSP_MSPA, x, self._packed_chain(dt).blob, None, mids, self.bottleneck[0].add,
-                                                    self.convs[3].packed(dt, False), wd, act_code(self.convs[0].act), self.convs[3].conv.out_channels, True)
+                                                    self.convs[3].packed(dt, False), wd, act_code(self.convs[0].act), self.convs[3].conv.out_channels, True,
+                                                    out=d_out if defer is not None else None)
+            if defer is not None:
+                deliver['attn'], deliver['row'] = ops.spr_attention_tiles(pool, slots, tiles, at.fc1.weight, at.fc1.bias, at.fc2.weight, at.fc2.bias, s, out.shape,
+                                                                          row_len=defer[0], offset=defer[1])
+                return out
             return ops.spr_attention_scale(out, at.fc1.weight, at.fc1.bias, at.fc2.weight, at.fc2.bias, s, out=d_out, part=pool, nsplit=slots, tiles=tiles, pools=d_pools)
         cat = ops.new_act(b, (s - 1 + n) * wd, h, w, dt, x.device)
         if not train and s == 4 and ops.pw_chain_supported(wd, cat.dtype) and x.dtype == cat.dtype and self._chain_ok():
@@ -233,6 +238,10 @@
         else:
             return ops.spr_attention_scale(out, at.fc1.weight, at.fc1.bias, at.fc2.weight, at.fc2.bias, s, out=d_out, pools=d_pools)
         return ops.scale_channels(out, attn)
+
+    def csp_route_ok(self, x):
+        return (self.nums == 4 and self.inwidth == self.outwidth and self._chain_ok() and _plain_block(self.convs[0], self.convs[3], self.bottleneck)
+                and ops.csp_block_supported(ops.CSP_MSPA, x, self.convs[3].conv.out_channels, self.inwidth, self.btnk_nums, self.convs[0].out_dtype(x)))
 
     def _chain_ok(self):
         cs = list(self.convs)[:3]
@@ -290,12 +299,15 @@
         self.cv2 = Conv(c_ * 4, c2, 1, 1)
         self.m = nn.MaxPool2d(kernel_size=k, stride=1, padding=k // 2)
 
-    def forward(self, x):
+    def forward(self, x, in_scale=None):
         b, _, h, w = x.shape
         c_ = self.cv1.conv.out_channels
         train = self.training and hasattr(self.cv1, 'bn')
         cat = ops.new_act(b, 4 * c_, h, w, self.cv1.out_dtype(x), x.device)
-        (self.cv1.train_fwd if train else self.cv1.run)(x, out=cat[:, :c_])
+        if in_scale is not None:
+            self.cv1.run(x, out=cat[:, :c_], in_scale=in_scale)
+        else:
+            (self.cv1.train_fwd if train else self.cv1.run)(x, out=cat[:, :c_])
         ops.sppf_pools(cat[:, :c_], cat[:, c_:2 * c_], cat[:, 2 * c_:3 * c_], cat[:, 3 * c_:])
         if train:
             self._cat = cat if ops.ctx_enabled() else None
@@ -443,14 +455,20 @@
         self.conv = nn.Sequential(Conv(inc, embed_dim_p), *[ConvNeXtV2_Block(embed_dim_p) for _ in range(fuse_block_num)],
                                   Conv(embed_dim_p, sum(ouc)))
 
-    def forward(self, x):
+    def forward(self, x, in_scale=None):
         mods = list(self.conv)
+        if in_scale is not None:
+            x, mods = mods[0].run(x, in_scale=in_scale), mods[1:]
         if (not self.training and len(mods) >= 2 and isinstance(mods[-2], ConvNeXtV2_Block) and not mods[-2]._forward_hooks and not self.conv._forward_hooks):
             for m in mods[:-2]:
                 x = m(x)
             r = mods[-2](x, tail=mods[-1])
             return r[0] if isinstance(r, tuple) else mods[-1](r)
-        return self.conv(x)
+        if in_scale is None:
+            return self.conv(x)
+        for m in mods:
+            x = m(x)
+        return x
 
     def backward(self, g):
         for m in reversed(list(self.conv)):
diff --git a/mgdt_yolo_amd/nn/modules/conv.py b/mgdt_yolo_amd/nn/modules/conv.py
--- a/mgdt_yolo_amd/nn/modules/conv.py
+++ b/mgdt_yolo_amd/nn/modules/conv.py
@@ -167,6 +167,21 @@
                 return ops.conv2d_fp8(x, self.packed_fp8(xq), s, act_code(self.act), out=out, x2=x2, r1=r1, r2=r2, in_scale=in_scale, in_shift=in_shift)
         pk = self.packed(dt, direct=not mfma)
         return ops.conv2d(x, pk, s, act_code(self.act), out=out, x2=x2, r1=r1, r2=r2, in_scale=in_scale, in_shift=in_shift)
+
+    def scaled_s2_ok(self, x):
+        c = self.conv
+        if not (c.kernel_size == (3, 3) and c.stride == (2, 2) and c.padding == (1, 1) and c.dilation == (1, 1) and c.groups == 1 and self.out_dtype(x) == torch.bfloat16
+                and x.dtype == torch.bfloat16 and ops.conv_can_mfma(x, c.in_channels, c.out_channels, 3, 2, 1, torch.bfloat16) and self.__dict__.get('_q8') is None):
+            return False
+        b, _, h, w = x.shape
+        ho, wo = ops.conv_out_hw(h, w, 3, 2)
+        y = torch.empty((b, c.out_channels, ho, wo), dtype=torch.bfloat16, device='meta', memory_format=torch.channels_last)
+        return ops.conv2d_route(x, y, 3, 2, act=act_code(self.act), in_scale=True)['family'] == 'lds3x3'
+
+    def run_scaled_s2(self, x, in_scale, pools=()):
+        if hasattr(self, 'bn'):
+            self._no_train_bn(self.bn)
+        return ops.conv3x3s2_scaled(x, self.packed(torch.bfloat16, direct=False), act_code(self.act), in_scale, pools=pools)
 
     def forward(self, x):
         if self.training and hasattr(self, 'bn'):
diff --git a/mgdt_yolo_amd/nn/tasks.py b/mgdt_yolo_amd/nn/tasks.py
--- a/mgdt_yolo_amd/nn/tasks.py
+++ b/mgdt_yolo_amd/nn/tasks.py
@@ -81,6 +81,8 @@
             y = [None, x if 1 in self.save else None]
             layers = list(self.model)[2:]
         plan = self._neck_plan(x) if not self.training else None
+        defer = self._spr_plan(plan)
+        scales = {}
         bufs = {}
         head = None
         side = self._side_branch() if not self.training else None
@@ -92,12 +94,46 @@
             nonlocal head
             src = lambda j: prev[m.i - 1] if j == -1 else y[m.i + j if j < 0 else j]
             xin = src(m.f) if isinstance(m.f, int) else [src(j) for j in m.f]
-            if head is not None:
+            unscaled = [j for j in self._abs_from(m) if j in scales] if scales else ()
+            if unscaled:
+                j = unscaled[0]
+                kind = lambda k: ('pooled' if m.i in defer[k]['pooled'] else 'concat' if (defer[k]['concat'] or (None,))[0] == m.i else None) if k in defer else None
+                if isinstance(m, (SimFusion_4in, SimFusion_3in)) and all(kind(k) for k in unscaled):
+                    out = m(xin, pre=bufs.get(m.i))
+                    for k in unscaled:
+                        if kind(k) == 'concat':
+                            scales[m.i] = defer[k]['row']
+                elif len(unscaled) > 1 or not isinstance(m.f, int):
+                    raise RuntimeError(f'layer {m.i} ({type(m).__name__}) reads the unscaled outputs of layers {unscaled}: not a reader BaseModel._spr_plan admits')
+                elif defer.get(j, {}).get('lds') == m.i:
+                    out = m.run_scaled_s2(xin, scales[j], defer[j]['pools'])
+                elif isinstance(m, Conv):
+                    out = m.run(xin, in_scale=scales[j])
+                elif isinstance(m, (SPPF, IFM)):
+                    out = m(xin, in_scale=scales[j])
+                else:
+                    raise RuntimeError(f'layer {m.i} ({type(m).__name__}) reads the unscaled output of layer {j}: not a reader BaseModel._spr_plan admits')
+            elif head is not None:
                 out, head = m(None, head=head), None
             elif self._injection_feeds_next(m):
                 head, out = (m, xin), None
-            elif plan is not None and m.i in plan['producers']:
-                out = m(xin, deliver=self._neck_deliveries(plan, m, xin, bufs))
+            elif plan is not None and (m.i in plan['producers'] or m.i in defer):
+                d = self._neck_deliveries(plan, m, xin, bufs) if m.i in plan['producers'] else None
+                pools = []
+                if m.i in defer:
+                    cat, lds = defer[m.i]['concat'], defer[m.i]['lds']
+                    if lds is not None:
+                        if (d is not None and d.get('out') is None and len(d.get('pools', ())) == len(defer[m.i]['pooled']) and m.csp_route_ok(xin)
+                                and self.model[lds].scaled_s2_ok(ops.new_act(xin.shape[0], m.convs[3].conv.out_channels, xin.shape[2], xin.shape[3], xin.dtype, 'meta'))):
+                            pools, d = d['pools'], {'defer': (0, 0)}
+                    elif cat is None or (d is not None and d.get('out') is not None and not d.get('pools')):
+                        d = dict(d or {}, defer=(cat[2], cat[1]) if cat else (0, 0))
+                out = m(xin, deliver=d)
+                if d is not None and d.get('attn') is not None:
+                    scales[m.i] = d['attn']
+                    defer[m.i]['row'], defer[m.i]['pools'] = d['row'], pools
+                elif pools:
+                    raise RuntimeError('MSPA_C2f did not take the csp_block route its deferred plan checked for')
             elif plan is not None and m.i in plan['consumers']:
                 out = m(xin, pre=bufs.get(m.i))
             else:
@@ -190,6 +226,62 @@
         if any(self.model[i]._forward_hooks for i in list(plan['producers']) + list(plan['consumers'])):
             return None
         return plan
+
+    def _abs_from(self, m):
+        return [m.i + f if f < 0 else f for f in ([m.f] if isinstance(m.f, int) else m.f)]
+
+    def _spr_plan(self, plan):
+        if plan is None or not ops.DEFERRED_SPR or ops.Q8_CALIB is not None or getattr(self, 'fp8_table', None):
+            return {}
+        static = self.__dict__.get('_spr_plan_cache')
+        if static is None:
+            static, rows = {}, set()
+            readers = {}
+            for m in self.model:
+                for j in self._abs_from(m):
+                    readers.setdefault(j, []).append(m.i)
+            conv_ok = lambda c: (isinstance(c, Conv) and not isinstance(c, DWConv) and c.conv.groups == 1 and c.conv.kernel_size in ((1, 1), (3, 3))
+                                 and c.conv.in_channels % 8 == 0 and c.conv.out_channels % 4 == 0)
+            for mj in self.model:
+                j = mj.i
+                if not isinstance(mj, MSPA_C2f) or not readers.get(j):
+                    continue
+                prods = plan['producers'].get(j, [])
+                concat, watch, ok, lds, igemm = None, [j], True, None, False
+                if any(k == 'pool' for k, _, _ in prods):
+                    convs = [i for i in readers[j] if isinstance(self.model[i].f, int) and conv_ok(self.model[i]) and self.model[i].conv.stride == (2, 2)
+                             and self.model[i].conv.kernel_size == (3, 3)]
+                    rest = [i for i in readers[j] if i not in convs]
+                    if (len(convs) == 1 and all(k == 'pool' for k, _, _ in prods) and len(prods) <= 2 and sorted(rest) == sorted(ci for _, ci, _ in prods)
+                            and len(set(rest)) == len(rest)):
+                        static[j] = {'concat': None, 'watch': [j] + readers[j], 'lds': convs[0], 'pooled': rest, 'igemm': False}
+                    continue
+                for i in readers[j]:
+                    m = self.model[i]
+                    watch.append(i)
+                    if isinstance(m.f, int) and (conv_ok(m) or (isinstance(m, SPPF) and conv_ok(m.cv1))):
+                        igemm = True
+                        continue
+                    nxt = self.model[i + 1] if i + 1 < len(self.model) else None
+                    if (isinstance(m, SimFusion_4in) and concat is None and i not in rows and self._abs_from(m).count(j) == 1 and self._abs_from(m)[2] == j
+                            and ('main', i, 2) in plan['producers'].get(j, []) and readers.get(i) == [i + 1] and i not in self.save
+                            and isinstance(nxt, IFM) and nxt.f == -1 and conv_ok(nxt.conv[0])):
+                        cs = [self.model[k].c2 for k in self._abs_from(m)]
+                        concat = (i, sum(cs[:2]), sum(cs))
+                        watch.append(i + 1)
+                        igemm = True
+                        continue
+                    ok = False
+                    break
+                if ok:
+                    static[j] = {'concat': concat, 'watch': watch, 'lds': None, 'pooled': [], 'igemm': igemm}
+                    if concat:
+                        rows.add(concat[0])
+            self.__dict__['_spr_plan_cache'] = static
+        only = ops.spr_defer_levels()
+        hooked = lambda i: bool(self.model[i]._forward_hooks) or (isinstance(self.model[i], IFM) and bool(self.model[i].conv._forward_hooks or self.model[i].conv[0]._forward_hooks)) \
+            or (isinstance(self.model[i], SPPF) and bool(self.model[i].cv1._forward_hooks))
+        return {j: dict(d) for j, d in static.items() if (j in only if only is not None else not d['igemm']) and not any(hooked(i) for i in d['watch'])}
 
     def _neck_deliveries(self, plan, m, x, bufs):
         b, c, h, w = x.shape
diff --git a/mgdt_yolo_amd/ops.py b/mgdt_yolo_amd/ops.py
--- a/mgdt_yolo_amd/ops.py
+++ b/mgdt_yolo_amd/ops.py
@@ -276,6 +276,23 @@
     return out
 
 
+def conv3x3s2_scaled(x, pk, act, in_scale, out=None, pools=()):
+    _need_gpu(x)
+    b, _, h, w = x.shape
+    ho, wo = conv_out_hw(h, w, 3, 2)
+    if out is None:
+        out = new_act(b, pk.cout, ho, wo, pk.dtype, x.device)
+    pools = list(pools)
+    if len(pools) > 2 or pk.k != 3 or pk.direct:
+        raise RuntimeError('conv3x3s2_scaled: a packed 3x3 MFMA panel and at most two pooled outputs')
+    _same(x, out, *pools)
+    if x.dtype != pk.dtype:
+        raise RuntimeError(f'conv3x3s2_scaled: the weights are packed for {pk.dtype}, the input is {x.dtype}')
+    pa, pb = (pools + [None, None])[:2]
+    _launch('conv3x3s2_scaled_fwd', 'mgdt_conv3x3s2_scaled_fwd', vp(x), ptr(in_scale), ptr(pk.w), ptr(pk.bias), act, vp(out), vp(pa), vp(pb), dtype_code(pk.dtype), stream())
+    return out
+
+
 def conv2d_route(x, y, k, stride, dtype=None, act=ACT_SILU, x2=False, in_scale=False, in_shift=False, r1=False, r2=False, fp8=False):
     def shape_view(t):
         b, c, h, w = t.shape
@@ -337,6 +354,25 @@
     _launch('spr_attn_scale_fwd', 'mgdt_spr_attn_scale_fwd', ptr(part), int(nsplit), int(tiles[0]), int(tiles[1]), ptr(fc1_w), ptr(fc1_b), ptr(fc2_w), ptr(fc2_b), groups, vp(x), vp(out),
             vp(pa), vp(pb), dtype_code(x.dtype), stream())
     return out
+
+
+def spr_attention_tiles(part, nsplit, tiles, fc1_w, fc1_b, fc2_w, fc2_b, groups, shape, attn=True, row_len=0, offset=0):
+    b, c, h, w = shape
+    a = torch.empty(b, c, dtype=torch.float32, device=part.device) if attn else None
+    row = torch.empty(b, int(row_len), dtype=torch.float32, device=part.device) if row_len else None
+    _launch('spr_attn_tiles_fwd', 'mgdt_spr_attn_tiles_fwd', ptr(part), int(nsplit), int(tiles[0]), int(tiles[1]), ptr(fc1_w), ptr(fc1_b), ptr(fc2_w), ptr(fc2_b),
+            int(groups), int(b), int(c), int(h), int(w), ptr(a), ptr(row), int(row_len), int(offset), stream())
+    return a, row
+
+
+DEFERRED_SPR = True
+
+
+def spr_defer_levels():
+    e = os.environ.get('MGDT_SPR_DEFER')
+    if e is None or e.strip() == '':
+        return None
+    return {int(t) for t in e.split(',') if t.strip().lstrip('-').isdigit()}
 
 
 FUSED_NECK = True
@@ -461,7 +497,7 @@
     return lib.mgdt_csp_block_tiles(mode, x.shape[0], x.shape[1], int(cout), int(wd), int(nbtl), x.shape[2], x.shape[3], None) > 0
 
 
-def csp_block(mode, x, front, front_bias, mids, shortcut, back, wd, act, cout, want_pool):
+def csp_block(mode, x, front, front_bias, mids, shortcut, back, wd, act, cout, want_pool, out=None):
     lib = L.lib()
     b, cin, h, w = x.shape
     nb = len(mids) // 2
@@ -469,7 +505,10 @@
     slots = lib.mgdt_csp_block_tiles(mode, b, cin, cout, wd, nb, h, w, geom)
     if slots <= 0:
         raise RuntimeError('csp_block: configuration not covered')
-    y = new_act(b, cout, h, w, x.dtype, x.device)
+    y = new_act(b, cout, h, w, x.dtype, x.device) if out is None else out
+    if tuple(y.shape) != (b, cout, h, w):
+        raise RuntimeError(f'csp_block: out must be {(b, cout, h, w)}, got {tuple(y.shape)}')
+    _same(x, y)
     pool = torch.empty(b * slots * cout, dtype=torch.float32, device=x.device) if want_pool else None
     marr = (C.c_void_p * len(mids))(*[m.w.data_ptr() for m in mids])
     barr = (C.c_void_p * len(mids))(*[m.bias.data_ptr() for m in mids])
```
